# SeanChenxy/TDRN

Measured on AMD Instinct MI355X. Metric: frames/sec/GPU @320x320 dualrefinedet_vggbn; box Linf vs CPU ref, higher is better.
Workload: dtype bf16; 1 GPU; dualrefinedet_vggbn 320x320 multihead, bf16, batch 32 per GPU, forward + Detect(top_k 200, conf 0.01, nms 0.45), synthetic VOC-shaped frames + synthetic weights; global_batch=32, parallelism=frame-sharded x1, no per-frame collective, launch=eager, resident_batches=4, steps_in_flight=2

## Files before the change

include/tdrn_hip.h:

```cpp
#ifndef TDRN_HIP_H
#define TDRN_HIP_H

#include <stddef.h>
#include <stdint.h>

#ifdef __cplusplus
extern "C" {
#endif

#define TDRN_API __attribute__((visibility("default")))

#define TDRN_OK 0
#define TDRN_E_ARG (-1)
#define TDRN_E_SHAPE (-2)
#define TDRN_E_WORKSPACE (-3)
#define TDRN_E_UNSUPPORTED (-4)
#define TDRN_E_PARAM (-5)
#define TDRN_E_STATE (-6)
#define TDRN_E_VALUE (-7)
#define TDRN_E_DEVICE (-8)

TDRN_API const char *tdrn_version(void);
TDRN_API const char *tdrn_error_string(int code);

// ... 23 lines not shown
                                                  float *grad_weight, int N, int Cin, int H, int W, int Cout, int kW,
                                                  int kH, int dW, int dH, int padW, int padH, int dilationH,
                                                  int dilationW, int deformable_group, float scale,
                                                  void *workspace, size_t workspace_bytes, void *stream);


TDRN_API size_t tdrn_nms_workspace_bytes(int n);
TDRN_API int tdrn_nms(const float *dets, int n, double thresh, int strict_gt, int32_t *keep_out,
                      int32_t *num_out, void *workspace, size_t workspace_bytes, void *stream);

TDRN_API int tdrn_nms_topk(const float *dets, int n, float overlap, float min_score, int top_k,
                           int32_t *keep_out, int32_t *num_out, void *workspace,
                           size_t workspace_bytes, void *stream);

TDRN_API size_t tdrn_nms_topk_classes_workspace_bytes(int n, int num_classes);
TDRN_API int tdrn_nms_topk_classes(const float *boxes, const float *scores, int n, int num_classes, int first_class,
                                   float overlap, float min_score, int top_k, int32_t *keep_out, int32_t *num_out,
                                   void *workspace, size_t workspace_bytes, void *stream);

TDRN_API int tdrn_roi_resample(const float *feature, int C, int H, int W, const int32_t *cells, int n, int S, float *out,
                               void *stream);
TDRN_API int tdrn_ota_similarity(const float *boxes, const float *roi, int n, int F, const float *rows, const int32_t *row_off,
                                 int m, float *best, int32_t *arg, void *stream);

TDRN_API int tdrn_gpu_nms_host(int *keep_out, int *num_out, const float *boxes_host,
                               int boxes_num, int boxes_dim, float nms_overlap_thresh,
                               int device_id);

TDRN_API int tdrn_decode(const float *loc, const float *priors, int P, float var0, float var1,
                         float *boxes_out, void *stream);
TDRN_API int tdrn_center_size(const float *boxes, int P, float *out, void *stream);

TDRN_API int tdrn_encode(const float *matched, const float *priors, int P, float var0, float var1, float *out, void *stream);
TDRN_API size_t tdrn_match_workspace_bytes(int B, int P, int max_truths);
TDRN_API int tdrn_match(const float *truths, const int32_t *truth_off, int T_total, int max_truths, int B,
                        const float *priors, int P, const float *arm_loc, float threshold, float var0, float var1,
                        float *loc_t, int32_t *conf_t, void *workspace, size_t workspace_bytes, void *stream);
TDRN_API size_t tdrn_multibox_loss_workspace_bytes(int B, int P, int C);
TDRN_API int tdrn_multibox_loss_forward(const float *loc, const float *conf, const float *loc_t, const int32_t *conf_t,
                                        int B, int P, int C, int negpos_ratio, float *loss_out, uint8_t *sel,
                                        int32_t *num_pos, void *workspace, size_t workspace_bytes, void *stream);
TDRN_API int tdrn_multibox_loss_backward(const float *loc, const float *conf, const float *loc_t, const int32_t *conf_t,
                                         const uint8_t *sel, const int32_t *num_pos, const float *grad_loss, int B,
                                         int P, int C, float *grad_loc, float *grad_conf, void *stream);

#define TDRN_AUGMENT_MAX_TRUTHS 512
#define TDRN_AUGMENT_MAX_ROUNDS 32
#define TDRN_AUGMENT_MAX_SIZE 2048
#define TDRN_AUGMENT_CROP_FALLBACK 1
#define TDRN_AUGMENT_TAPE_EXHAUSTED 2
typedef struct {
    float brightness;
    float contrast_pre;
    float contrast_post;
    float saturation;
    float hue;
    int32_t perm[3];
    int32_t canvas_w, canvas_h, img_x, img_y;
    int32_t crop_x0, crop_y0, crop_x1, crop_y1;
    int32_t cropped;
    int32_t mirror;
    int32_t kept;
    int32_t status;
} tdrn_augment_params;
typedef struct {
    const uint8_t *data;
    int32_t h, w;
} tdrn_augment_image;
TDRN_API int tdrn_augment_sample(const int32_t *hw, const double *truths, const int32_t *truth_off, int T_total, int max_truths,
                                 int B, uint64_t seed, const int64_t *sample_ids, const double *tape, const int32_t *tape_off,
                                 tdrn_augment_params *params, float *out_truths, int32_t *out_off, void *stream);
TDRN_API int tdrn_augment_apply(const tdrn_augment_image *images, const tdrn_augment_params *params, int B, const float *mean,
                                int S, int to_rgb, float *out, void *stream);

#define TDRN_AUGMENT_TRANS_FALLBACK 4
typedef struct {
    tdrn_augment_params base;
    double shift_x, shift_y;
    int32_t trans_x, trans_y;
    int32_t attempts;
    int32_t reserved;
} tdrn_augment_pair_params;
TDRN_API int tdrn_augment_pair_sample(const int32_t *hw, const double *truths, const double *truths_t, const int32_t *truth_off,
                                      int T_total, int max_truths, int B, double max_trans_ratio, uint64_t seed,
                                      const int64_t *sample_ids, const double *tape, const int32_t *tape_off,
                                      tdrn_augment_pair_params *params, float *out_truths, float *out_truths_t,
                                      int32_t *out_off, void *stream);
TDRN_API int tdrn_augment_pair_apply(const tdrn_augment_image *images, const tdrn_augment_image *images_t,
                                     const tdrn_augment_pair_params *params, int B, const float *mean, int S, int to_rgb,
                                     float *out, float *out_t, void *stream);

TDRN_API int tdrn_prior_box(int n_maps, const int *feature_maps, double image_size,
                            const double *steps, const double *min_sizes,
                            const double *max_sizes, int n_max_sizes, const int *ar_count,
                            const double *ars, int clip, int flip, float *out_host);

TDRN_API size_t tdrn_detect_workspace_bytes(int B, int P, int C, int top_k);
TDRN_API int tdrn_detect(const float *loc, const float *conf, const float *priors,
                         const float *arm_loc, const float *scale_host, int B, int P, int C,
                         int top_k, float conf_thresh, double nms_thresh, float *out,
                         int32_t *counts_out, void *workspace, size_t workspace_bytes,
                         void *stream);
TDRN_API int tdrn_detect_dev_scale(const float *loc, const float *conf, const float *priors,
                                   const float *arm_loc, const float *scale_dev, int B, int P, int C,
                                   int top_k, float conf_thresh, double nms_thresh, float *out,
                                   int32_t *counts_out, void *workspace, size_t workspace_bytes,
                                   void *stream);

TDRN_API int tdrn_preprocess(const uint8_t *frames, int B, int H0, int W0, int S, const float mean_bgr[3],
                             int to_rgb, float *out, void *stream);
TDRN_API int tdrn_preprocess_u8(const uint8_t *frames, int B, int H0, int W0, int S, int to_rgb, uint8_t *out, void *stream);

typedef enum {
    TDRN_DRN_VGGBN = 0,
    TDRN_DRN_MOBILENET = 1,
    TDRN_SSD4SCALE_MOBILE = 2,
    TDRN_REFINEDET_VGG = 3,
    TDRN_SSD4SCALE_VGG = 4
} tdrn_model;

typedef struct {
    int model;
    int size;
    int num_classes;
    int c7_channel;
    int def_groups;
    int bn;
    int multihead;
    int deform;
    int test_phase;
    int dtype;
    int use_refine;
    int plan_flags;
    int reserved[4];
} tdrn_net_config;

#define TDRN_PLAN_NO_FUSE_FIRST 1
#define TDRN_PLAN_NO_LATE_SIDE  2
#define TDRN_PLAN_ONE_STREAM    4
#define TDRN_PLAN_NO_DEFORM_TS  8
#define TDRN_PLAN_CHAIN         16
#define TDRN_PLAN_NO_CONV_PP    32
#define TDRN_PLAN_NO_PP_SK      64
#define TDRN_PLAN_NO_CONV_PATCH 128
#define TDRN_PLAN_DWPW          512
#define TDRN_PLAN_NO_PW1X1      1024
#define TDRN_PLAN_NO_DW_SLIDE   2048
#define TDRN_PLAN_DW_SLIDE_ALL  4096
#define TDRN_PLAN_NO_CONV_WS    8192
#define TDRN_PLAN_NO_YGEMM_V2  16384
#define TDRN_PLAN_NO_HEAD3X3   32768
#define TDRN_PLAN_TS_ONE_RANGE  65536
#define TDRN_PLAN_NO_PATCH_TAIL 131072
#define TDRN_PLAN_FAULT_HANDOFF 256

typedef struct tdrn_net tdrn_net;

TDRN_API int tdrn_net_create(const tdrn_net_config *cfg, tdrn_net **out);
TDRN_API void tdrn_net_destroy(tdrn_net *net);

TDRN_API int tdrn_net_param_count(const tdrn_net *net);
TDRN_API int tdrn_net_param_info(const tdrn_net *net, int index, const char **name,
                                 int64_t shape[4], int *ndim);
TDRN_API int tdrn_net_set_param(tdrn_net *net, const char *name, const float *data_host,
                                int64_t numel);

TDRN_API size_t tdrn_net_weight_bytes(const tdrn_net *net);
TDRN_API size_t tdrn_net_workspace_bytes(const tdrn_net *net, int batch);
TDRN_API int tdrn_net_num_priors(const tdrn_net *net);

TDRN_API int tdrn_net_pack_weights(tdrn_net *net, void *weights_dev, size_t weights_bytes,
                                   void *stream);
TDRN_API int tdrn_net_adopt_weights(tdrn_net *net);

typedef struct {
    const float *x;
    int batch;
    float *arm_loc;
    float *odm_loc;
    float *conf;
    float *offsets[4];
    const float *ref_loc[4];
    float *loc_maps[4];
    void *reserved[4];
} tdrn_net_io;
typedef struct {
    const uint8_t *planes;
    float mean[3];
} tdrn_u8_frames;

TDRN_API int tdrn_net_forward(tdrn_net *net, const void *weights_dev, void *workspace,
                              size_t workspace_bytes, const tdrn_net_io *io, void *stream);

TDRN_API int tdrn_net_check(tdrn_net *net, unsigned *detail);

typedef struct {
    char name[48];
    int launches;
    double flops;
    double bytes;
    double ms;
} tdrn_kernel_stat;
TDRN_API int tdrn_net_profile(tdrn_net *net, int enable);
TDRN_API int tdrn_net_kernel_stats(tdrn_net *net, tdrn_kernel_stat *out, int max_entries);
TDRN_API int tdrn_net_op_stats(tdrn_net *net, tdrn_kernel_stat *out, int max_entries);
TDRN_API int tdrn_net_op_timeline(tdrn_net *net, float *start_ms, float *end_ms, int *lane, int max_entries);

typedef struct {
    int kind;
    int in, out, res;
    int pool;
    int off, y;
    int k, stride, pad, dil, relu, ceil_mode, splitk, groups;
    int out_kind;
    int level;
    int n_branches, k2, pad2, off_c0[2];
    int y_tap_major;
    int fused_first;
    int fused_dw;
    char w[48], b[48], bn[48], w2[48], b2[48];
    int y_groups;
} tdrn_op_info;
TDRN_API int tdrn_net_op_count(const tdrn_net *net);
TDRN_API int tdrn_net_op_info(const tdrn_net *net, int index, tdrn_op_info *out);

TDRN_API int tdrn_net_tensor_count(const tdrn_net *net);
TDRN_API int tdrn_net_tensor_info(const tdrn_net *net, int index, const char **label, int *C, int *H,
                                  int *W);
TDRN_API int tdrn_net_read_tensor(const tdrn_net *net, const void *workspace, int batch, int index,
                                  float *out_dev, void *stream);
TDRN_API int tdrn_net_write_tensor(const tdrn_net *net, void *workspace, int batch, int index,
                                   const float *in_dev, void *stream);
TDRN_API int tdrn_net_forward_from(tdrn_net *net, const void *weights_dev, void *workspace,
                                   size_t workspace_bytes, const tdrn_net_io *io, int first_op, void *stream);

#ifdef __cplusplus
}
#endif
#endif
```

tdrn_amd/_lib.py:

```python
import ctypes as C
import os

_HERE = os.path.dirname(os.path.abspath(__file__))
LIB_PATH = os.environ.get("TDRN_LIB_PATH") or os.path.join(_HERE, "lib", "libtdrn_hip.so")

F32, BF16, F16 = 0, 1, 2
DTYPES = {"fp32": F32, "f32": F32, "float32": F32, "bf16": BF16, "bfloat16": BF16, "fp16": F16,
          "f16": F16, "float16": F16, "half": F16}
DRN_VGGBN, DRN_MOBILENET, SSD4SCALE_MOBILE, REFINEDET_VGG, SSD4SCALE_VGG = range(5)

E_VALUE = -7


class TdrnError(RuntimeError):
    def __init__(self, code, what=""):
        self.code = code
        super().__init__("%s (tdrn error %d)%s" % (error_string(code), code,
                                                    (": " + what) if what else ""))


class NetConfig(C.Structure):
    _fields_ = [("model", C.c_int), ("size", C.c_int), ("num_classes", C.c_int),
                ("c7_channel", C.c_int), ("def_groups", C.c_int), ("bn", C.c_int),
                ("multihead", C.c_int), ("deform", C.c_int), ("test_phase", C.c_int),
                ("dtype", C.c_int), ("use_refine", C.c_int), ("plan_flags", C.c_int), ("reserved", C.c_int * 4)]


PLAN_NO_FUSE_FIRST, PLAN_NO_LATE_SIDE, PLAN_ONE_STREAM, PLAN_NO_DEFORM_TS, PLAN_CHAIN = 1, 2, 4, 8, 16
PLAN_NO_CONV_PP, PLAN_NO_PP_SK, PLAN_NO_CONV_PATCH, PLAN_FAULT_HANDOFF, PLAN_DWPW, PLAN_NO_PW1X1 = 32, 64, 128, 256, 512, 1024
PLAN_NO_DW_SLIDE, PLAN_DW_SLIDE_ALL, PLAN_NO_CONV_WS, PLAN_NO_YGEMM_V2, PLAN_NO_HEAD3X3, PLAN_TS_ONE_RANGE = 2048, 4096, 8192, 16384, 32768, 65536
PLAN_NO_PATCH_TAIL = 131072
E_DEVICE = -8


class NetIO(C.Structure):
    _fields_ = [("x", C.c_void_p), ("batch", C.c_int), ("arm_loc", C.c_void_p),
                ("odm_loc", C.c_void_p), ("conf", C.c_void_p), ("offsets", C.c_void_p * 4),
                ("ref_loc", C.c_void_p * 4), ("loc_maps", C.c_void_p * 4),
                ("reserved", C.c_void_p * 4)]


class KernelStat(C.Structure):
    _fields_ = [("name", C.c_char * 48), ("launches", C.c_int), ("flops", C.c_double),
                ("bytes", C.c_double), ("ms", C.c_double)]


class U8FramesABI(C.Structure):
    _fields_ = [("planes", C.c_void_p), ("mean", C.c_float * 3)]


class OpInfo(C.Structure):
    _fields_ = [("kind", C.c_int), ("in_", C.c_int), ("out", C.c_int), ("res", C.c_int), ("pool", C.c_int), ("off", C.c_int),
                ("y", C.c_int), ("k", C.c_int), ("stride", C.c_int), ("pad", C.c_int), ("dil", C.c_int), ("relu", C.c_int),
                ("ceil_mode", C.c_int), ("splitk", C.c_int), ("groups", C.c_int), ("out_kind", C.c_int), ("level", C.c_int),
                ("n_branches", C.c_int), ("k2", C.c_int), ("pad2", C.c_int), ("off_c0", C.c_int * 2), ("y_tap_major", C.c_int),
                ("fused_first", C.c_int), ("fused_dw", C.c_int), ("w", C.c_char * 48), ("b", C.c_char * 48), ("bn", C.c_char * 48), ("w2", C.c_char * 48),
                ("b2", C.c_char * 48), ("y_groups", C.c_int)]


class AugmentParams(C.Structure):
    _fields_ = [("brightness", C.c_float), ("contrast_pre", C.c_float), ("contrast_post", C.c_float), ("saturation", C.c_float),
                ("hue", C.c_float), ("perm", C.c_int32 * 3), ("canvas_w", C.c_int32), ("canvas_h", C.c_int32),
                ("img_x", C.c_int32), ("img_y", C.c_int32), ("crop_x0", C.c_int32), ("crop_y0", C.c_int32),
                ("crop_x1", C.c_int32), ("crop_y1", C.c_int32), ("cropped", C.c_int32), ("mirror", C.c_int32),
                ("kept", C.c_int32), ("status", C.c_int32)]


class AugmentImage(C.Structure):
    _fields_ = [("data", C.c_void_p), ("h", C.c_int32), ("w", C.c_int32)]


class AugmentPairParams(C.Structure):
    _fields_ = [("base", AugmentParams), ("shift_x", C.c_double), ("shift_y", C.c_double), ("trans_x", C.c_int32),
                ("trans_y", C.c_int32), ("attempts", C.c_int32), ("reserved", C.c_int32)]


AUGMENT_MAX_TRUTHS, AUGMENT_MAX_SIZE = 512, 2048
AUGMENT_CROP_FALLBACK, AUGMENT_TAPE_EXHAUSTED, AUGMENT_TRANS_FALLBACK = 1, 2, 4

OP_KINDS = ("first_conv", "conv", "conv_transpose", "depthwise", "maxpool", "l2norm", "offset_conv", "deform_heads", "other")

_lib = None

_SIGS = {
    "tdrn_version": (C.c_char_p, []),
    "tdrn_error_string": (C.c_char_p, [C.c_int]),
    "tdrn_deform_conv_workspace_bytes": (C.c_size_t, [C.c_int] * 15),
    "tdrn_deform_conv_forward": (C.c_int, [C.c_void_p] * 4 + [C.c_int] * 15 + [C.c_void_p, C.c_size_t, C.c_void_p]),
    "tdrn_deform_conv_backward_workspace_bytes": (C.c_size_t, [C.c_int] * 14),
    "tdrn_deform_conv_backward_input": (C.c_int, [C.c_void_p] * 6 + [C.c_int] * 14 + [C.c_void_p, C.c_size_t, C.c_void_p]),
    "tdrn_deform_conv_backward_parameters": (C.c_int, [C.c_void_p] * 4 + [C.c_int] * 14 + [C.c_float, C.c_void_p, C.c_size_t,
                                                                                            C.c_void_p]),
    "tdrn_nms_workspace_bytes": (C.c_size_t, [C.c_int]),
    "tdrn_nms": (C.c_int, [C.c_void_p, C.c_int, C.c_double, C.c_int, C.c_void_p, C.c_void_p,
                           C.c_void_p, C.c_size_t, C.c_void_p]),
    "tdrn_nms_topk": (C.c_int, [C.c_void_p, C.c_int, C.c_float, C.c_float, C.c_int, C.c_void_p, C.c_void_p,
                                C.c_void_p, C.c_size_t, C.c_void_p]),
    "tdrn_gpu_nms_host": (C.c_int, [C.c_void_p, C.c_void_p, C.c_void_p, C.c_int, C.c_int, C.c_float, C.c_int]),
    "tdrn_decode": (C.c_int, [C.c_void_p, C.c_void_p, C.c_int, C.c_float, C.c_float, C.c_void_p, C.c_void_p]),
    "tdrn_center_size": (C.c_int, [C.c_void_p, C.c_int, C.c_void_p, C.c_void_p]),
    "tdrn_encode": (C.c_int, [C.c_void_p, C.c_void_p, C.c_int, C.c_float, C.c_float, C.c_void_p, C.c_void_p]),
    "tdrn_match_workspace_bytes": (C.c_size_t, [C.c_int] * 3),
    "tdrn_match": (C.c_int, [C.c_void_p, C.c_void_p, C.c_int, C.c_int, C.c_int, C.c_void_p, C.c_int, C.c_void_p, C.c_float,
                             C.c_float, C.c_float, C.c_void_p, C.c_void_p, C.c_void_p, C.c_size_t, C.c_void_p]),
    "tdrn_multibox_loss_workspace_bytes": (C.c_size_t, [C.c_int] * 3),
    "tdrn_multibox_loss_forward": (C.c_int, [C.c_void_p] * 4 + [C.c_int] * 4 + [C.c_void_p] * 4 + [C.c_size_t, C.c_void_p]),
    "tdrn_multibox_loss_backward": (C.c_int, [C.c_void_p] * 7 + [C.c_int] * 3 + [C.c_void_p] * 3),
    "tdrn_augment_sample": (C.c_int, [C.c_void_p] * 3 + [C.c_int] * 3 + [C.c_uint64] + [C.c_void_p] * 7),
    "tdrn_augment_apply": (C.c_int, [C.c_void_p, C.c_void_p, C.c_int, C.c_void_p, C.c_int, C.c_int, C.c_void_p, C.c_void_p]),
    "tdrn_augment_pair_sample": (C.c_int, [C.c_void_p] * 4 + [C.c_int] * 3 + [C.c_double, C.c_uint64] + [C.c_void_p] * 8),
    "tdrn_augment_pair_apply": (C.c_int, [C.c_void_p] * 3 + [C.c_int, C.c_void_p, C.c_int, C.c_int] + [C.c_void_p] * 3),
    "tdrn_prior_box": (C.c_int, [C.c_int, C.c_void_p, C.c_double, C.c_void_p, C.c_void_p, C.c_void_p,
                                 C.c_int, C.c_void_p, C.c_void_p, C.c_int, C.c_int, C.c_void_p]),
    "tdrn_nms_topk_classes_workspace_bytes": (C.c_size_t, [C.c_int, C.c_int]),
    "tdrn_nms_topk_classes": (C.c_int, [C.c_void_p, C.c_void_p, C.c_int, C.c_int, C.c_int, C.c_float, C.c_float, C.c_int, C.c_void_p,
                                        C.c_void_p, C.c_void_p, C.c_size_t, C.c_void_p]),
    "tdrn_roi_resample": (C.c_int, [C.c_void_p, C.c_int, C.c_int, C.c_int, C.c_void_p, C.c_int, C.c_int, C.c_void_p, C.c_void_p]),
    "tdrn_ota_similarity": (C.c_int, [C.c_void_p, C.c_void_p, C.c_int, C.c_int, C.c_void_p, C.c_void_p, C.c_int, C.c_void_p, C.c_void_p,
                                      C.c_void_p]),
    "tdrn_preprocess": (C.c_int, [C.c_void_p, C.c_int, C.c_int, C.c_int, C.c_int, C.c_void_p, C.c_int, C.c_void_p, C.c_void_p]),
    "tdrn_preprocess_u8": (C.c_int, [C.c_void_p, C.c_int, C.c_int, C.c_int, C.c_int, C.c_int, C.c_void_p, C.c_void_p]),
    "tdrn_detect_workspace_bytes": (C.c_size_t, [C.c_int] * 4),
    "tdrn_detect": (C.c_int, [C.c_void_p] * 5 + [C.c_int] * 4 + [C.c_float, C.c_double, C.c_void_p,
                                                                  C.c_void_p, C.c_void_p, C.c_size_t, C.c_void_p]),
    "tdrn_detect_dev_scale": (C.c_int, [C.c_void_p] * 5 + [C.c_int] * 4 + [C.c_float, C.c_double, C.c_void_p,
                                                                            C.c_void_p, C.c_void_p, C.c_size_t, C.c_void_p]),
    "tdrn_net_create": (C.c_int, [C.POINTER(NetConfig), C.POINTER(C.c_void_p)]),
    "tdrn_net_destroy": (None, [C.c_void_p]),
    "tdrn_net_param_count": (C.c_int, [C.c_void_p]),
    "tdrn_net_param_info": (C.c_int, [C.c_void_p, C.c_int, C.POINTER(C.c_char_p), C.POINTER(C.c_int64 * 4),
                                      C.POINTER(C.c_int)]),
    "tdrn_net_set_param": (C.c_int, [C.c_void_p, C.c_char_p, C.c_void_p, C.c_int64]),
    "tdrn_net_weight_bytes": (C.c_size_t, [C.c_void_p]),
    "tdrn_net_workspace_bytes": (C.c_size_t, [C.c_void_p, C.c_int]),
    "tdrn_net_num_priors": (C.c_int, [C.c_void_p]),
    "tdrn_net_pack_weights": (C.c_int, [C.c_void_p, C.c_void_p, C.c_size_t, C.c_void_p]),
    "tdrn_net_adopt_weights": (C.c_int, [C.c_void_p]),
    "tdrn_net_forward": (C.c_int, [C.c_void_p, C.c_void_p, C.c_void_p, C.c_size_t, C.POINTER(NetIO), C.c_void_p]),
    "tdrn_net_check": (C.c_int, [C.c_void_p, C.POINTER(C.c_uint)]),
    "tdrn_net_op_count": (C.c_int, [C.c_void_p]),
    "tdrn_net_op_info": (C.c_int, [C.c_void_p, C.c_int, C.POINTER(OpInfo)]),
    "tdrn_net_tensor_count": (C.c_int, [C.c_void_p]),
    "tdrn_net_tensor_info": (C.c_int, [C.c_void_p, C.c_int, C.POINTER(C.c_char_p), C.POINTER(C.c_int),
                                       C.POINTER(C.c_int), C.POINTER(C.c_int)]),
    "tdrn_net_read_tensor": (C.c_int, [C.c_void_p, C.c_void_p, C.c_int, C.c_int, C.c_void_p, C.c_void_p]),
    "tdrn_net_write_tensor": (C.c_int, [C.c_void_p, C.c_void_p, C.c_int, C.c_int, C.c_void_p, C.c_void_p]),
    "tdrn_net_forward_from": (C.c_int, [C.c_void_p, C.c_void_p, C.c_void_p, C.c_size_t, C.POINTER(NetIO), C.c_int, C.c_void_p]),
    "tdrn_net_profile": (C.c_int, [C.c_void_p, C.c_int]),
    "tdrn_net_kernel_stats": (C.c_int, [C.c_void_p, C.POINTER(KernelStat), C.c_int]),
    "tdrn_net_op_stats": (C.c_int, [C.c_void_p, C.POINTER(KernelStat), C.c_int]),
    "tdrn_net_op_timeline": (C.c_int, [C.c_void_p, C.POINTER(C.c_float), C.POINTER(C.c_float), C.POINTER(C.c_int), C.c_int]),
}
EXPORTS = tuple(_SIGS)


def lib():
    global _lib
    if _lib is None:
        if not os.path.exists(LIB_PATH):
            raise ImportError(
                "libtdrn_hip.so is missing (%s): build it with `python -c 'import __graft_entry__ as g; "
                "g.build()'` or `make -C tdrn_amd/csrc`.  tdrn_amd has no CPU fallback." % LIB_PATH)
        try:
            import torch
            if torch.cuda.is_available():
                torch.cuda.init()
        except ImportError:
            pass
        l = C.CDLL(LIB_PATH)
        for name, (res, args) in _SIGS.items():
            fn = getattr(l, name)
            fn.restype = res
            fn.argtypes = args
        _lib = l
    return _lib


def error_string(code):
    try:
        return lib().tdrn_error_string(int(code)).decode()
    except Exception:
        return "tdrn error"


# ... 28 lines not shown
```

tdrn_amd/csrc/conv3x3_patch.hip:

```cpp
#include <cstdio>
#include <cstdlib>
#include <type_traits>

#include "kernels.h"
#include "mfma_prims.h"

#ifndef TDRN_PATCH_PRIO
#define TDRN_PATCH_PRIO 4
#endif
#ifndef TDRN_PATCH_ABLATE
#define TDRN_PATCH_ABLATE 0
#endif

namespace tdrn {

struct PatchParams {
    const char *in, *w, *zero;
    const float *bias;
    char *out, *out_pool;
    int B, H, W, Cin, Cout, Cs, Ktot;
    int relu;
    int tw, lgtw;
    int tiles_x, tiles_per_img;
    int m_tiles, n_tiles, items;
    int M;
    int tail_split;
    const float *fx, *fw, *fb;
    int fS, fCout;
    int ablate;
#ifdef TDRN_PATCH_STAMP
    unsigned *stamps;
#endif
#ifdef TDRN_PATCH_WGTIME
    unsigned long long *wgt;
#endif
};

#ifdef TDRN_PATCH_STAMP
#define STAMP_DECL unsigned long long st_t = __builtin_amdgcn_s_memtime(); unsigned st_acc[8] = {0, 0, 0, 0, 0, 0, 0, 0};
#define STAMP(k) do { const unsigned long long t_ = __builtin_amdgcn_s_memtime(); st_acc[k] += (unsigned)(t_ - st_t); st_t = t_; } while (0)
#define STAMP_FLUSH do { if (lane == 0) for (int k_ = 0; k_ < 8; ++k_) p.stamps[((size_t)blockIdx.x * 12 + wave) * 8 + k_] = st_acc[k_]; } while (0)
#else
#define STAMP_DECL
#define STAMP(k) do { } while (0)
#define STAMP_FLUSH do { } while (0)
#endif

namespace {

#ifndef TDRN_PATCH_RING
#define TDRN_PATCH_RING 3
#endif
constexpr int kRing = TDRN_PATCH_RING;
constexpr int kPatchSlots = kRing == 4 ? 43 : 44;
constexpr int kSlotsPerLoader = (kPatchSlots + 3) / 4;

}

template <typename DT, int BN, int TW, bool FUSE = false>
__global__ __launch_bounds__(768) void conv3x3_patch_kernel(const PatchParams p)
{
    static_assert(!FUSE || (BN == 64 && TW == 32 && sizeof(DT) == 2), "fused first conv: 16-bit, 64 couts, 8x32 tiles");
    constexpr bool FLAT = TW == 0;
    constexpr int LGTW = TW == 32 ? 5 : 4;
    constexpr int TPX = FUSE ? 512 : 256;
    constexpr int TH = TW ? TPX / TW : 0;
    constexpr int PXG = TPX / 64;
    constexpr int CG = 8 / PXG;
    constexpr int ES = elem_traits<DT>::bytes;
    constexpr int P16 = elem_traits<DT>::per16;
    constexpr int CK = 128 / ES;
    constexpr int BNH = BN / CG;
    constexpr int WC = BNH / 32;
    constexpr int WBYTES = BN * 128;
    constexpr int WL = BN / 32;
    constexpr int RING = BN == 128 ? kRing : 3;
    constexpr int SROWS = (ES == 2 ? 16 : 8) / ((RING == 4 && BN == 128) ? 2 : 1);
    constexpr int SSTRIDE = BNH * ES + 16;
    constexpr int NPB = FUSE ? 1 : 2;
    constexpr int PSLOTS = FUSE ? ((TH + 2) * (TW + 2) + 7) / 8 : kPatchSlots;
    constexpr int PBYTES = PSLOTS * 1024;
    constexpr int OFF_W = NPB * PBYTES;
    constexpr int OFF_S = OFF_W + RING * WBYTES;
    constexpr int OFF_B = OFF_S + 8 * SROWS * SSTRIDE;
    constexpr int RAWR = TH + 4, RAWC = 36;
    constexpr int RAWN = 3 * RAWR * RAWC;
    constexpr int RAWP = (RAWN + 63) / 64, RAWJ = (RAWP + 3) / 4;
    constexpr int FTILES = ((TH + 2) * (TW + 2) + 31) / 32, FTJ = (FTILES + 3) / 4;
    constexpr int RAWB = ((RAWN + 63) / 64) * 256;
    constexpr int OFF_R = OFF_B + 1024;
    constexpr int LDS = FUSE ? OFF_R + 2 * RAWB + 256 : OFF_B + 1024;
    static_assert(LDS <= 160 * 1024, "LDS budget");
    __shared__ __attribute__((aligned(16))) char smem[LDS];

    const int lane = threadIdx.x & 63;
    const int wave = __builtin_amdgcn_readfirstlane(threadIdx.x >> 6);
    const int nchunks = p.Cin / CK;
#ifdef TDRN_PATCH_WGTIME
    if (threadIdx.x == 0) p.wgt[2 * blockIdx.x] = __builtin_amdgcn_s_memrealtime();
#endif

    const XcdItems xi = xcd_items(p.items);
    const int slot = xi.slot, istride = xi.istride;
    int avail = p.items - xi.xcd * xi.per_xcd;
    avail = avail < xi.per_xcd ? avail : xi.per_xcd;
    int n_full = avail > slot ? (avail - slot + istride - 1) / istride : 0;
    const int item0 = xi.item0();
    [[maybe_unused]] int n_tail = 0, tail_enc = 0;
    constexpr bool TAILOK = BN == 128 && sizeof(DT) == 2 && !FUSE;
    if constexpr (TAILOK) {
        if (p.tail_split && avail > 0) {
            const int full = avail / istride, rem = avail - full * istride;
            if (full > 0 && rem > 0 && 2 * rem <= istride) {
                n_full = full;
                if (slot < 2 * rem) {
                    n_tail = 1;
                    tail_enc = 2 * (xi.xcd * xi.per_xcd + full * istride) + slot;
                }
            }
        }
    }
    const int n_it = n_full + n_tail;
    const int n_steps = n_it * nchunks * 9;
    auto item_mt = [&](int it) { return (it < n_full ? item0 + it * istride : tail_enc >> 1) / p.n_tiles; };
    auto item_c0 = [&](int it) {
        const int item = it < n_full ? item0 + it * istride : tail_enc >> 1;
        return (item % p.n_tiles) * BN + (it < n_full ? 0 : (tail_enc & 1) * 64);
    };
    const int RS = TW ? TW + 2 : p.W;

    if (wave >= 8) {
        if (TDRN_PATCH_PRIO == 4) __builtin_amdgcn_s_setprio(2);
        if (TDRN_PATCH_PRIO == 5) __builtin_amdgcn_s_setprio(3);
        const int lw = wave - 8;
        const int lrow = lane >> 3, pc = lane & 7;
        unsigned poff[kSlotsPerLoader];
        int pyx[kSlotsPerLoader];
        int plc[kSlotsPerLoader];
        {
#pragma unroll
            for (int j = 0; j < kSlotsPerLoader; ++j) {
                const int pr = (lw + 4 * j) * 8 + lrow;
                plc[j] = (pc ^ ((pr >> 1) & 7)) << 4;
                if (TW) {
                    const int py = pr / RS, px = pr - py * RS;
                    pyx[j] = py < TH + 2 ? ((py << 16) | px) : -1;
                } else {
                    pyx[j] = pr < 256 + 2 * p.W + 2 ? pr : -1;
                }
            }
        }
        const int f_r32 = lane & 31, f_hh = lane >> 5;
        [[maybe_unused]] int r_rq[FUSE ? RAWJ : 1], r_off[FUSE ? RAWJ : 1];
        [[maybe_unused]] int koff1[16];
        [[maybe_unused]] u32x4 wq1[2][2];
        if constexpr (FUSE) {
#pragma unroll
            for (int j = 0; j < RAWJ; ++j) {
                const int i = (lw + 4 * j) * 64 + lane;
                const int c = i / (RAWR * RAWC), rem = i - c * (RAWR * RAWC);
                const int r = rem / RAWC, q = rem - r * RAWC;
                r_rq[j] = i < RAWN ? ((r << 16) | q) : -1;
                r_off[j] = (c * p.fS + r) * p.fS + q;
            }
#pragma unroll
            for (int s2 = 0; s2 < 16; ++s2) {
                const int k = 16 * (s2 >> 3) + 8 * f_hh + (s2 & 7);
                const int c = k / 9, r = (k - 9 * c) / 3, q = k - 9 * c - 3 * r;
                koff1[s2] = k < 27 ? (c * RAWR + r) * RAWC + q : 0;
            }
#pragma unroll
            for (int ci = 0; ci < 2; ++ci)
#pragma unroll
                for (int ks = 0; ks < 2; ++ks)
#pragma unroll
                    for (int jj = 0; jj < 4; ++jj) {
                        const int co = ci * 32 + f_r32, k0 = 16 * ks + 8 * f_hh + 2 * jj;
                        const float a = (k0 < 27 && co < p.fCout) ? p.fw[co * 27 + k0] : 0.f;
                        const float b2 = (k0 + 1 < 27 && co < p.fCout) ? p.fw[co * 27 + k0 + 1] : 0.f;
                        wq1[ci][ks][jj] = pack2<DT>(a, b2);
                    }
            if (lw == 0) ((float *)(smem + OFF_R + 2 * RAWB))[lane] = lane < p.fCout ? p.fb[lane] : 0.f;
        }
        auto tile_origin = [&](int item, int &b, int &y0, int &x0) {
            const int mt = item / p.n_tiles;
            b = mt / p.tiles_per_img;
            const int tt = mt - b * p.tiles_per_img, ty = tt / p.tiles_x, tx = tt - ty * p.tiles_x;
            y0 = ty * TH; x0 = tx * TW;
        };
        auto load_raw = [&](int item, int buf) -> int {
            int n = 0;
            if constexpr (FUSE) {
                int b, y0, x0;
                tile_origin(item, b, y0, x0);
                const int iy0 = y0 - 2, ix0 = x0 - 2;
                const float *xb = p.fx + (size_t)b * 3 * p.fS * p.fS + ((long long)iy0 * p.fS + ix0);
                char *dst = smem + OFF_R + buf * RAWB;
#pragma unroll
                for (int j = 0; j < RAWJ; ++j) {
                    if ((lw + 4 * j) * 64 >= RAWN) continue;
                    const int yy = iy0 + (r_rq[j] >> 16), xx = ix0 + (r_rq[j] & 0xffff);
                    const bool ok = r_rq[j] >= 0 && (unsigned)yy < (unsigned)p.fS && (unsigned)xx < (unsigned)p.fS;
                    const char *src = ok ? (const char *)(xb + r_off[j]) : p.zero + (lane & 15) * 4;
                    if constexpr (!(TDRN_PATCH_ABLATE & 1))
                        __builtin_amdgcn_global_load_lds((const __attribute__((address_space(1))) void *)src,
                                                         (__attribute__((address_space(3))) void *)(dst + (lw + 4 * j) * 256), 4, 0, 0);
                    ++n;
                }
            }
            return n;
        };
        [[maybe_unused]] int f_y0 = 0, f_x0 = 0;
        auto first_conv_tile = [&](int tt, int rawb, char *dstbuf) {
            if constexpr (FUSE) {
                const int y0 = f_y0, x0 = f_x0;
                const int pq = tt * 32 + f_r32;
                const bool valid = pq < (TH + 2) * RS;
                const int py = pq / RS, px = pq - py * RS;
                const bool inimg = valid && (unsigned)(y0 - 1 + py) < (unsigned)p.fS && (unsigned)(x0 - 1 + px) < (unsigned)p.fS;
                const float *raw = (const float *)(smem + OFF_R + rawb * RAWB);
                const float *b1 = (const float *)(smem + OFF_R + 2 * RAWB);
                const int porg = valid ? py * RAWC + px : 0;
                float xv[16];
#pragma unroll
                for (int s2 = 0; s2 < 16; ++s2) xv[s2] = raw[porg + koff1[s2]];
                f32x16 a1[2];
#pragma unroll
                for (int ci = 0; ci < 2; ++ci)
#pragma unroll
                    for (int g = 0; g < 4; ++g) {
                        const f32x4 bv = *(const f32x4 *)(b1 + ci * 32 + 8 * g + 4 * f_hh);
#pragma unroll
                        for (int j = 0; j < 4; ++j) a1[ci][4 * g + j] = bv[j];
                    }
#pragma unroll
                for (int ks = 0; ks < 2; ++ks) {
                    u32x4 xq;
#pragma unroll
                    for (int jj = 0; jj < 4; ++jj) xq[jj] = pack2<DT>(xv[8 * ks + 2 * jj], xv[8 * ks + 2 * jj + 1]);
#pragma unroll
                    for (int ci = 0; ci < 2; ++ci) Mma32<DT>::run(wq1[ci][ks], xq, a1[ci]);
                }
                if (valid) {
                    char *row = dstbuf + pq * 128 + 8 * f_hh;
                    const int sw = (pq >> 1) & 7;
#pragma unroll
                    for (int ci = 0; ci < 2; ++ci)
#pragma unroll
                        for (int g = 0; g < 4; ++g) {
                            float q4[4];
#pragma unroll
                            for (int j = 0; j < 4; ++j) q4[j] = inimg ? fmaxf(a1[ci][4 * g + j], 0.f) : 0.f;
                            *(uint2 *)(row + (((4 * ci + g) ^ sw) << 4)) = make_uint2(pack2<DT>(q4[0], q4[1]), pack2<DT>(q4[2], q4[3]));
                        }
                }
            }
        };
        int table_mt = -1;
        auto patch_table = [&](int mt) {
            if (mt == table_mt) return;
            table_mt = mt;
            const long long rowbytes = (long long)p.Cin * ES;
            if (TW) {
                const int b = mt / p.tiles_per_img, tt = mt - b * p.tiles_per_img;
                const int ty = tt / p.tiles_x, tx = tt - ty * p.tiles_x;
                const int y0 = ty * TH - 1, x0 = tx * TW - 1;
#pragma unroll
                for (int j = 0; j < kSlotsPerLoader; ++j) {
                    const int y = y0 + (pyx[j] >> 16), x = x0 + (pyx[j] & 0xffff);
                    const bool ok = pyx[j] >= 0 && (unsigned)y < (unsigned)p.H && (unsigned)x < (unsigned)p.W;
                    poff[j] = ok ? (unsigned)((((long long)b * p.H + y) * p.W + x) * rowbytes + plc[j]) : 0xFFFFFFFFu;
                }
            } else {
                const long long j0 = (long long)mt * 256 - p.W - 1;
#pragma unroll
                for (int j = 0; j < kSlotsPerLoader; ++j) {
                    const long long pix = j0 + pyx[j];
                    const bool ok = pyx[j] >= 0 && pix >= 0 && pix < p.M;
                    poff[j] = ok ? (unsigned)(pix * rowbytes + plc[j]) : 0xFFFFFFFFu;
                }
            }
        };
        unsigned woff[WL];
#pragma unroll
        for (int k = 0; k < WL; ++k) {
            const int n = (lw + 4 * k) * 8 + lrow;
            woff[k] = (unsigned)((size_t)n * p.Ktot * ES + ((pc ^ ((n >> 1) & 7)) << 4));
        }
        constexpr bool live = !(TDRN_PATCH_ABLATE & 1);
        int ws = 0, w_it = 0, w_cc = 0, w_tap = 0, wslot = 0;
        const char *wbase = p.w;
        unsigned wk = 0;
        int w_pieces = WL;
        auto weight_item = [&]() {
            wbase = p.w + (size_t)item_c0(w_it) * p.Ktot * ES;
            if constexpr (TAILOK) w_pieces = w_it < n_full ? WL : WL / 2;
        };
        constexpr bool wfixed = (TDRN_PATCH_ABLATE & 16) != 0, pfixed = (TDRN_PATCH_ABLATE & 32) != 0;
        auto load_weights = [&]() -> int {
            const int np = w_pieces;
            if (live) {
                char *dst = smem + OFF_W + wslot * WBYTES;
#pragma unroll
                for (int k = 0; k < WL; ++k)
                    if (!TAILOK || k < np) lds_dma16_ptr(wfixed ? p.w + (woff[k] & 0xffffu) : wbase + wk + woff[k], dst + (lw + 4 * k) * 1024);
            }
            ++ws;
            wslot = wslot == RING - 1 ? 0 : wslot + 1;
            wk += (unsigned)(p.Cin * ES);
            if (++w_tap == 9) {
                w_tap = 0;
                if (++w_cc == nchunks) {
                    w_cc = 0;
                    ++w_it;
                    if (w_it < n_it) weight_item();
                }
                wk = (unsigned)(w_cc * 128);
            }
            return np;
        };
        auto load_patch = [&](int j, unsigned ccoff, char *dstbuf) {
            if (!live || lw + 4 * j >= kPatchSlots || FUSE) return;
            const unsigned o = poff[j];
            lds_dma16_ptr(o == 0xFFFFFFFFu ? p.zero : (pfixed ? p.in + (o & 0xfffffu) : p.in + (size_t)o + ccoff), dstbuf + (lw + 4 * j) * 1024);
        };
        int p_it = 0, p_cc = 0, pbuf = 0;
        auto next_patch_chunk = [&]() {
            if (NPB == 2) pbuf ^= 1;
            if (++p_cc == nchunks) {
                p_cc = 0;
                ++p_it;
            }
        };

        if constexpr (FUSE) {
            if (n_it > 0) load_raw(item0, 0);
            asm volatile("s_waitcnt vmcnt(0) lgkmcnt(0)" ::: "memory");
            __builtin_amdgcn_s_barrier();
            if (n_it > 0) {
                int b_;
                tile_origin(item0, b_, f_y0, f_x0);
#pragma unroll
                for (int q = 0; q < FTJ; ++q)
                    if (lw + 4 * q < FTILES) first_conv_tile(lw + 4 * q, 0, smem);
            }
        }
        if (n_it > 0) {
            weight_item();
            if constexpr (!FUSE) {
                patch_table(item_mt(0));
#pragma unroll
                for (int j = 0; j < kSlotsPerLoader; ++j) load_patch(j, 0u, smem);
            }
#pragma unroll
            for (int k = 0; k < RING - 1; ++k)
                if (k < n_steps) load_weights();
            next_patch_chunk();
            if (lw == 0 && live)
                lds_dma16_ptr(lane < (n_full > 0 ? BN : 64) / 4 ? (const char *)(p.bias + item_c0(0)) + lane * 16 : p.zero, smem + OFF_B);
        }
        asm volatile("s_waitcnt vmcnt(0) lgkmcnt(0)" ::: "memory");
        __builtin_amdgcn_s_barrier();

        int tap = 0, c_it = 0, c_cc = 0, carried = 0;
        STAMP_DECL
        const int last_piece = lw + 4 * (kSlotsPerLoader - 1) < kPatchSlots ? 1 : 0;
        for (int g = 0; g < n_steps; ++g) {
            int issued = 0;
            if (ws < n_steps) issued = load_weights();
            if constexpr (FUSE) {
                if (tap == 0 && c_it + 1 < n_it) issued += load_raw(item0 + (c_it + 1) * istride, (c_it + 1) & 1);
            } else if (p_it < n_it && tap < 6) {
                char *dstbuf = smem + pbuf * PBYTES;
                const unsigned ccoff = (unsigned)(p_cc * 128);
                switch (tap) {
                    case 0:
                        patch_table(item_mt(p_it));
                        load_patch(0, ccoff, dstbuf); load_patch(1, ccoff, dstbuf); issued += 2; break;
                    case 1: load_patch(2, ccoff, dstbuf); load_patch(3, ccoff, dstbuf); issued += 2; break;
                    case 2: load_patch(4, ccoff, dstbuf); load_patch(5, ccoff, dstbuf); issued += 2; break;
                    case 3: load_patch(6, ccoff, dstbuf); load_patch(7, ccoff, dstbuf); issued += 2; break;
                    case 4: load_patch(8, ccoff, dstbuf); load_patch(9, ccoff, dstbuf); issued += 2; break;
                    default: load_patch(10, ccoff, dstbuf); issued += last_piece; break;
                }
            }
            if (lw == 0 && c_cc == nchunks - 1 && tap == 6 && c_it + 1 < n_it) {
                if (live) lds_dma16_ptr(lane < (c_it + 1 < n_full ? BN : 64) / 4 ? (const char *)(p.bias + item_c0(c_it + 1)) + lane * 16 : p.zero, smem + OFF_B);
                issued += 1;
            }
            STAMP(0);
            wait_vmcnt(live ? issued + (RING == 4 ? carried : 0) : 0);
            if constexpr (FUSE) asm volatile("s_waitcnt lgkmcnt(0)" ::: "memory");
            STAMP(1);
            carried = issued;
            __builtin_amdgcn_s_barrier();
            STAMP(2);
            if (++tap == 9) {
                tap = 0;
                next_patch_chunk();
                if (++c_cc == nchunks) {
                    if constexpr (FUSE) {
                        if (c_it + 1 < n_it) {
                            int b_;
                            tile_origin(item0 + (c_it + 1) * istride, b_, f_y0, f_x0);
#pragma unroll
                            for (int q = 0; q < FTJ; ++q)
                                if (lw + 4 * q < FTILES) first_conv_tile(lw + 4 * q, (c_it + 1) & 1, smem);
                            asm volatile("s_waitcnt lgkmcnt(0)" ::: "memory");
                            __builtin_amdgcn_s_barrier();
                        }
                    }
                    c_cc = 0;
                    ++c_it;
                }
            }
        }
        STAMP_FLUSH;
        return;
    }

    const int r32 = lane & 31, hh = lane >> 5;
    const int cw = wave % PXG;
    const int chalf = wave / PXG;
    char *stg = smem + OFF_S + wave * SROWS * SSTRIDE;
    f32x16 acc[WC][2];

    int base_i[2];
    unsigned tapmask[2] = {0x1FFu, 0x1FFu};
    unsigned need_mask = 0;
#pragma unroll
    for (int pt = 0; pt < 2; ++pt) {
        const int i = cw * 64 + pt * 32 + r32;
        base_i[pt] = TW ? (i >> LGTW) * RS + (i & (TW - 1)) : i;
    }
    const int wsw = (r32 >> 1) & 7;
    constexpr int CPR = BNH * ES / 16;
    constexpr int RPI = 64 / CPR;
    const int my_ch = lane % CPR, my_row = lane / CPR;
    constexpr bool compute = !(TDRN_PATCH_ABLATE & 2);

    int cur_mt = -1, n0 = 0;
    long long tile_pix0 = 0;
    int tile_row0 = 0, tile_x0 = 0;
    auto setup_item = [&](int it) {
        const int mt = item_mt(it);
        n0 = item_c0(it);
        if (mt == cur_mt) return;
        cur_mt = mt;
        if (TW) {
            const int b = mt / p.tiles_per_img, tt = mt - b * p.tiles_per_img;
            const int ty = tt / p.tiles_x, tx = tt - ty * p.tiles_x;
            tile_row0 = b * p.H + ty * TH;
            tile_x0 = tx * TW;
            tile_pix0 = (long long)tile_row0 * p.W + tile_x0;
            return;
        }
        tile_pix0 = (long long)mt * 256;
        need_mask = 0;
#pragma unroll
        for (int pt = 0; pt < 2; ++pt) {
            const long long m = tile_pix0 + cw * 64 + pt * 32 + r32;
            unsigned mk = 0;
            if (m < p.M) {
                const int rem = (int)(m % ((long long)p.H * p.W));
                const int y = rem / p.W, x = rem - y * p.W;
#pragma unroll
                for (int t = 0; t < 9; ++t) {
                    const int yy = y + t / 3 - 1, xx = x + t % 3 - 1;
                    if ((unsigned)yy < (unsigned)p.H && (unsigned)xx < (unsigned)p.W) mk |= 1u << t;
                }
            }
            tapmask[pt] = mk;
            unsigned bad = ~mk & 0x1FFu;
#pragma unroll
            for (int o = 32; o >= 1; o >>= 1) bad |= __shfl_xor(bad, o, 64);
            need_mask |= bad;
        }
        need_mask = __builtin_amdgcn_readfirstlane(need_mask);
    };

    typedef short pk_s2 __attribute__((ext_vector_type(2)));
    [[maybe_unused]] const pk_s2 relu_lo = p.relu ? pk_s2{0, 0} : pk_s2{(short)-32768, (short)-32768};
    auto pack_relu16 = [&](float a, float b) -> unsigned {
        if constexpr (sizeof(DT) == 2) return __builtin_bit_cast(unsigned, __builtin_elementwise_max(__builtin_bit_cast(pk_s2, pack2<DT>(a, b)), relu_lo));
        else return 0u;
    };
    auto epilogue16 = [&](auto wcn_tag) {
        if constexpr (sizeof(DT) == 2) {
            constexpr int WCN = decltype(wcn_tag)::value;
            const int cbase = n0 + chalf * (32 * WCN);
            constexpr int NPAIR = 2 * WCN;
            if (p.out && !(TDRN_PATCH_ABLATE & 4)) {
#pragma unroll
                for (int pt = 0; pt < 2; ++pt) {
                    const int i = cw * 64 + pt * 32 + r32;
                    long long gp;
                    if (TW) gp = tile_pix0 + (long long)(i >> LGTW) * p.W + (i & (TW - 1));
                    else { gp = tile_pix0 + i; if (gp >= p.M) gp = -1; }
                    char *row = p.out + ((size_t)(gp < 0 ? 0 : gp) * p.Cs + cbase) * 2;
#pragma unroll
                    for (int pr = 0; pr < NPAIR; ++pr) {
                        const int ci = pr >> 1, g0 = 2 * (pr & 1);
                        const f32x16 &t = acc[ci][pt];
                        const unsigned ax = pack_relu16(t[4 * g0], t[4 * g0 + 1]), ay = pack_relu16(t[4 * g0 + 2], t[4 * g0 + 3]);
                        const unsigned bx = pack_relu16(t[4 * g0 + 4], t[4 * g0 + 5]), by = pack_relu16(t[4 * g0 + 6], t[4 * g0 + 7]);
                        auto rx = __builtin_amdgcn_permlane32_swap(ax, bx, false, false);
                        auto ry = __builtin_amdgcn_permlane32_swap(ay, by, false, false);
                        if (gp >= 0 && cbase + (2 * pr + hh) * 8 < p.Cout)
                            *(u32x4 *)(row + (2 * pr + hh) * 16) = u32x4{rx[0], ry[0], rx[1], ry[1]};
                    }
                }
            }
            if constexpr (TW != 0) if (p.out_pool) {
                const int PW = p.W >> 1;
#pragma unroll
                for (int pt = 0; pt < 2; ++pt) {
                    if (TW == 32 && pt == 1) break;
                    uint2 pk[WCN][4];
#pragma unroll
                    for (int ci = 0; ci < WCN; ++ci)
#pragma unroll
                        for (int g = 0; g < 4; ++g) {
                            float m[4];
#pragma unroll
                            for (int j = 0; j < 4; ++j) {
                                float v = acc[ci][pt][4 * g + j];
                                if (TW == 32) {
                                    v = fmaxf(v, acc[ci][1][4 * g + j]);
                                } else {
                                    float va = v, vb = v;
                                    asm volatile("s_nop 1\n\tv_permlane16_swap_b32 %0, %1" : "+v"(va), "+v"(vb));
                                    v = fmaxf(va, vb);
                                }
                                v = fmaxf(v, __builtin_bit_cast(float, __builtin_amdgcn_update_dpp(0, __builtin_bit_cast(int, v), 0xB1, 0xF, 0xF, true)));
                                m[j] = v;
                            }
                            pk[ci][g] = make_uint2(pack_relu16(m[0], m[1]), pack_relu16(m[2], m[3]));
                        }
                    const int i = cw * 64 + pt * 32 + r32;
                    const long long gpool = (long long)((tile_row0 + (i >> LGTW)) >> 1) * PW + ((tile_x0 + (i & (TW - 1))) >> 1);
                    char *row = p.out_pool + ((size_t)gpool * p.Cs + cbase) * 2;
                    constexpr int NDUP = TW == 32 ? 2 : 4;
                    const int sel = TW == 32 ? (r32 & 1) : ((r32 & 1) | ((r32 >> 3) & 2));
#pragma unroll
                    for (int rd = 0; rd < (NPAIR + NDUP - 1) / NDUP; ++rd) {
                        uint2 a = pk[0][0], b = pk[0][1];
#pragma unroll
                        for (int d = 0; d < NDUP; ++d) {
                            const int pr = rd * NDUP + d;
                            if (pr < NPAIR) {
                                const bool mine = sel == d;
                                a.x = mine ? pk[pr >> 1][2 * (pr & 1)].x : a.x; a.y = mine ? pk[pr >> 1][2 * (pr & 1)].y : a.y;
                                b.x = mine ? pk[pr >> 1][2 * (pr & 1) + 1].x : b.x; b.y = mine ? pk[pr >> 1][2 * (pr & 1) + 1].y : b.y;
                            }
                        }
                        const int mypr = rd * NDUP + sel;
                        auto rx = __builtin_amdgcn_permlane32_swap(a.x, b.x, false, false);
                        auto ry = __builtin_amdgcn_permlane32_swap(a.y, b.y, false, false);
                        if (mypr < NPAIR && cbase + (2 * mypr + hh) * 8 < p.Cout)
                            *(u32x4 *)(row + (2 * mypr + hh) * 16) = u32x4{rx[0], ry[0], rx[1], ry[1]};
                    }
                }
            }
        }
    };

    auto epilogue = [&](auto wcn_tag) {
        if constexpr (sizeof(DT) == 2) { epilogue16(wcn_tag); return; }
        const int my_c = n0 + chalf * BNH + my_ch * P16;
        auto pixel_of = [&](int i) -> long long {
            if (TW) return tile_pix0 + (long long)(i >> LGTW) * p.W + (i & (TW - 1));
            const long long m = tile_pix0 + i;
            return m < p.M ? m : -1;
        };
        auto stage_quad = [&](const f32x16 &t, int ci, int g, int srow) {
            float q4[4];
#pragma unroll
            for (int j = 0; j < 4; ++j) q4[j] = p.relu ? fmaxf(t[4 * g + j], 0.f) : t[4 * g + j];
            char *d = stg + srow * SSTRIDE + (ci * 32 + 8 * g + 4 * hh) * ES;
            if constexpr (ES == 4) {
                *(f32x4 *)d = f32x4{q4[0], q4[1], q4[2], q4[3]};
            } else if constexpr (sizeof(DT) == 2 && __is_same(DT, bf16_t)) {
                typedef __bf16 bf2 __attribute__((ext_vector_type(2)));
                typedef float fl2 __attribute__((ext_vector_type(2)));
                const bf2 lo = __builtin_convertvector(fl2{q4[0], q4[1]}, bf2), hi = __builtin_convertvector(fl2{q4[2], q4[3]}, bf2);
                *(uint2 *)d = make_uint2(__builtin_bit_cast(unsigned, lo), __builtin_bit_cast(unsigned, hi));
            } else {
                typedef _Float16 h2 __attribute__((ext_vector_type(2)));
                typedef float fl2 __attribute__((ext_vector_type(2)));
                const h2 lo = __builtin_convertvector(fl2{q4[0], q4[1]}, h2), hi = __builtin_convertvector(fl2{q4[2], q4[3]}, h2);
                *(uint2 *)d = make_uint2(__builtin_bit_cast(unsigned, lo), __builtin_bit_cast(unsigned, hi));
            }
        };
        if (p.out && !(TDRN_PATCH_ABLATE & 4)) {
#pragma unroll
            for (int pt = 0; pt < 2; ++pt) {
#pragma unroll 1
                for (int rd = 0; rd < 32 / SROWS; ++rd) {
                    if (r32 / SROWS == rd) {
#pragma unroll
                        for (int ci = 0; ci < WC; ++ci)
#pragma unroll
                            for (int g = 0; g < 4; ++g) stage_quad(acc[ci][pt], ci, g, r32 % SROWS);
                    }
                    __builtin_amdgcn_s_waitcnt(0xC07F);
                    __builtin_amdgcn_wave_barrier();
#pragma unroll
                    for (int k = 0; k < SROWS / RPI; ++k) {
                        const int row = my_row + k * RPI;
                        const long long gp = pixel_of(cw * 64 + pt * 32 + rd * SROWS + row);
                        if (gp >= 0 && my_c < p.Cout)
                            *(u32x4 *)(p.out + ((size_t)gp * p.Cs + my_c) * ES) = *(const u32x4 *)(stg + row * SSTRIDE + my_ch * 16);
                    }
                    __builtin_amdgcn_wave_barrier();
                }
            }
        }
        if (p.out_pool) {
            const int PW = p.W >> 1;
            constexpr int npool = TW == 32 ? 16 : 8;
            const bool holder = (r32 & 1) == 0 && (TW == 32 || r32 < 16);
            const int prow_l = r32 >> 1;
#pragma unroll
            for (int pt = 0; pt < 2; ++pt) {
                if (TW == 32 && pt == 1) break;
#pragma unroll
                for (int ci = 0; ci < WC; ++ci)
#pragma unroll
                    for (int e = 0; e < 16; ++e) {
                        float v = acc[ci][pt][e];
                        if (TW == 32) v = fmaxf(v, acc[ci][1][e]);
                        else v = fmaxf(v, __shfl_xor(v, 16, 64));
                        v = fmaxf(v, __builtin_bit_cast(float, __builtin_amdgcn_update_dpp(0, __builtin_bit_cast(int, v), 0xB1, 0xF, 0xF, true)));
                        acc[ci][pt][e] = v;
                    }
#pragma unroll 1
                for (int rd = 0; rd < (npool + SROWS - 1) / SROWS; ++rd) {
                    if (holder && prow_l / SROWS == rd) {
#pragma unroll
                        for (int ci = 0; ci < WC; ++ci)
#pragma unroll
                            for (int g = 0; g < 4; ++g) stage_quad(acc[ci][pt], ci, g, prow_l % SROWS);
                    }
                    __builtin_amdgcn_s_waitcnt(0xC07F);
                    __builtin_amdgcn_wave_barrier();
                    const int rows_here = (npool - rd * SROWS) < SROWS ? (npool - rd * SROWS) : SROWS;
#pragma unroll
                    for (int k = 0; k < SROWS / RPI; ++k) {
                        const int row = my_row + k * RPI;
                        if (row < rows_here && my_c < p.Cout) {
                            const int pl = rd * SROWS + row;
                            const int i0 = cw * 64 + pt * 32 + 2 * pl;
                            const long long gpool = (long long)((tile_row0 + (i0 >> LGTW)) >> 1) * PW + ((tile_x0 + (i0 & (TW - 1))) >> 1);
                            *(u32x4 *)(p.out_pool + ((size_t)gpool * p.Cs + my_c) * ES) = *(const u32x4 *)(stg + row * SSTRIDE + my_ch * 16);
                        }
                    }
                    __builtin_amdgcn_wave_barrier();
                }
            }
        }
    };

    u32x4 wfA[WC], pfA[2], wfB[WC], pfB[2];
    const char *wsb = smem + OFF_W;
    const char *psb = smem;
    int prow[2] = {base_i[0], base_i[1]};
    int psw[2] = {(base_i[0] >> 1) & 7, (base_i[1] >> 1) & 7};
    auto load_frags = [&](auto wcn_tag, u32x4 *wf, u32x4 *pf, int kk) {
        constexpr int WCN = decltype(wcn_tag)::value;
        if (!compute) return;
        const int lc = 2 * kk + hh;
#pragma unroll
        for (int ci = 0; ci < WCN; ++ci) wf[ci] = *(const u32x4 *)(wsb + (chalf * (32 * WCN) + ci * 32 + r32) * 128 + ((lc ^ wsw) << 4));
#pragma unroll
        for (int pt = 0; pt < 2; ++pt) pf[pt] = *(const u32x4 *)(psb + prow[pt] * 128 + ((lc ^ psw[pt]) << 4));
    };
    auto mma_frags = [&](auto wcn_tag, const u32x4 *wf, u32x4 *pf, unsigned m0, unsigned m1) {
        constexpr int WCN = decltype(wcn_tag)::value;
        if (!compute) return;
        if constexpr (FLAT) {
#pragma unroll
            for (int j = 0; j < 4; ++j) {
                pf[0][j] &= m0;
                pf[1][j] &= m1;
            }
        }
#pragma unroll
        for (int ci = 0; ci < WCN; ++ci)
#pragma unroll
            for (int pt = 0; pt < 2; ++pt) Mma32<DT>::run(wf[ci], pf[pt], acc[ci][pt]);
    };
    auto init_acc = [&](auto wcn_tag) {
        constexpr int WCN = decltype(wcn_tag)::value;
        const char *bsrc = smem + OFF_B;
#pragma unroll
        for (int ci = 0; ci < WCN; ++ci)
#pragma unroll
            for (int g = 0; g < 4; ++g) {
                const f32x4 bv = *(const f32x4 *)(bsrc + (chalf * (32 * WCN) + ci * 32 + 8 * g + 4 * hh) * 4);
#pragma unroll
                for (int pt = 0; pt < 2; ++pt)
#pragma unroll
                    for (int j = 0; j < 4; ++j) acc[ci][pt][4 * g + j] = bv[j];
            }
    };

    if constexpr (FUSE) __builtin_amdgcn_s_barrier();
    __builtin_amdgcn_s_barrier();
    if (TDRN_PATCH_PRIO == 2 && wave >= 4) __builtin_amdgcn_s_setprio(1);
    if (TDRN_PATCH_PRIO == 3) __builtin_amdgcn_s_setprio(1);
    typedef std::integral_constant<int, WC> full_t;
    typedef std::integral_constant<int, 1> half_t;
    if (n_it > 0) {
        setup_item(0);
        init_acc(full_t{});
        load_frags(full_t{}, wfA, pfA, 0);
    }
    int it = 0, cc = 0, tap = 0, tq = 0, delta = 0, wslot = 0, pbuf = 0;
    STAMP_DECL
    auto step = [&](auto wcn) {
        unsigned m0 = 0xFFFFFFFFu, m1 = 0xFFFFFFFFu;
        if constexpr (FLAT) {
            m0 = ((tapmask[0] >> tap) & 1u) ? 0xFFFFFFFFu : 0u;
            m1 = ((tapmask[1] >> tap) & 1u) ? 0xFFFFFFFFu : 0u;
        }
        if (TDRN_PATCH_PRIO == 0) __builtin_amdgcn_s_setprio(1);
        load_frags(wcn, wfB, pfB, 1);
        __builtin_amdgcn_sched_barrier(0);
        mma_frags(wcn, wfA, pfA, m0, m1);
        __builtin_amdgcn_sched_barrier(0);
        load_frags(wcn, wfA, pfA, 2);
        __builtin_amdgcn_sched_barrier(0);
        mma_frags(wcn, wfB, pfB, m0, m1);
        __builtin_amdgcn_sched_barrier(0);
        load_frags(wcn, wfB, pfB, 3);
        __builtin_amdgcn_sched_barrier(0);
        mma_frags(wcn, wfA, pfA, m0, m1);
        if (TDRN_PATCH_PRIO == 0) __builtin_amdgcn_s_setprio(0);
        __builtin_amdgcn_s_waitcnt(0xC07F);
        STAMP(0);
        __builtin_amdgcn_s_barrier();
        STAMP(1);
        const bool item_done = tap == 8 && cc == nchunks - 1;
        wslot = wslot == RING - 1 ? 0 : wslot + 1;
        ++tap;
        if (++tq == 3) {
            tq = 0;
            delta += RS;
        }
        if (tap == 9) {
            tap = 0; tq = 0; delta = 0;
            pbuf ^= 1;
            if (++cc == nchunks) cc = 0;
        }
        wsb = smem + OFF_W + wslot * WBYTES;
        psb = smem + (NPB == 2 ? pbuf : 0) * PBYTES;
#pragma unroll
        for (int pt = 0; pt < 2; ++pt) {
            prow[pt] = base_i[pt] + delta + tq;
            psw[pt] = (prow[pt] >> 1) & 7;
        }
        if (!(FUSE && item_done)) load_frags(wcn, wfA, pfA, 0);
        __builtin_amdgcn_sched_barrier(0);
        if (TDRN_PATCH_PRIO == 0) __builtin_amdgcn_s_setprio(1);
        mma_frags(wcn, wfB, pfB, m0, m1);
        if (TDRN_PATCH_PRIO == 0) __builtin_amdgcn_s_setprio(0);
        STAMP(2);
        if (item_done) {
            epilogue(wcn);
            ++it;
            if (it < n_it) {
                setup_item(it);
                if (TAILOK && it >= n_full) {
                    init_acc(half_t{});
                    load_frags(half_t{}, wfA, pfA, 0);
                } else {
                    init_acc(full_t{});
                }
                if constexpr (FUSE) {
                    __builtin_amdgcn_s_barrier();
                    load_frags(wcn, wfA, pfA, 0);
                }
            }
            STAMP(3);
        }
    };
    const int n_steps_full = n_full * nchunks * 9;
#pragma unroll 1
    for (int g = 0; g < n_steps_full; ++g) step(full_t{});
    if constexpr (TAILOK) {
#pragma unroll 1
        for (int g = n_steps_full; g < n_steps; ++g) step(half_t{});
    }
    STAMP_FLUSH;
#ifdef TDRN_PATCH_WGTIME
    if (threadIdx.x == 0) p.wgt[2 * blockIdx.x + 1] = __builtin_amdgcn_s_memrealtime();
#endif
}

int patch_conv_supported(const ConvArgs &a)
{
    if (a.kdisable & KOFF_CONV_PATCH) return 0;
    if (a.kh != 3 || a.kw != 3 || a.stride != 1 || a.pad != 1 || a.dil != 1) return 0;
    if (a.phases != 1 || a.out_f32 || a.res) return 0;
    if (a.Ho != a.H || a.Wo != a.W) return 0;
    if (a.Npad % 64) return 0;
    if (a.o_rs != (long long)a.Wo * a.o_cs || a.o_bs != (long long)a.Ho * a.Wo * a.o_cs || a.o_base) return 0;
    if (!a.fuse_x && (long long)a.B * a.H * a.W * a.Cin * dtype_bytes(a.dtype) >= (1ll << 32)) return 0;
    if (a.W % 32 == 0 && a.H % 8 == 0) return 32;
    if (a.W % 16 == 0 && a.H % 16 == 0) return 16;
    if (2 * a.W + 2 + 256 <= kPatchSlots * 8) return -1;
    return 0;
}

template <typename DT, int BN> static int launch_patch_cfg(const PatchParams &p_in, hipStream_t s)
{
    PatchParams p = p_in;
    const int grid = persistent_grid(p.items);
#ifdef TDRN_PATCH_WGTIME
    static unsigned long long *wgt = nullptr;
    static long calls = 0, want = -1;
    if (!wgt) TDRN_HIP_TRY(hipMalloc((void **)&wgt, 256 * 2 * sizeof(unsigned long long)));
    if (want < 0) { const char *e = getenv("TDRN_WGTIME_CALL"); want = e ? atol(e) : 2000; }
    p.wgt = wgt;
    const bool report = calls >= want && calls < want + 18;
    ++calls;
    if (report) TDRN_HIP_TRY(hipMemsetAsync(wgt, 0, 256 * 2 * sizeof(unsigned long long), s));
    struct Report {
        bool on; hipStream_t s; int grid; const PatchParams &p; unsigned long long *d;
        ~Report() {
            if (!on) return;
            (void)hipStreamSynchronize(s);
            unsigned long long h[512];
            (void)hipMemcpy(h, d, sizeof(h), hipMemcpyDeviceToHost);
            unsigned long long t0 = ~0ull, t1 = 0;
            int n = 0;
            for (int i = 0; i < grid; ++i) if (h[2 * i]) { t0 = h[2 * i] < t0 ? h[2 * i] : t0; t1 = h[2 * i + 1] > t1 ? h[2 * i + 1] : t1; ++n; }
            double late = 0, busy = 0, worst = 0, e_min = 1e18; int n5 = 0, n20 = 0;
            for (int i = 0; i < grid; ++i) if (h[2 * i]) {
                const double d0 = (h[2 * i] - t0) * 0.01, b = (h[2 * i + 1] - h[2 * i]) * 0.01, e = (h[2 * i + 1] - t0) * 0.01;
                late += d0; busy += b; worst = d0 > worst ? d0 : worst; e_min = e < e_min ? e : e_min; n5 += d0 > 5; n20 += d0 > 20;
            }
            fprintf(stderr, "wgtime %dx%d Cin %d Cout %d items %d grid %d: span %.1f us, workgroup busy mean %.1f us, first end at %.1f us; start later than the first: mean %.1f us, max %.1f us, > 5 us: %d, > 20 us: %d of %d\n",
                    p.H, p.W, p.Cin, p.Cout, p.items, grid, (t1 - t0) * 0.01, busy / n, e_min, late / n, worst, n5, n20, n);
        }
    } rep{report, s, grid, p, wgt};
#endif
    if constexpr (BN == 64 && sizeof(DT) == 2) {
        if (p.fx) {
            if (p.tw != 32 || p.n_tiles != 1 || p.H % 16) return TDRN_E_UNSUPPORTED;
            hipLaunchKernelGGL((conv3x3_patch_kernel<DT, 64, 32, true>), dim3(grid), dim3(768), 0, s, p);
            return hip_status(hipGetLastError());
        }
    }
    if (p.fx) return TDRN_E_UNSUPPORTED;
    if (p.tw == 0) hipLaunchKernelGGL((conv3x3_patch_kernel<DT, BN, 0>), dim3(grid), dim3(768), 0, s, p);
    else if (p.tw == 32) hipLaunchKernelGGL((conv3x3_patch_kernel<DT, BN, 32>), dim3(grid), dim3(768), 0, s, p);
    else hipLaunchKernelGGL((conv3x3_patch_kernel<DT, BN, 16>), dim3(grid), dim3(768), 0, s, p);
    return hip_status(hipGetLastError());
}

int launch_conv3x3_patch(const ConvArgs &a, void *out_pool, hipStream_t s)
{
    const int mode = patch_conv_supported(a);
    if (!mode) return TDRN_E_UNSUPPORTED;
    if (out_pool && (mode < 0 || (a.H & 1) || (a.W & 1))) return TDRN_E_UNSUPPORTED;
    if (out_pool && ws_conv_supported(a)) {
        const int rc = launch_conv3x3_ws(a, out_pool, s);
        if (rc != TDRN_E_UNSUPPORTED) return rc;
    }
    if (!out_pool && pp_conv_supported(a)) {
        const int rc = launch_conv3x3_pp(a, s);
        if (rc != TDRN_E_UNSUPPORTED) return rc;
    }
    PatchParams p;
    p.in = (const char *)a.in; p.w = (const char *)a.w; p.zero = (const char *)a.zero_page; p.bias = a.bias;
    p.out = (char *)a.out; p.out_pool = (char *)out_pool;
    p.B = a.B; p.H = a.H; p.W = a.W; p.Cin = a.Cin; p.Cout = a.Cout; p.Cs = (int)a.o_cs; p.Ktot = 9 * a.Cin;
    p.relu = a.relu;
    p.tw = mode > 0 ? mode : 0;
    p.lgtw = mode == 32 ? 5 : (mode == 16 ? 4 : 0);
    p.M = a.B * a.H * a.W;
    conv_tiles(a.B, a.H, a.W, p.tw, a.fuse_x ? 512 : 256, p.tiles_x, p.tiles_per_img, p.m_tiles);
    int BN = a.Npad % 128 == 0 ? 128 : 64;
    if (BN == 128 && p.m_tiles * (a.Npad / 128) < 160) BN = 64;
    p.n_tiles = a.Npad / BN;
    p.items = p.m_tiles * p.n_tiles;
    static int ablate = -1;
    if (ablate < 0) ablate = dev_ablate_env("TDRN_CONV_ABLATE");
    p.ablate = ablate;
    p.fx = a.fuse_x; p.fw = a.fuse_w; p.fb = a.fuse_b; p.fS = a.H; p.fCout = a.fuse_cout;
    p.tail_split = !(a.kdisable & KOFF_PATCH_TAIL);
    if (p.items <= 0) return TDRN_OK;
#ifdef TDRN_PATCH_STAMP
    static unsigned *stamps = nullptr;
    if (!stamps) TDRN_HIP_TRY(hipMalloc((void **)&stamps, 256 * 12 * 8 * sizeof(unsigned)));
    TDRN_HIP_TRY(hipMemsetAsync(stamps, 0, 256 * 12 * 8 * sizeof(unsigned), s));
    p.stamps = stamps;
    struct Report {
        const PatchParams &p; hipStream_t s; int BN, nchunks;
        ~Report()
        {
            static unsigned host[256 * 12 * 8];
            (void)hipStreamSynchronize(s);
            (void)hipMemcpy(host, p.stamps, sizeof(host), hipMemcpyDeviceToHost);
            double c[4] = {0, 0, 0, 0}, l[3] = {0, 0, 0};
            int nc = 0, nl = 0;
            for (int b = 0; b < 256; ++b)
                for (int w = 0; w < 12; ++w) {
                    const unsigned *v = host + (b * 12 + w) * 8;
                    if (v[0] + v[1] + v[2] == 0) continue;
                    if (w < 8) { for (int k = 0; k < 4; ++k) c[k] += v[k]; ++nc; }
                    else { for (int k = 0; k < 3; ++k) l[k] += v[k]; ++nl; }
                }
            if (!nc || !nl) return;
            const double steps = (double)((p.items + 255) / 256) * nchunks * 9;
            fprintf(stderr, "patch_stamp H%d W%d Cin%d Cout%d BN%d tw%d items%d steps/CU~%.0f | consumer cyc/wave: slices0-2 %.0f barrier %.0f slice3 %.0f epilogue %.0f"
                            " | loader cyc/wave: issue %.0f vmcnt %.0f barrier %.0f\n",
                    p.H, p.W, p.Cin, p.Cout, BN, p.tw, p.items, steps, c[0] / nc, c[1] / nc, c[2] / nc, c[3] / nc, l[0] / nl, l[1] / nl, l[2] / nl);
        }
    } report{p, s, BN, (int)(p.Cin * dtype_bytes(a.dtype) / 128)};
#endif
#define LP(DT)                                                    \
    return BN == 128 ? launch_patch_cfg<DT, 128>(p, s) : launch_patch_cfg<DT, 64>(p, s)
    switch (a.dtype) {
        case TDRN_F32: LP(float);
        case TDRN_BF16: LP(bf16_t);
        case TDRN_F16: LP(f16_t);
    }
#undef LP
    return TDRN_E_ARG;
}

}
```

tdrn_amd/csrc/conv3x3_pp.hip:

```cpp
#include <cstdio>
#include <type_traits>

#include "kernels.h"
#include "mfma_prims.h"

#ifndef TDRN_PP_ABLATE
#define TDRN_PP_ABLATE 0
#endif

namespace tdrn {

struct PPParams {
    const char *in, *w, *zero;
    const float *bias;
    char *out;
    int B, H, W, Cin, Cout, Cs, Ktot;
    int relu;
    int tiles_x, tiles_per_img;
    int m_tiles, n_tiles, items;
    int n_major;
    int M;
    float *sk_slab;
    unsigned *sk_flag;
    unsigned *status;
// ... 319 lines not shown
            for (int pt = 0; pt < 2; ++pt) Mma32<DT>::run(wf[ci][k2], pf[pt][k2], acc[ci][pt]);
    };
#define PP_SB() __builtin_amdgcn_sched_barrier(0)

    int kseg = 0, cur_item, cc, c1cur;
    seg(0, cur_item, cc, c1cur);
    int n_kseg = 0, n_item = 0, n_cc = 0, n_c1 = 0;
    auto next_chunk = [&]() {
        if (cc + 1 < c1cur) {
            n_kseg = kseg; n_item = cur_item; n_cc = cc + 1; n_c1 = c1cur;
        } else {
            n_kseg = kseg + 1;
            if (n_kseg < n_seg) seg(n_kseg, n_item, n_cc, n_c1);
        }
    };
    next_chunk();
    unsigned w_cur = weight_off(cur_item, cc), w_nxt = n_kseg < n_seg ? weight_off(n_item, n_cc) : 0u;
    int pbuf = 0, cpar = 0;
    patch_tile(cur_item);
#pragma unroll
    for (int j = 0; j < kPPPieces; ++j) {
        prep_patch(j, (unsigned)(cc * 128), 0);
        issue_patch();
    }
    pp_any = false;
#pragma unroll
    for (int k = 0; k < 4; ++k) weight_piece(k, w_cur, 0);
    if (wave == 0 && cc == 0) load_bias(cur_item);
    if (wave == 1 && lane < 8) *(u32x4 *)(smem + OFF_Z + lane * 16) = u32x4{0u, 0u, 0u, 0u};
    asm volatile("s_waitcnt vmcnt(0) lgkmcnt(0)" ::: "memory");
    PP_VM0();
    wg_barrier();
    setup_item(cur_item);
    begin_acc(cc);
    step_addresses(0, 0, 0, 0u);
    PP_LGKM0();
    PP_VM0();
    if (grp == 1) wg_barrier();

    const unsigned tapbytes = (unsigned)(p.Cin * ES);
    auto step = [&](auto tapc) {
        constexpr int T = decltype(tapc)::value;
        const bool nvalid = n_kseg < n_seg;
        const bool more = T < 8 || nvalid;
        const unsigned w_next = T < 8 ? w_cur + (unsigned)(T + 1) * tapbytes : w_nxt;
        const int slot_next = (cpar + T + 1) & 1;
        read_frags(0);
        PP_SB();
        if (more) {
            weight_piece(0, w_next, slot_next);
            weight_piece(1, w_next, slot_next);
        }
        PP_LGKM0();
        wg_barrier();
        __builtin_amdgcn_s_setprio(1);
        mma_quad(0, 0);
        PP_SB();
        if (more) weight_piece(2, w_next, slot_next);
        PP_SB();
        mma_quad(0, 1);
        mma_quad(1, 0);
        PP_SB();
        if (more) weight_piece(3, w_next, slot_next);
        PP_SB();
        mma_quad(1, 1);
        __builtin_amdgcn_s_setprio(0);
        wg_barrier();
        read_frags(1);
        PP_SB();
        pp_any = false;
        if constexpr (T < kPPPieces) {
            if (nvalid) {
                if constexpr (T == 0) patch_tile(n_item);
                prep_patch(T, (unsigned)(n_cc * 128), (pbuf ^ 1) * PBYTES);
            }
        }
        const int fly_patch = pp_any ? 1 : 0;
        if constexpr (T < kPPPieces) issue_patch();
        bool bias_now = false;
        if constexpr (T == 6) {
            bias_now = wave == 0 && nvalid && n_kseg != kseg && n_cc == 0;
            if (bias_now) load_bias(n_item);
        }
        PP_LGKM0();
        wg_barrier();
        __builtin_amdgcn_s_setprio(1);
        mma_quad(0, 0);
        mma_quad(0, 1);
        PP_SB();
        if constexpr (T < 8) step_addresses(slot_next, pbuf, ((T + 1) / 3) * RS + (T + 1) % 3, (unsigned)(T + 1));
        else if (n_kseg == kseg) step_addresses(slot_next, pbuf ^ 1, 0, 0u);
        PP_SB();
        mma_quad(1, 0);
        mma_quad(1, 1);
        __builtin_amdgcn_s_setprio(0);
        {
            const int fly = (TDRN_PP_ABLATE & (1 | 8 | 16)) ? 0 : fly_patch + (bias_now ? 1 : 0);
            if (fly == 0) asm volatile("s_waitcnt vmcnt(0)" ::: "memory");
            else if (fly == 1) asm volatile("s_waitcnt vmcnt(1)" ::: "memory");
            else asm volatile("s_waitcnt vmcnt(2)" ::: "memory");
        }
        wg_barrier();
    };
#pragma unroll 1
    for (;;) {
        step(std::integral_constant<int, 0>{});
        step(std::integral_constant<int, 1>{});
        step(std::integral_constant<int, 2>{});
        step(std::integral_constant<int, 3>{});
        step(std::integral_constant<int, 4>{});
        step(std::integral_constant<int, 5>{});
        step(std::integral_constant<int, 6>{});
        step(std::integral_constant<int, 7>{});
        step(std::integral_constant<int, 8>{});
        const bool seg_done = n_kseg != kseg;
        const int dead_buf = pbuf;
        const int c1_done = c1cur;
        pbuf ^= 1;
        cpar ^= 1;
        kseg = n_kseg; cur_item = n_item; cc = n_cc; c1cur = n_c1;
        if (kseg < n_seg) {
            w_cur = w_nxt;
            next_chunk();
            w_nxt = n_kseg < n_seg ? weight_off(n_item, n_cc) : 0u;
        }
        if (seg_done) {
            if (grp == 0) wg_barrier();
            if (c1_done == nchunks) epilogue(smem + dead_buf * PBYTES + wave * STRIP);
            else write_partial();
            if (kseg < n_seg) {
                setup_item(cur_item);
                begin_acc(cc);
                step_addresses(cpar, pbuf, 0, 0u);
            }
            PP_LGKM0();
            if (grp == 1) wg_barrier();
            if (kseg >= n_seg) break;
        }
    }
    if (grp == 0) wg_barrier();

}

size_t conv_pp_sk_bytes() { return 1024 + (size_t)256 * 8 * 32 * 64 * 16; }

int pp_conv_supported(const ConvArgs &a)
{
    if (a.kdisable & KOFF_CONV_PP) return 0;
    if (a.dtype == TDRN_F32 || a.fuse_x) return 0;
    if (a.Cin < 256 || a.Cin % 64 || a.Npad % 256) return 0;
    return patch_conv_supported(a);
}

int launch_conv3x3_pp(const ConvArgs &a, hipStream_t s)
{
    const int mode = pp_conv_supported(a);
    if (!mode) return TDRN_E_UNSUPPORTED;
    PPParams p;
    p.in = (const char *)a.in; p.w = (const char *)a.w; p.zero = (const char *)a.zero_page; p.bias = a.bias;
    p.out = (char *)a.out;
    p.B = a.B; p.H = a.H; p.W = a.W; p.Cin = a.Cin; p.Cout = a.Cout; p.Cs = (int)a.o_cs; p.Ktot = 9 * a.Cin;
    p.relu = a.relu;
    p.M = a.B * a.H * a.W;
    const int tw = mode > 0 ? mode : 0;
    conv_tiles(a.B, a.H, a.W, tw, 256, p.tiles_x, p.tiles_per_img, p.m_tiles);
    p.n_tiles = a.Npad / 256;
    p.items = p.m_tiles * p.n_tiles;
    p.n_major = p.n_tiles > 1 ? 1 : 0;
    if (p.items <= 0) return TDRN_OK;
    if (p.items < 192) return TDRN_E_UNSUPPORTED;
    const int grid = persistent_grid(p.items);
    p.sk_slab = nullptr; p.sk_flag = nullptr;
    p.status = a.status; p.fault = a.fault_handoff; p.poll_max = a.fault_handoff ? (1u << 10) : (1u << 20);
    if (a.sk_ws && !(a.kdisable & KOFF_PP_SK) && grid == 256 && p.items > grid && p.items % grid != 0) {
        p.sk_flag = (unsigned *)a.sk_ws;
        p.sk_slab = (float *)((char *)a.sk_ws + 1024);
        if (!a.sk_flags_zero) TDRN_HIP_TRY(hipMemsetAsync(p.sk_flag, 0, 1024, s));
    }
#define PP_LAUNCH(DT)                                                                                                  \
    do {                                                                                                               \
        if (tw == 0) hipLaunchKernelGGL((conv3x3_pp_kernel<DT, 0>), dim3(grid), dim3(512), 0, s, p);                  \
        else if (tw == 32) hipLaunchKernelGGL((conv3x3_pp_kernel<DT, 32>), dim3(grid), dim3(512), 0, s, p);           \
        else hipLaunchKernelGGL((conv3x3_pp_kernel<DT, 16>), dim3(grid), dim3(512), 0, s, p);                          \
    } while (0)
    if (a.dtype == TDRN_BF16) PP_LAUNCH(bf16_t);
    else PP_LAUNCH(f16_t);
#undef PP_LAUNCH
    return hip_status(hipGetLastError());
}

}
```

tdrn_amd/csrc/kernels.h:

```cpp
#pragma once
#include <cmath>

#include "common.h"

namespace tdrn {

constexpr size_t kZeroPageBytes = 256;

int allow_big_lds(const void *kernel);

enum KernelOff {
    KOFF_CONV_PP = 1,
    KOFF_PP_SK = 2,
    KOFF_CONV_PATCH = 4,
    KOFF_PW1X1 = 8,
    KOFF_DW_SLIDE = 16,
    KOFF_DW_STRIP_SMALL = 32,
    KOFF_CONV_WS = 64,
    KOFF_YGEMM_V2 = 128,
    KOFF_HEAD3X3 = 256,
    KOFF_TS_RANGES = 512,
    KOFF_PATCH_TAIL = 1024,
};

struct ConvArgs {
    const void *in = nullptr, *w = nullptr, *res = nullptr, *zero_page = nullptr;
    const float *bias = nullptr;
    void *out = nullptr;
    int B = 0, H = 0, W = 0, Cin = 0;
    int Ho = 0, Wo = 0, Cout = 0, Npad = 0;
    int kh = 1, kw = 1, stride = 1, pad = 0, dil = 1;
    int relu = 0, out_f32 = 0, phases = 1;
    int splitk = 1;
    void *partial = nullptr;
    long long o_bs = 0, o_rs = 0, o_cs = 0, o_base = 0, o_pr = 0, o_pc = 0;
    int dtype = TDRN_BF16;
    const float *fuse_x = nullptr, *fuse_w = nullptr, *fuse_b = nullptr;
    int fuse_cout = 0;
    const unsigned char *fuse_x8 = nullptr;
    float fuse_mean[3] = {0.f, 0.f, 0.f};
    void *sk_ws = nullptr;
    bool sk_flags_zero = false;
    int kdisable = 0;
    unsigned *status = nullptr;
    int fault_handoff = 0;
};
int launch_conv(const ConvArgs &a, hipStream_t s);
struct ChainLayer { ConvArgs a; int dep[2] = {-1, -1}; };
int conv_chain_supported(const ConvArgs &a);
int conv_chain_max_layers();
size_t conv_chain_ctr_bytes();
int launch_conv_chain(const ChainLayer *layers, int n, unsigned *ctr, hipStream_t s, unsigned *status = nullptr);
int conv_splitk_choice(const ConvArgs &a);
size_t conv_splitk_bytes(const ConvArgs &a, int splits);
int head3x3_supported(const ConvArgs &a);
int launch_head3x3(const ConvArgs &a, hipStream_t s);
int patch_conv_supported(const ConvArgs &a);
int patch_conv_takes(const ConvArgs &a);
int launch_conv3x3_patch(const ConvArgs &a, void *out_pool, hipStream_t s);
int pp_conv_supported(const ConvArgs &a);
int launch_conv3x3_pp(const ConvArgs &a, hipStream_t s);
size_t conv_pp_sk_bytes();
int ws_conv_supported(const ConvArgs &a);
int launch_conv3x3_ws(const ConvArgs &a, void *out_pool, hipStream_t s);
inline int persistent_grid(int items) { return items >= 256 ? 256 : ((items + 7) / 8) * 8; }
inline void conv_tiles(int B, int H, int W, int tw, int px, int &tiles_x, int &tiles_per_img, int &m_tiles)
{
    tiles_x = tw ? W / tw : 0;
    tiles_per_img = tw ? tiles_x * (H / (px / tw)) : 0;
    m_tiles = tw ? B * tiles_per_img : cdiv(B * H * W, 256);
}
int conv_n_pad(int cout);
constexpr int kChanPad = 64;

int launch_first_conv(const float *x, const float *w, const float *bias, void *out, int B, int S,
                      int stride, int Cout, int Cpad, int relu, int dtype, hipStream_t s);
int launch_maxpool2(const void *in, void *out, int B, int H, int W, int C, int ceil_mode, int dtype,
                    hipStream_t s);
int launch_l2norm(const void *in, const float *w, void *out, long long pixels, int C, int dtype,
                  hipStream_t s);
int launch_dwconv3(const void *in, const float *w, const float *bias, void *out, int B, int H, int W,
                   int C, int stride, int relu, int dtype, hipStream_t s, int kdisable = 0);
struct DwPwArgs {
    const void *in = nullptr, *w = nullptr;
    const float *wdw = nullptr, *bdw = nullptr, *bias = nullptr;
    void *out = nullptr;
    int B = 0, H = 0, W = 0, Cin = 0, Cout = 0, Npad = 0, Cs = 0;
    int stride = 1, relu_dw = 1, relu = 1, dtype = TDRN_BF16;
};
int dwpw_supported(const DwPwArgs &a);
int launch_dwpw(const DwPwArgs &a, hipStream_t s);
int pw1x1_supported(const ConvArgs &a);
int launch_pw1x1(const ConvArgs &a, hipStream_t s);
int launch_softmax_rows(const float *in, float *out, long long R, int C, hipStream_t s);
int launch_offset_conv(const float *loc, long long loc_bs, long long loc_ps, const float *w,
                       const float *bias, float *off, int B, int HW, int n_in, int n_out,
                       hipStream_t s);
struct OffsetProblem { const float *loc; long long loc_bs, loc_ps; const float *w, *bias; float *off; int B, HW, n_out, blk0; };
struct OffsetMulti { OffsetProblem pr[4]; int n; };
int launch_offset_conv_multi(const OffsetProblem *pr, int n, hipStream_t s);
int launch_nchw_to_nhwc(const float *in, void *out, int B, int C, int HW, int Cpad, int dtype,
                        hipStream_t s);
int launch_nchw_to_nhwc_grouped(const float *in, void *out, int B, int C, int HW, int G, int cpg_pad, int dtype,
                                hipStream_t s);
int launch_repack_oihw(const float *w, void *out, int Cout, int Npad, int Cin, int taps, int G, int cpg_pad, int dtype,
                       hipStream_t s);
int launch_nhwc_to_nchw_f32(const float *in, long long in_bs, long long in_ps, float *out, int B,
                            int C, int HW, hipStream_t s);
int launch_nhwc_any_to_nchw_f32(const void *in, int dtype, int Cpad, float *out, int B, int C, int HW, hipStream_t s);
int launch_preprocess(const unsigned char *in, int B, int H0, int W0, int S, const float *mean_bgr, int to_rgb, float *out,
                      hipStream_t s);
int launch_preprocess_u8(const unsigned char *in, int B, int H0, int W0, int S, int to_rgb, unsigned char *out, hipStream_t s);
int launch_u8_planes_to_f32(const unsigned char *in, int B, int S, const float *mean, float *out, hipStream_t s);
int launch_fill_zero(void *p, size_t bytes, hipStream_t s);

struct DeformBranch {
    const float *off = nullptr;
    int off_stride = 0;
    const void *w = nullptr;
    int kh = 3, kw = 3, pad = 1, stride = 1, dil = 1, G = 1;
    int pad_w = -1, stride_w = -1, dil_w = -1;
    int off_rows = 0, off_row0 = 0;
};
struct DeformArgs {
    const void *in = nullptr, *zero_page = nullptr;
    DeformBranch br[2];
    int n_branches = 1;
    int B = 0, H = 0, W = 0, Cin = 0, Ho = 0, Wo = 0, Cout = 0, Npad = 0;
    float *out0 = nullptr, *out1 = nullptr;
    int split = 0;
    long long o0_bs = 0, o0_ps = 0, o1_bs = 0, o1_ps = 0;
    int dtype = TDRN_BF16;
};
int launch_deform(const DeformArgs &a, hipStream_t s);
int launch_deform_multi(const DeformArgs *args, int n, hipStream_t s, int split_branches);
int deform_n_pad(int cout);
struct DeformBwdGeom { int N, Cin, H, W, Cout, kh, kw, sh, sw, ph, pw, dh, dw, G, Ho, Wo; };
int deform_bwd_cpg64(const DeformBwdGeom &g);
int deform_bwd_data_px(const DeformBwdGeom &g);
int launch_deform_bwd_data(const DeformBwdGeom &g, const float *in_nhwc, const float *off, const float *gout, const float *wr,
                           float *gin_nhwc, float *goff, hipStream_t s);
int launch_deform_bwd_input_add(const DeformBwdGeom &g, const float *gin_nhwc, float *grad_input, hipStream_t s);
void deform_bwd_weight_splits(const DeformBwdGeom &g, int &splits, int &per_split);
int launch_deform_bwd_weight(const DeformBwdGeom &g, const float *in_nhwc, const float *off, const float *gout, float *slab, float *grad_weight,
                             float scale, hipStream_t s);
int deform_sample_supported(const DeformArgs &a);
int deform_sample_cols(int taps);
constexpr int deform_y_col(int tap) { return (tap / 3) * 256 + (tap % 3) * 80; }
int deform_ts_max_batch(int H, int W, int ycs, int taps);
int launch_deform_sample_multi(const DeformArgs *args, const void *const *y, const int *ycs, int n, hipStream_t s, int tap_major = 0);
int ygemm_supported(int Cin, int ycols, int dtype);
int launch_ygemm(const void *x, const void *w, void *y, long long M, int N, int ycs, int dtype, hipStream_t s, int taps = 0);
struct YGemmProblem { const void *x, *w; void *y; long long M; int N, ycs, taps; };
int launch_ygemm_multi(const YGemmProblem *pr, int n, int dtype, hipStream_t s, int kdisable = 0);

int launch_decode(const float *loc, const float *priors, int P, float v0, float v1, float *out,
                  hipStream_t s);
int launch_center_size(const float *boxes, int P, float *out, hipStream_t s);
size_t detect_workspace_bytes(int B, int P, int C, int top_k);
int launch_detect(const float *loc, const float *conf, const float *priors, const float *arm_loc,
                  const float *scale4, int scale_on_device, int B, int P, int C, int top_k, float conf_thresh,
                  double nms_thresh, float *out, int32_t *counts, void *ws, size_t ws_bytes,
                  hipStream_t s);
size_t nms_workspace_bytes(int n);
size_t nms_classes_workspace_bytes(int n, int C);
int launch_roi_resample(const float *feat, int C, int H, int W, const int32_t *cells, int n, int S, float *out, hipStream_t s);
int launch_ota_similarity(const float *boxes, const float *roi, int n, int F, const float *rows, const int32_t *row_off, int m, float *best,
                          int32_t *arg, hipStream_t s);
int launch_nms_classes(const float *boxes, const float *scores, int n, int C, int first_class, float overlap, float min_score, int top_k,
                       int32_t *keep_out, int32_t *num_out, void *ws, size_t ws_bytes, hipStream_t s);
int launch_nms(const float *dets, int n, double thresh, int strict_gt, int presorted,
               int32_t *keep_out, int32_t *num_out, void *ws, size_t ws_bytes, hipStream_t s,
               int plain_rule = 0, float min_score = -INFINITY, int pre_top_k = 0);

constexpr int kMaxMatchTruths = 512;
constexpr int kMaxLossClasses = 1024;
size_t match_workspace_bytes(int B, int P, int max_truths);
int launch_match(const float *truths, const int32_t *truth_off, int T_total, int max_truths, int B, const float *priors, int P,
                 const float *arm_loc, float threshold, float var0, float var1, float *loc_t, int32_t *conf_t, void *ws,
                 size_t ws_bytes, hipStream_t s);
int launch_encode(const float *matched, const float *priors, int P, float v0, float v1, float *out, hipStream_t s);
size_t multibox_loss_workspace_bytes(int B, int P, int C);
int launch_multibox_loss_forward(const float *loc, const float *conf, const float *loc_t, const int32_t *conf_t, int B, int P,
                                 int C, int negpos_ratio, float *loss_out, uint8_t *sel, int32_t *num_pos, void *ws,
                                 size_t ws_bytes, hipStream_t s);
int launch_multibox_loss_backward(const float *loc, const float *conf, const float *loc_t, const int32_t *conf_t,
                                  const uint8_t *sel, const int32_t *num_pos, const float *grad_loss, int B, int P, int C,
                                  float *grad_loc, float *grad_conf, hipStream_t s);

int launch_augment_sample(const int32_t *hw, const double *truths, const int32_t *truth_off, int T_total, int max_truths, int B,
                          uint64_t seed, const int64_t *sample_ids, const double *tape, const int32_t *tape_off,
                          tdrn_augment_params *params, float *out_truths, int32_t *out_off, hipStream_t s);
int launch_augment_apply(const tdrn_augment_image *images, const tdrn_augment_params *params, int B, const float *mean, int S,
                         int to_rgb, float *out, hipStream_t s);

int launch_augment_pair_sample(const int32_t *hw, const double *truths, const double *truths_t, const int32_t *truth_off,
                               int T_total, int max_truths, int B, double max_trans_ratio, uint64_t seed,
                               const int64_t *sample_ids, const double *tape, const int32_t *tape_off,
                               tdrn_augment_pair_params *params, float *out_truths, float *out_truths_t, int32_t *out_off,
                               hipStream_t s);
int launch_augment_pair_apply(const tdrn_augment_image *images, const tdrn_augment_image *images_t,
                              const tdrn_augment_pair_params *params, int B, const float *mean, int S, int to_rgb, float *out,
                              float *out_t, hipStream_t s);

}
```

tdrn_amd/csrc/net.h:

```cpp
#pragma once
#include "net_plan.h"

struct tdrn_net : tdrn::Plan {
    tdrn::StagedParams staged;
    bool weights_ready = false;
    int profile = 0;
    std::vector<hipEvent_t> ev;
    std::vector<int> ev_stat;
    std::vector<int> ev_op;
    tdrn_kernel_stat stats[tdrn::ST_COUNT];
    int last_batch = 0;
    const void *offs_ws = nullptr;
    int offs_batch = 0, offs_key_batch = 0;
    int dev = -1;
    unsigned *status = nullptr;
    bool lanes_ready = false;
    hipStream_t side[tdrn::kLanes - 1] = {nullptr, nullptr, nullptr};
    hipEvent_t ev_fork = nullptr, ev_zero = nullptr, ev_skz = nullptr, ev_join[tdrn::kLanes - 1] = {nullptr, nullptr, nullptr};
    std::vector<hipEvent_t> tensor_ev;
    int first_op = 0;

    int init_lanes();
    int check_status(unsigned *detail);
    int collect_stats(tdrn_kernel_stat *out, int max_entries);
};

namespace tdrn {
namespace pool {
int cur_dev();
int get_timing_event(int dev, hipEvent_t *e);
int get_status(unsigned **w);
}
int run_forward(tdrn_net &n, const void *blob, void *ws, size_t ws_bytes, const tdrn_net_io *io, hipStream_t s0);
}
```

tdrn_amd/csrc/net.hip:

```cpp
#include <cstring>
#include <mutex>

#include "net.h"

namespace tdrn {

namespace pool {
std::mutex mu;
std::map<int, std::vector<hipStream_t>> streams;
std::map<int, std::vector<hipEvent_t>> events;
std::map<int, std::vector<hipEvent_t>> timing_events;
std::vector<unsigned *> status_words;
int cur_dev()
{
    int d = 0;
    (void)hipGetDevice(&d);
    return d;
}
template <class H, class Create>
int get(std::map<int, std::vector<H>> &m, int dev, H *h, Create create)
{
    {
        std::lock_guard<std::mutex> g(mu);
        auto &v = m[dev];
        if (!v.empty()) { *h = v.back(); v.pop_back(); return TDRN_OK; }
    }
    return hip_status(create(h));
}
template <class H>
void put(std::map<int, std::vector<H>> &m, int dev, H h) { if (h) { std::lock_guard<std::mutex> g(mu); m[dev].push_back(h); } }
int get_stream(int dev, hipStream_t *s) { return get(streams, dev, s, [](hipStream_t *p) { return hipStreamCreateWithFlags(p, hipStreamNonBlocking); }); }
int get_event(int dev, hipEvent_t *e) { return get(events, dev, e, [](hipEvent_t *p) { return hipEventCreateWithFlags(p, hipEventDisableTiming); }); }
int get_timing_event(int dev, hipEvent_t *e) { return get(timing_events, dev, e, [](hipEvent_t *p) { return hipEventCreate(p); }); }
int get_status(unsigned **w)
{
    {
        std::lock_guard<std::mutex> g(mu);
        if (!status_words.empty()) { *w = status_words.back(); status_words.pop_back(); memset(*w, 0, 64); return TDRN_OK; }
    }
    void *p = nullptr;
    TDRN_HIP_TRY(hipHostMalloc(&p, 64, hipHostMallocMapped | hipHostMallocPortable));
    memset(p, 0, 64);
    *w = (unsigned *)p;
    return TDRN_OK;
}
void put_status(unsigned *w) { if (w) { std::lock_guard<std::mutex> g(mu); status_words.push_back(w); } }
}

namespace {
const char *kStatNames[] = {"conv_igemm_mfma", "first_conv", "maxpool2x2", "l2norm", "dwconv3x3", "offset_conv1x1",
                            "deform_gemm_mfma", "softmax21", "layout", "conv3x3_patch_mfma", "dwpw_mfma"};
}
}

using namespace tdrn;

int tdrn_net::init_lanes()
{
    if (lanes_ready) return TDRN_OK;
    for (int i = 0; i < kLanes - 1; ++i) {
        TDRN_TRY(pool::get_stream(dev, &side[i]));
        TDRN_TRY(pool::get_event(dev, &ev_join[i]));
    }
    TDRN_TRY(pool::get_event(dev, &ev_fork));
    TDRN_TRY(pool::get_event(dev, &ev_zero));
    TDRN_TRY(pool::get_event(dev, &ev_skz));
    tensor_ev.assign(tensors.size(), nullptr);
    for (size_t t = 0; t < tensors.size(); ++t)
        if (tensor_shared[t]) TDRN_TRY(pool::get_event(dev, &tensor_ev[t]));
    lanes_ready = true;
    return TDRN_OK;
}

int tdrn_net::check_status(unsigned *detail)
{
    unsigned d = 0;
    if (status) {
        volatile unsigned *w = status;
        d = (w[0] ? 1u : 0u) | (w[1] ? 2u : 0u);
        if (d) { w[0] = 0; w[1] = 0; }
    }
    if (detail) *detail = d;
    return d ? TDRN_E_DEVICE : TDRN_OK;
}

int tdrn_net::collect_stats(tdrn_kernel_stat *out, int max_entries)
{
    for (int i = 0; i < ST_COUNT; ++i) {
        memset(&stats[i], 0, sizeof(stats[i]));
        strncpy(stats[i].name, kStatNames[i], sizeof(stats[i].name) - 1);
    }
    for (size_t i = 0; i < ops.size(); ++i) {
        const Op &o = ops[i];
        if (launch_head(i)) stats[o.stat].launches += 1;
        stats[o.stat].flops += o.flops * last_batch;
        stats[o.stat].bytes += o.bytes * last_batch;
    }
    for (size_t i = 0; i < ev_stat.size(); ++i) {
        float ms = 0.f;
        TDRN_HIP_TRY(hipEventSynchronize(ev[2 * i + 1]));
        TDRN_HIP_TRY(hipEventElapsedTime(&ms, ev[2 * i], ev[2 * i + 1]));
        stats[ev_stat[i]].ms += ms;
    }
    int n = 0;
    for (int i = 0; i < ST_COUNT && n < max_entries; ++i)
        if (stats[i].launches) out[n++] = stats[i];
    return n;
}

extern "C" {

int tdrn_net_create(const tdrn_net_config *cfg, tdrn_net **out)
{
    if (!cfg || !out) return TDRN_E_ARG;
    tdrn_net *n = new tdrn_net();
    n->cfg = *cfg;
    const int rc = n->build();
    if (rc != TDRN_OK) {
        delete n;
        return rc;
    }
    *out = n;
    return TDRN_OK;
}

void tdrn_net_destroy(tdrn_net *net)
{
    if (!net) return;
    const int d = net->dev;
    for (hipEvent_t e : net->ev) pool::put(pool::timing_events, d, e);
    for (hipEvent_t e : net->tensor_ev) pool::put(pool::events, d, e);
    for (int i = 0; i < kLanes - 1; ++i) {
        pool::put(pool::events, d, net->ev_join[i]);
        pool::put(pool::streams, d, net->side[i]);
    }
    pool::put(pool::events, d, net->ev_fork);
    pool::put(pool::events, d, net->ev_zero);
    pool::put(pool::events, d, net->ev_skz);
    pool::put_status(net->status);
    delete net;
}

int tdrn_net_param_count(const tdrn_net *net) { return net ? (int)net->params.size() : TDRN_E_ARG; }

int tdrn_net_param_info(const tdrn_net *net, int index, const char **name, int64_t shape[4], int *ndim)
{
    if (!net || index < 0 || index >= (int)net->params.size()) return TDRN_E_ARG;
    const ParamSpec &p = net->params[index];
    if (name) *name = p.name.c_str();
    if (ndim) *ndim = (int)p.shape.size();
    if (shape)
        for (size_t i = 0; i < 4; ++i) shape[i] = i < p.shape.size() ? p.shape[i] : 1;
    return TDRN_OK;
}

int tdrn_net_set_param(tdrn_net *net, const char *name, const float *data_host, int64_t numel)
{
    if (!net || !name || !data_host) return TDRN_E_ARG;
    auto it = net->param_index.find(name);
    if (it == net->param_index.end()) return TDRN_E_PARAM;
    int64_t want = 1;
    for (int64_t d : net->params[it->second].shape) want *= d;
    if (want != numel) return TDRN_E_PARAM;
    net->staged[name].assign(data_host, data_host + numel);
    net->weights_ready = false;
    return TDRN_OK;
}

size_t tdrn_net_weight_bytes(const tdrn_net *net) { return net ? net->blob_bytes : 0; }
size_t tdrn_net_workspace_bytes(const tdrn_net *net, int batch) { return net && batch > 0 ? net->ws_per_sample * (size_t)batch + net->ws_fixed : 0; }
int tdrn_net_num_priors(const tdrn_net *net) { return net ? net->P : TDRN_E_ARG; }

int tdrn_net_pack_weights(tdrn_net *net, void *weights_dev, size_t weights_bytes, void *stream)
{
    if (!net || !weights_dev) return TDRN_E_ARG;
    if (weights_bytes < net->blob_bytes) return TDRN_E_WORKSPACE;
    for (const ParamSpec &p : net->params)
        if (!net->staged.count(p.name)) return TDRN_E_PARAM;
    std::vector<char> host;
    TDRN_TRY(pack_weights(*net, net->staged, host));
    hipStream_t s = (hipStream_t)stream;
    TDRN_HIP_TRY(hipMemcpyAsync(weights_dev, host.data(), host.size(), hipMemcpyHostToDevice, s));
    TDRN_HIP_TRY(hipStreamSynchronize(s));
    net->weights_ready = true;
    net->staged.clear();
    return TDRN_OK;
}

int tdrn_net_adopt_weights(tdrn_net *net)
{
    if (!net) return TDRN_E_ARG;
    net->weights_ready = true;
    return TDRN_OK;
}

int tdrn_net_forward(tdrn_net *net, const void *weights_dev, void *workspace, size_t workspace_bytes, const tdrn_net_io *io,
                     void *stream)
{
    if (!net) return TDRN_E_ARG;
    return run_forward(*net, weights_dev, workspace, workspace_bytes, io, (hipStream_t)stream);
}

int tdrn_net_check(tdrn_net *net, unsigned *detail)
{
    if (!net) return TDRN_E_ARG;
    return net->check_status(detail);
}

int tdrn_net_op_count(const tdrn_net *net) { return net ? (int)net->ops.size() : TDRN_E_ARG; }

int tdrn_net_op_info(const tdrn_net *net, int index, tdrn_op_info *out)
{
    if (!net || !out || index < 0 || index >= (int)net->ops.size()) return TDRN_E_ARG;
    const Op &o = net->ops[index];
    memset(out, 0, sizeof(*out));
    switch (o.kind) {
        case OP_FIRST: out->kind = 0; break;
        case OP_CONV: out->kind = o.phases == 4 ? 2 : 1; break;
        case OP_DW: out->kind = 3; break;
        case OP_POOL: out->kind = 4; break;
        case OP_L2NORM: out->kind = 5; break;
        case OP_OFFSET: out->kind = 6; break;
        case OP_DEFORM: out->kind = 7; break;
        default: out->kind = 8; break;
    }
    out->in = o.in; out->out = o.out; out->res = o.res; out->pool = o.pool_t; out->off = o.off_t; out->y = o.y_t;
    out->k = o.k; out->stride = o.stride; out->pad = o.pad; out->dil = o.dil; out->relu = o.relu; out->ceil_mode = o.ceil;
    out->splitk = o.splitk; out->groups = o.G; out->out_kind = o.out_kind; out->level = o.scale;
    out->n_branches = o.n_branches; out->k2 = o.k2; out->pad2 = o.pad2; out->off_c0[0] = o.off_c0[0]; out->off_c0[1] = o.off_c0[1];
    if (o.kind == OP_DEFORM && o.y_t >= 0) {
        out->y_tap_major = net->y_tap_major ? 1 : 0;
        out->y_groups = o.y_groups;
    }
    out->fused_first = (index == net->fuse_first) ? 1 : 0;
    out->fused_dw = o.fused_dw;
    auto cp = [](char *d, const std::string &v) { strncpy(d, v.c_str(), 47); };
    cp(out->w, o.w); cp(out->b, o.b); cp(out->bn, o.bn); cp(out->w2, o.w2); cp(out->b2, o.b2);
    return TDRN_OK;
}

int tdrn_net_tensor_count(const tdrn_net *net) { return net ? (int)net->tensors.size() : TDRN_E_ARG; }

int tdrn_net_tensor_info(const tdrn_net *net, int index, const char **label, int *C, int *H, int *W)
{
    if (!net || index < 0 || index >= (int)net->tensors.size()) return TDRN_E_ARG;
    const Tensor &t = net->tensors[index];
    if (label) *label = t.label.c_str();
    if (C) *C = t.C;
    if (H) *H = t.H;
    if (W) *W = t.W;
    return TDRN_OK;
}

int tdrn_net_read_tensor(const tdrn_net *net, const void *workspace, int batch, int index, float *out_dev, void *stream)
{
    if (!net || !workspace || !out_dev || batch <= 0 || index < 0 || index >= (int)net->tensors.size()) return TDRN_E_ARG;
    const Tensor &t = net->tensors[index];
    return launch_nhwc_any_to_nchw_f32((const char *)workspace + t.off * (size_t)batch, t.f32 ? TDRN_F32 : net->cfg.dtype,
                                       t.Cpad, out_dev, batch, t.C, t.H * t.W, (hipStream_t)stream);
}

int tdrn_net_write_tensor(const tdrn_net *net, void *workspace, int batch, int index, const float *in_dev, void *stream)
{
    if (!net || !workspace || !in_dev || batch <= 0 || index < 0 || index >= (int)net->tensors.size()) return TDRN_E_ARG;
    const Tensor &t = net->tensors[index];
    return launch_nchw_to_nhwc(in_dev, (char *)workspace + t.off * (size_t)batch, batch, t.C, t.H * t.W, t.Cpad,
                               t.f32 ? TDRN_F32 : net->cfg.dtype, (hipStream_t)stream);
}

int tdrn_net_forward_from(tdrn_net *net, const void *weights_dev, void *workspace, size_t workspace_bytes, const tdrn_net_io *io,
                          int first_op, void *stream)
{
    if (!net || first_op < 0 || first_op > (int)net->ops.size()) return TDRN_E_ARG;
    if (net->use_lanes) return TDRN_E_STATE;
    net->first_op = first_op;
    const int rc = run_forward(*net, weights_dev, workspace, workspace_bytes, io, (hipStream_t)stream);
    net->first_op = 0;
    return rc;
}

int tdrn_net_profile(tdrn_net *net, int enable)
{
    if (!net) return TDRN_E_ARG;
    net->profile = enable < 0 ? 0 : (enable > 2 ? 2 : enable);
    return TDRN_OK;
}

int tdrn_net_op_stats(tdrn_net *net, tdrn_kernel_stat *out, int max_entries)
{
    if (!net || !out || max_entries <= 0) return TDRN_E_ARG;
    int n = 0;
    for (size_t i = 0; i < net->ev_op.size() && n < max_entries; ++i) {
        const Op &o = net->ops[net->ev_op[i]];
        float ms = 0.f;
        TDRN_HIP_TRY(hipEventSynchronize(net->ev[2 * i + 1]));
        TDRN_HIP_TRY(hipEventElapsedTime(&ms, net->ev[2 * i], net->ev[2 * i + 1]));
        tdrn_kernel_stat &k = out[n++];
        memset(&k, 0, sizeof(k));
        std::string name = std::string(kStatNames[o.stat]) + ":" + (o.w.empty() ? (o.in >= 0 ? net->tensors[o.in].label : "") : o.w);
        if (o.kind == OP_CONV && o.chain == 0) name = "conv_chain:" + o.w + "+" + std::to_string(net->chain_ops.size() - 1);
        strncpy(k.name, name.c_str(), sizeof(k.name) - 1);
        k.launches = 1;
        k.flops = o.flops * net->last_batch;
        k.bytes = o.bytes * net->last_batch;
        if (o.kind == OP_CONV && o.chain == 0)
            for (size_t j = 1; j < net->chain_ops.size(); ++j) {
                k.flops += net->ops[net->chain_ops[j]].flops * net->last_batch;
                k.bytes += net->ops[net->chain_ops[j]].bytes * net->last_batch;
            }
        if (o.kind == OP_DEFORM)
            for (int j = net->ev_op[i] - 1; j >= 0 && net->ops[j].kind == OP_DEFORM; --j) {
                k.flops += net->ops[j].flops * net->last_batch;
                k.bytes += net->ops[j].bytes * net->last_batch;
            }
        k.ms = ms;
    }
    return n;
}

int tdrn_net_op_timeline(tdrn_net *net, float *start_ms, float *end_ms, int *lane, int max_entries)
{
    if (!net || !start_ms || !end_ms || max_entries <= 0) return TDRN_E_ARG;
    int n = 0;
    for (size_t i = 0; i < net->ev_op.size() && n < max_entries; ++i, ++n) {
        TDRN_HIP_TRY(hipEventSynchronize(net->ev[2 * i + 1]));
        TDRN_HIP_TRY(hipEventElapsedTime(&start_ms[n], net->ev[0], net->ev[2 * i]));
        TDRN_HIP_TRY(hipEventElapsedTime(&end_ms[n], net->ev[0], net->ev[2 * i + 1]));
        if (lane) lane[n] = net->profile == 2 && net->use_lanes ? net->ops[net->ev_op[i]].lane : 0;
    }
    return n;
}

int tdrn_net_kernel_stats(tdrn_net *net, tdrn_kernel_stat *out, int max_entries)
{
    if (!net || !out || max_entries <= 0) return TDRN_E_ARG;
    return net->collect_stats(out, max_entries);
}

}
```

tdrn_amd/csrc/net_plan.h:

```cpp
#pragma once
#include <map>
#include <string>
#include <vector>

#include "kernels.h"

namespace tdrn {

enum OpKind { OP_FIRST, OP_CONV, OP_POOL, OP_L2NORM, OP_DW, OP_OFFSET, OP_DEFORM, OP_SOFTMAX, OP_OFF_OUT, OP_LOC_OUT,
              OP_REFLOC_IN };
enum OutKind { OUT_TENSOR = 0, OUT_ARM_LOC = 1, OUT_ODM_LOC = 2, OUT_CONF = 3 };
enum { ST_CONV, ST_FIRST, ST_POOL, ST_L2, ST_DW, ST_OFFSET, ST_DEFORM, ST_SOFTMAX, ST_LAYOUT, ST_CONV3, ST_DWPW, ST_COUNT };

struct Tensor { int C, Cpad, H, W; bool f32; size_t off;  std::string label; };
struct ParamSpec { std::string name; std::vector<int64_t> shape; };
using StagedParams = std::map<std::string, std::vector<float>>;

struct Op {
    OpKind kind;
    int in = -1, out = -1, res = -1;
    int Cin = 0, Cout = 0, Npad = 0, k = 1, stride = 1, pad = 0, dil = 1, relu = 0, phases = 1, ceil = 0;
    int out_kind = OUT_TENSOR, scale = 0, hw = 0;
    int G = 1, n_branches = 1, k2 = 0, pad2 = 0;
    int taps = 0;
    int split = 0;
    int off_t = -1, off_c0[2] = {0, 0}, off_n = 0;
    int loc_src = OUT_ARM_LOC;
    std::string w, b, bn, w2, b2;
    size_t w_off = 0, b_off = 0, w2_off = 0;
    int y_t = -1, y_cols = 0;
    int y_groups = 1;
    size_t wt_off = 0, bt_off = 0;
    double flops = 0, bytes = 0;
    int stat = 0;
    int lane = 0;
    int pool_t = -1;
    int splitk = 1;
    bool chain_tag = false;
    int chain = -1;
    int fused_dw = 0;
    size_t chain_partial = 0;
};

constexpr int kLanes = 4;
constexpr size_t kTailCtl = 256;

struct Plan {
    tdrn_net_config cfg{};
    int es = 2;
    std::vector<Tensor> tensors;
    std::vector<ParamSpec> params;
    std::map<std::string, size_t> param_index;
    std::vector<Op> ops;
    size_t ws_per_sample = 0, blob_bytes = kZeroPageBytes;
    size_t ws_fixed = 0;
    int P = 0, fm[4] = {0, 0, 0, 0}, scale_off[5] = {0, 0, 0, 0, 0};
    size_t splitk_off[kLanes] = {0, 0, 0, 0};
    int t_late = -1;
    std::vector<int> chain_ops;
    size_t chain_partial_off = 0;
    bool pp_sk_planned = false;
    int fuse_first = -1;
    int x_t = -1;
    bool late_side = true;
    bool use_lanes = true;
    bool y_tap_major = true;
    int kdisable = 0, fault_handoff = 0;
    std::vector<int> tensor_lane;
    std::vector<char> tensor_shared;

    int build();
    int producer_of(int t) const;
    int readers_of(int t) const;
    void conv_geometry(const Op &o, int B, ConvArgs &a) const;
    bool launch_continues(size_t i) const
    {
        return i + 1 < ops.size() && ops[i + 1].kind == ops[i].kind && (ops[i].kind == OP_DEFORM || ops[i].kind == OP_OFFSET);
    }
    bool launch_head(size_t i) const
    {
        const Op &o = ops[i];
        return !(i > 0 && launch_continues(i - 1)) && !(o.kind == OP_CONV && (o.chain > 0 || o.fused_dw));
    }

private:
    int cur_lane = 0, plan_error = TDRN_OK;
    int T(int C, int H, int W, bool f32 = false);
    void P_(const std::string &name, std::vector<int64_t> shape);
    void bn_params(const std::string &bn, int C);
    int push(Op &o, const std::string &l = "") { o.lane = cur_lane; if (!l.empty()) label(o.out, l); ops.push_back(o); return o.out; }
    void label(int t, const std::string &l) { if (t >= 0) tensors[t].label = l; }
    size_t blob(size_t bytes);
    int first_conv(const std::string &w, bool bias, const std::string &bn, int Cout, int stride, int S);
    int conv(int in, const std::string &w, bool bias, const std::string &bn, int Cout, int k, int stride, int pad, int dil,
             int relu, int res = -1, int out_kind = OUT_TENSOR, int scale = 0, const std::string &w2 = "", int k2 = 0);
    int conv_transpose2(int in, const std::string &w, bool bias, int Cout, int res, int relu);
    bool can_fuse_pool(int in) const;
    int pool(int in, int ceil_mode, bool in_needed_elsewhere = false);
    int l2norm(int in, const std::string &name);
    int dwconv(int in, const std::string &w, const std::string &bn, int stride);
    int conv_dw(int in, const std::string &name, int Cout, int stride);
    int offset_conv(int scale, int H, int W, const std::string &w1, const std::string &w2, bool bias, int n1, int n2,
                    int loc_src, int ref_tensor = -1);
    void deform_heads(int in, int off_t, int scale, int G, const std::string &loc1, const std::string &conf1,
                      const std::string &loc2, const std::string &conf2, int off_c1, int out_loc_kind);
    void softmax_op();
    void offsets_out(int scale, int off_t, int n);
    void loc_maps_out(int scale);
    int ref_loc_in(int scale, int H, int W);
    void set_pyramid(int s0);
    void vgg_trunk(int S, bool bn, int c7, int &c43, int &c53, int &fc7);
    void vgg_sources(int src[4]);
    void tcb(const int src[4], bool bias, int odm[4]);
    void drn_heads(const int src[4], const int odm[4], bool bias);
    void mobilenet_sources(int S, int c7, bool extras_bias, int src[4]);
    int build_drn(bool mobile);
    int build_refinedet_vgg();
    int build_ssd4scale(bool mobile);
    void alias_u8_input();
    void hoist_l2norm_to_side_lanes();
    void plan_fuse_first();
    void plan_splitk();
    void plan_chain();
    void place_splitk_slabs();
    void plan_dwpw();
    void plan_workspace_tail();
    void mark_shared_tensors();
};

int pack_weights(const Plan &p, const StagedParams &staged, std::vector<char> &host);

}
```

tdrn_amd/csrc/net_plan.hip:

```cpp
#include <algorithm>
#include <cstdlib>

#include "net_plan.h"

namespace tdrn {

int Plan::T(int C, int H, int W, bool f32)
{
    Tensor t;
    t.C = C; t.H = H; t.W = W; t.f32 = f32;
    t.Cpad = f32 ? C : (int)align_up((size_t)C, kChanPad);
    t.off = ws_per_sample;
    ws_per_sample += align_up((size_t)t.Cpad * H * W * (f32 ? 4 : es), 256);
    tensors.push_back(t);
    return (int)tensors.size() - 1;
}
void Plan::P_(const std::string &name, std::vector<int64_t> shape)
{
    param_index[name] = params.size();
    params.push_back(ParamSpec{name, std::move(shape)});
}
void Plan::bn_params(const std::string &bn, int C)
{
    P_(bn + ".weight", {C}); P_(bn + ".bias", {C}); P_(bn + ".running_mean", {C}); P_(bn + ".running_var", {C});
// ... 371 lines not shown
        for (int s = 0; s < 4; ++s) rl[s] = ref_loc_in(s, fm[s], fm[s]);
        for (int s = 0; s < 4; ++s) ot[s] = offset_conv(s, fm[s], fm[s], "offset." + std::to_string(s), "", true, 8 * 18, 0, -1, rl[s]);
        for (int s = 0; s < 4; ++s) offsets_out(s, ot[s], 8 * 18);
        for (int s = 0; s < 4; ++s) {
            const std::string ss = std::to_string(s);
            deform_heads(src[s], ot[s], s, 8, "arm_loc." + ss, "arm_conf." + ss, "", "", 0, OUT_ARM_LOC);
        }
    }
    for (int s = 0; s < 4 && !cfg.deform; ++s) {
        const std::string ss = std::to_string(s);
        conv(src[s], "arm_loc." + ss, true, "", 12, 3, 1, 1, 1, 0, -1, OUT_ARM_LOC, s);
        conv(src[s], "arm_conf." + ss, true, "", nc3, 3, 1, 1, 1, 0, -1, OUT_CONF, s);
        loc_maps_out(s);
    }
    if (cfg.test_phase) softmax_op();
    return TDRN_OK;
}

int Plan::producer_of(int t) const
{
    int prod = -1;
    for (size_t j = 0; j < ops.size(); ++j)
        if (ops[j].out == t || ops[j].pool_t == t) prod = (int)j;
    return prod;
}

int Plan::readers_of(int t) const
{
    int readers = 0;
    for (const Op &o : ops) readers += (o.in == t) + (o.res == t);
    return readers;
}

void Plan::conv_geometry(const Op &o, int B, ConvArgs &a) const
{
    const Tensor &ti = tensors[o.in];
    a.B = B; a.H = ti.H; a.W = ti.W; a.Cin = o.Cin; a.Ho = o.hw >> 16; a.Wo = o.hw & 0xffff;
    a.Cout = o.Cout; a.Npad = o.Npad; a.kh = a.kw = o.k; a.stride = o.stride; a.pad = o.pad; a.dil = o.dil;
    a.phases = o.phases; a.dtype = cfg.dtype;
    a.kdisable = kdisable;
}

void Plan::alias_u8_input()
{
    if (ops.empty() || ops[0].kind != OP_FIRST) return;
    const size_t need = align_up((size_t)3 * cfg.size * cfg.size * 4, 256);
    auto touched_early = [&](int t) {
        for (size_t i = 0; i < 2 && i < ops.size(); ++i)
            if (ops[i].in == t || ops[i].out == t || ops[i].res == t || ops[i].pool_t == t || ops[i].off_t == t) return true;
        return false;
    };
    int victim = -1;
    for (size_t i = 2; i < ops.size() && victim < 0; ++i) {
        if (ops[i].lane != 0 || !(ops[i].kind == OP_CONV || ops[i].kind == OP_DW || ops[i].kind == OP_POOL) || ops[i].in < 0) continue;
        for (int t : {ops[i].out, ops[i].pool_t}) {
            if (t < 0 || victim >= 0 || touched_early(t)) continue;
            const Tensor &v = tensors[t];
            if (align_up((size_t)v.Cpad * v.H * v.W * (v.f32 ? 4 : es), 256) >= need) victim = t;
        }
    }
    if (victim >= 0) {
        Tensor t;
        t.C = 3; t.H = cfg.size; t.W = cfg.size; t.f32 = true; t.Cpad = 3; t.off = tensors[victim].off;
        tensors.push_back(t);
        x_t = (int)tensors.size() - 1;
    } else {
        x_t = T(3, cfg.size, cfg.size, true);
    }
}

void Plan::hoist_l2norm_to_side_lanes()
{
    int side = 1;
    for (size_t i = 0; i < ops.size(); ++i) {
        if (ops[i].kind != OP_L2NORM) continue;
        const int prod = producer_of(ops[i].in);
        if (prod < 0) continue;
        Op o = ops[i];
        o.lane = side;
        side = side == 1 ? 2 : 1;
        ops.erase(ops.begin() + (long)i);
        ops.insert(ops.begin() + prod + 1, o);
    }
}

void Plan::plan_fuse_first()
{
    fuse_first = -1;
    if ((cfg.plan_flags & TDRN_PLAN_NO_FUSE_FIRST) || cfg.dtype == TDRN_F32 || (kdisable & KOFF_CONV_PATCH) || ops.size() <= 1 || ops[0].kind != OP_FIRST ||
        ops[1].kind != OP_CONV || ops[0].stride != 1 || tensors[ops[0].out].Cpad != 64) return;
    const Op &c = ops[1];
    const Tensor &ti = tensors[ops[0].out];
    if (c.in == ops[0].out && readers_of(ops[0].out) == 1 && c.k == 3 && c.stride == 1 && c.pad == 1 && c.dil == 1 && c.phases == 1 && c.res < 0 &&
        c.out_kind == OUT_TENSOR && c.Npad == 64 && c.Cin == 64 && ti.W % 32 == 0 && ti.H % 16 == 0 && ti.H == ti.W && c.lane == 0)
        fuse_first = 1;
    if (fuse_first >= 0) {
        ops[1].flops += ops[0].flops;
        ops[1].bytes += 3.0 * ops[0].hw * ops[0].hw * 4 - (double)ti.H * ti.W * ti.Cpad * es;
        ops[0].flops = 0; ops[0].bytes = 0;
    }
}

void Plan::plan_splitk()
{
    constexpr int kSplitkRefBatch = 32;
    for (Op &o : ops) {
        if (o.kind == OP_CONV && o.pool_t >= 0) o.stat = ST_CONV3;
        if (o.kind != OP_CONV || o.pool_t >= 0) continue;
        ConvArgs a;
        conv_geometry(o, kSplitkRefBatch, a);
        a.out_f32 = o.out_kind != OUT_TENSOR;
        o.splitk = conv_splitk_choice(a);
        a.o_cs = o.out_kind == OUT_TENSOR ? tensors[o.out].Cpad : 0;
        a.o_rs = (long long)a.Wo * a.o_cs; a.o_bs = (long long)a.Ho * a.Wo * a.o_cs;
        a.res = o.res >= 0 ? (const void *)1 : nullptr;
        if (o.splitk == 1 && patch_conv_takes(a)) o.stat = ST_CONV3;
        if (o.chain_tag && !(o.out_kind == OUT_TENSOR && conv_chain_supported(a))) o.chain_tag = false;
    }
}

void Plan::plan_chain()
{
    chain_ops.clear();
    const bool chain_on = (cfg.plan_flags & TDRN_PLAN_CHAIN) != 0;
    int first = -1;
    for (size_t i = 0; i < ops.size() && chain_on; ++i) {
        Op &o = ops[i];
        if (o.kind != OP_CONV || !o.chain_tag || (int)chain_ops.size() == conv_chain_max_layers()) continue;
        bool ok = true;
        for (int t : {o.in, o.res}) {
            if (t < 0) continue;
            const int prod = producer_of(t);
            const bool member = prod >= 0 && ops[prod].chain >= 0;
            if (!member && first >= 0 && prod > first) ok = false;
        }
        if (!ok) continue;
        if (first < 0) first = (int)i;
        o.chain = (int)chain_ops.size();
        chain_ops.push_back((int)i);
    }
    if (chain_ops.size() < 3) {
        for (int i : chain_ops) ops[i].chain = -1;
        chain_ops.clear();
    }
    std::vector<int> level(ops.size(), 0);
    for (size_t k = 0; k < chain_ops.size(); ++k)
        for (int t : {ops[chain_ops[k]].in, ops[chain_ops[k]].res})
            for (size_t j = 0; j < k; ++j)
                if (t >= 0 && ops[chain_ops[j]].out == t && level[chain_ops[j]] + 1 > level[chain_ops[k]]) level[chain_ops[k]] = level[chain_ops[j]] + 1;
    std::stable_sort(chain_ops.begin(), chain_ops.end(), [&](int a, int b) { return level[a] < level[b]; });
    for (size_t k = 0; k < chain_ops.size(); ++k) ops[chain_ops[k]].chain = (int)k;
}

void Plan::place_splitk_slabs()
{
    size_t lane_bytes[kLanes] = {0, 0, 0, 0};
    size_t chain_bytes = 0;
    for (Op &o : ops) {
        if (o.kind != OP_CONV || o.pool_t >= 0 || o.splitk <= 1) continue;
        const size_t per_sample = align_up((size_t)o.splitk * o.phases * (o.hw >> 16) * (o.hw & 0xffff) * o.Npad * sizeof(float), 256);
        if (o.chain >= 0) {
            o.chain_partial = chain_bytes;
            chain_bytes += per_sample;
        } else if (per_sample > lane_bytes[o.lane]) {
            lane_bytes[o.lane] = per_sample;
        }
    }
    for (int i : chain_ops) ops[i].lane = 0;
    chain_partial_off = ws_per_sample;
    ws_per_sample += chain_bytes;
    if (const char *pd = getenv("TDRN_PLAN_DUMP")) {
        if (atoi(pd))
            for (const Op &o : ops)
                if (o.kind == OP_CONV)
                    fprintf(stderr, "plan: %-28s lane %d  %dx%d k%d s%d d%d  Cin %4d Cout %4d  splitk %d  %s  chain %d\n", o.w.c_str(), o.lane,
                            o.hw >> 16, o.hw & 0xffff, o.k, o.stride, o.dil, o.Cin, o.Cout, o.splitk, o.stat == ST_CONV3 ? "patch" : "igemm", o.chain);
    }
    for (int l = 0; l < kLanes; ++l) {
        splitk_off[l] = ws_per_sample;
        ws_per_sample += lane_bytes[l];
    }
}

void Plan::plan_dwpw()
{
    if (cfg.dtype == TDRN_F32 || !(cfg.plan_flags & TDRN_PLAN_DWPW)) return;
    for (size_t i = 0; i + 1 < ops.size(); ++i) {
        Op &d = ops[i];
        Op &c = ops[i + 1];
        if (d.kind != OP_DW || c.kind != OP_CONV || c.in != d.out || c.k != 1 || c.stride != 1 || c.pad != 0 || c.phases != 1 || c.res >= 0 ||
            c.out_kind != OUT_TENSOR || c.splitk != 1 || c.lane != d.lane || c.pool_t >= 0 || c.chain >= 0) continue;
        if (readers_of(d.out) != 1) continue;
        const Tensor &ti = tensors[d.in];
        DwPwArgs a;
        a.B = 1; a.H = ti.H; a.W = ti.W; a.Cin = c.Cin; a.Cout = c.Cout; a.Npad = c.Npad; a.Cs = tensors[c.out].Cpad;
        a.stride = d.stride; a.dtype = cfg.dtype;
        if (ti.Cpad != c.Cin || !dwpw_supported(a)) continue;
        d.fused_dw = 1; c.fused_dw = 1;
        d.stat = ST_DWPW;
        d.flops += c.flops;
        d.bytes = (double)ti.H * ti.W * ti.Cpad * es + (double)ti.H * ti.W * tensors[c.out].Cpad * es;
        c.flops = 0; c.bytes = 0;
    }
}

void Plan::plan_workspace_tail()
{
    ws_fixed = 0;
    pp_sk_planned = false;
    if (cfg.dtype != TDRN_F32)
        for (const Op &o : ops)
            if (o.kind == OP_CONV && o.stat == ST_CONV3 && o.lane == 0 && o.Cin >= 256 && o.Npad % 256 == 0) pp_sk_planned = true;
    if (pp_sk_planned || !chain_ops.empty()) ws_fixed = kTailCtl + (pp_sk_planned ? align_up(conv_pp_sk_bytes(), 256) : 1024);
}

void Plan::mark_shared_tensors()
{
    tensor_lane.assign(tensors.size(), 0);
    tensor_shared.assign(tensors.size(), 0);
    for (const Op &o : ops) {
        if (o.out >= 0) tensor_lane[o.out] = o.lane;
        if (o.pool_t >= 0) tensor_lane[o.pool_t] = o.lane;
    }
    for (const Op &o : ops)
        for (int t : {o.in, o.res, o.off_t})
            if (t >= 0 && tensor_lane[t] != o.lane) tensor_shared[t] = 1;
}

int Plan::build()
{
    es = dtype_bytes(cfg.dtype);
    static const struct { int plan_flag, koff; } kSwitches[] = {
        {TDRN_PLAN_NO_CONV_PP, KOFF_CONV_PP},       {TDRN_PLAN_NO_PP_SK, KOFF_PP_SK},
        {TDRN_PLAN_NO_CONV_PATCH, KOFF_CONV_PATCH}, {TDRN_PLAN_NO_PW1X1, KOFF_PW1X1},
        {TDRN_PLAN_NO_DW_SLIDE, KOFF_DW_SLIDE},     {TDRN_PLAN_DW_SLIDE_ALL, KOFF_DW_STRIP_SMALL},
        {TDRN_PLAN_NO_CONV_WS, KOFF_CONV_WS},       {TDRN_PLAN_NO_YGEMM_V2, KOFF_YGEMM_V2},
        {TDRN_PLAN_NO_HEAD3X3, KOFF_HEAD3X3},       {TDRN_PLAN_TS_ONE_RANGE, KOFF_TS_RANGES},
        {TDRN_PLAN_NO_PATCH_TAIL, KOFF_PATCH_TAIL},
    };
    kdisable = 0;
    for (const auto &sw : kSwitches)
        if (cfg.plan_flags & sw.plan_flag) kdisable |= sw.koff;
    fault_handoff = (cfg.plan_flags & TDRN_PLAN_FAULT_HANDOFF) ? 1 : 0;
    late_side = !(cfg.plan_flags & TDRN_PLAN_NO_LATE_SIDE);
    use_lanes = !(cfg.plan_flags & TDRN_PLAN_ONE_STREAM);
    if (cfg.size < 128 || cfg.size > 1280 || cfg.size % 64 != 0) return TDRN_E_ARG;
    if (cfg.num_classes < 2 || cfg.num_classes > 21 * 4) return TDRN_E_ARG;
    if (cfg.dtype < 0 || cfg.dtype > 2) return TDRN_E_ARG;
    if (cfg.def_groups < 1) return TDRN_E_ARG;
    int rc;
    switch (cfg.model) {
        case TDRN_DRN_VGGBN: rc = build_drn(false); break;
        case TDRN_DRN_MOBILENET: rc = build_drn(true); break;
        case TDRN_SSD4SCALE_MOBILE: rc = build_ssd4scale(true); break;
        case TDRN_SSD4SCALE_VGG: rc = build_ssd4scale(false); break;
        case TDRN_REFINEDET_VGG: rc = build_refinedet_vgg(); break;
        default: return TDRN_E_UNSUPPORTED;
    }
    if (rc != TDRN_OK) return rc;
    if (plan_error != TDRN_OK) return plan_error;
    alias_u8_input();
    hoist_l2norm_to_side_lanes();
    plan_fuse_first();
    plan_splitk();
    plan_chain();
    place_splitk_slabs();
    plan_dwpw();
    plan_workspace_tail();
    y_tap_major = true;
    for (const Op &d : ops)
        if (d.kind == OP_DEFORM && d.y_t >= 0 && !ygemm_supported(d.Cin, d.y_cols, cfg.dtype)) y_tap_major = false;
    mark_shared_tensors();
    return TDRN_OK;
}

}
```

tdrn_amd/csrc/net_run.hip:

```cpp
#include "net.h"

namespace tdrn {
namespace {

struct Run {
    tdrn_net &n;
    const Plan &p;
    const void *blob; void *ws; size_t ws_bytes; const tdrn_net_io *io; hipStream_t s0;
    const char *wb = nullptr;
    const tdrn_u8_frames *u8 = nullptr;
    const float *xin = nullptr;
    int B = 0, C = 0;
    int Bk = 0;
    bool lanes = false, join_on = false, reuse_offsets = false;
    bool lane_used[kLanes] = {true, false, false, false};
    bool zeroed_early = false, skz_pending = false, dwpw_done = false;
    char *tail = nullptr;
    DeformArgs dargs[4];
    int ts_op[4] = {-1, -1, -1, -1}, n_dargs = 0;
    OffsetProblem oq[4];
    int oq_op[4], n_oq = 0;
    size_t evi = 0;
    int offset_ops_enqueued = 0;

    Run(tdrn_net &net, const void *blob_, void *ws_, size_t ws_bytes_, const tdrn_net_io *io_, hipStream_t s)
        : n(net), p(net), blob(blob_), ws(ws_), ws_bytes(ws_bytes_), io(io_), s0(s) {}
    ~Run() { (void)join(); }
    int join()
    {
        if (!join_on) return TDRN_OK;
        join_on = false;
        int rc = TDRN_OK;
        for (int l = 1; l < kLanes; ++l)
            if (lane_used[l]) {
                hipError_t e = hipEventRecord(n.ev_join[l - 1], n.side[l - 1]);
                if (e == hipSuccess) e = hipStreamWaitEvent(s0, n.ev_join[l - 1], 0);
                if (e != hipSuccess && rc == TDRN_OK) rc = (int)e;
            }
        return rc;
    }

    char *tptr(int id) const { return (char *)ws + p.tensors[id].off * (size_t)B; }
    float *loc_out(const Op &o) const { return o.out_kind == OUT_ARM_LOC ? io->arm_loc : io->odm_loc; }
    bool launch_open(const Op &o) const { return (o.kind == OP_DEFORM && n_dargs > 0) || (o.kind == OP_OFFSET && n_oq > 0); }
    int record(int t, hipStream_t s) const
    {
        if (lanes && t >= 0 && p.tensor_shared[t]) TDRN_HIP_TRY(hipEventRecord(n.tensor_ev[t], s));
        return TDRN_OK;
    }

    int check_args()
    {
        if (!n.weights_ready) return TDRN_E_STATE;
        if (!blob || !ws || !io || io->batch <= 0) return TDRN_E_ARG;
        u8 = (const tdrn_u8_frames *)io->reserved[3];
        if (u8 ? !u8->planes : !io->x) return TDRN_E_ARG;
        xin = u8 ? nullptr : io->x;
        B = io->batch;
        if (ws_bytes < p.ws_per_sample * (size_t)B + p.ws_fixed) return TDRN_E_WORKSPACE;
        if (!io->conf) return TDRN_E_ARG;
        const int d = pool::cur_dev();
        if (n.dev < 0) n.dev = d;
        else if (n.dev != d) return TDRN_E_STATE;
        if (p.ws_fixed) {
            if (!n.status) TDRN_TRY(pool::get_status(&n.status));
            TDRN_TRY(n.check_status(nullptr));
        }
        const bool is_drn = p.cfg.model == TDRN_DRN_VGGBN || p.cfg.model == TDRN_DRN_MOBILENET || p.cfg.model == TDRN_REFINEDET_VGG;
        const bool has_arm = p.cfg.model != TDRN_REFINEDET_VGG || p.cfg.use_refine;
        if (is_drn && !io->odm_loc) return TDRN_E_ARG;
        if (has_arm && !io->arm_loc) return TDRN_E_ARG;
        wb = (const char *)blob;
        C = p.cfg.num_classes;
        n.last_batch = B;
        return TDRN_OK;
    }

    int fork()
    {
        if (n.profile && n.ev.size() < 2 * p.ops.size()) {
            const size_t old = n.ev.size();
            n.ev.resize(2 * p.ops.size());
            for (size_t i = old; i < n.ev.size(); ++i) TDRN_TRY(pool::get_timing_event(n.dev, &n.ev[i]));
        }
        n.ev_stat.clear();
        n.ev_op.clear();
        lanes = p.use_lanes && n.profile != 1;
        if (lanes) {
            TDRN_TRY(n.init_lanes());
            TDRN_HIP_TRY(hipEventRecord(n.ev_fork, s0));
        }
        join_on = lanes;
        return TDRN_OK;
    }

    int open_lane(int lane, hipStream_t s)
    {
        if (!lane_used[lane]) TDRN_HIP_TRY(hipStreamWaitEvent(s, n.ev_fork, 0));
        lane_used[lane] = true;
        return TDRN_OK;
    }

    int zero_split_outputs(const Op &o, hipStream_t s) const
    {
        TDRN_HIP_TRY(hipMemsetAsync(loc_out(o), 0, (size_t)B * p.P * 4 * sizeof(float), s));
        TDRN_HIP_TRY(hipMemsetAsync(io->conf, 0, (size_t)B * p.P * C * sizeof(float), s));
        return TDRN_OK;
    }

    int zero_early()
    {
        if (lanes) {
            const Op *dsplit = nullptr;
            int n_deform_groups = 0;
            for (size_t k = 0; k < p.ops.size(); ++k)
                if (p.ops[k].kind == OP_DEFORM) {
                    if (p.ops[k].split && p.ops[k].y_t < 0 && !dsplit) dsplit = &p.ops[k];
                    if (k == 0 || p.ops[k - 1].kind != OP_DEFORM) ++n_deform_groups;
                }
            if (dsplit && n_deform_groups == 1) {
                TDRN_TRY(open_lane(1, n.side[0]));
                TDRN_TRY(zero_split_outputs(*dsplit, n.side[0]));
                TDRN_HIP_TRY(hipEventRecord(n.ev_zero, n.side[0]));
                zeroed_early = true;
            }
        }
        tail = (char *)ws + p.ws_per_sample * (size_t)B;
        if (!p.ws_fixed) return TDRN_OK;
        if (lanes) {
            TDRN_TRY(open_lane(1, n.side[0]));
            TDRN_HIP_TRY(hipMemsetAsync(tail, 0, kTailCtl + 1024, n.side[0]));
            TDRN_HIP_TRY(hipEventRecord(n.ev_skz, n.side[0]));
            skz_pending = true;
        } else {
            TDRN_HIP_TRY(hipMemsetAsync(tail, 0, kTailCtl + 1024, s0));
        }
        return TDRN_OK;
    }

    int check_reuse()
    {
        reuse_offsets = p.cfg.deform && io->reserved[0] != nullptr;
        if (reuse_offsets && (n.offs_ws != ws || n.offs_batch != B)) return TDRN_E_STATE;
        Bk = B;
        if (io->reserved[1]) {
            const long long kb = (long long)(intptr_t)io->reserved[1];
            if (!p.cfg.deform || kb < 1 || kb > B || B % kb) return TDRN_E_ARG;
            Bk = (int)kb;
        }
        if (reuse_offsets && n.offs_key_batch != Bk) return TDRN_E_STATE;
        if (p.cfg.deform && !reuse_offsets) { n.offs_ws = nullptr; n.offs_batch = 0; n.offs_key_batch = 0; }
        return TDRN_OK;
    }

    int prologue()
    {
        TDRN_TRY(check_args());
        TDRN_TRY(fork());
        TDRN_TRY(zero_early());
        return check_reuse();
    }

    int epilogue()
    {
        const int jrc = join();
        int offset_ops_planned = 0;
        for (const Op &d : p.ops) offset_ops_planned += d.kind == OP_OFFSET;
        if (jrc == TDRN_OK && p.cfg.deform && !reuse_offsets && offset_ops_planned > 0 && offset_ops_enqueued == offset_ops_planned) {
            n.offs_ws = ws; n.offs_batch = B; n.offs_key_batch = Bk;
        }
        return jrc;
    }

    bool skipped(size_t oi)
    {
        const Op &o = p.ops[oi];
        if (o.kind == OP_CONV && o.fused_dw && dwpw_done) { dwpw_done = false; return true; }
        if (o.kind == OP_OFF_OUT && !io->offsets[o.scale]) return true;
        if (o.kind == OP_LOC_OUT && !io->loc_maps[o.scale]) return true;
        if (reuse_offsets && (o.kind == OP_REFLOC_IN || o.kind == OP_OFFSET)) return true;
        if (o.kind == OP_FIRST && p.fuse_first >= 0) return true;
        if (o.kind == OP_CONV && o.chain > 0) return true;
        return (int)oi < n.first_op;
    }

    int stream_for(const Op &o, int &lane, hipStream_t &s)
    {
        lane = lanes ? o.lane : 0;
        s = lane == 0 ? s0 : n.side[lane - 1];
        if (!lanes) return TDRN_OK;
        TDRN_TRY(open_lane(lane, s));
        for (int t : {o.in, o.res, o.off_t})
            if (t >= 0 && p.tensor_lane[t] != lane) TDRN_HIP_TRY(hipStreamWaitEvent(s, n.tensor_ev[t], 0));
        if (p.late_side && lane != 0 && (o.kind == OP_CONV || o.kind == OP_OFFSET) && p.t_late >= 0 && p.tensor_shared[p.t_late])
            TDRN_HIP_TRY(hipStreamWaitEvent(s, n.tensor_ev[p.t_late], 0));
        return TDRN_OK;
    }

    int wait_tail_zeroed()
    {
        if (!skz_pending) return TDRN_OK;
        TDRN_HIP_TRY(hipStreamWaitEvent(s0, n.ev_skz, 0));
        skz_pending = false;
        return TDRN_OK;
    }

    void conv_args(const Op &o, ConvArgs &a) const
    {
        p.conv_geometry(o, B, a);
        a.in = tptr(o.in); a.w = wb + o.w_off; a.bias = (const float *)(wb + o.b_off); a.zero_page = wb;
        a.relu = o.relu;
        a.status = n.status; a.fault_handoff = p.fault_handoff;
        if (o.out_kind == OUT_TENSOR) {
            const Tensor &to = p.tensors[o.out];
            a.out = tptr(o.out);
            if (o.res >= 0) a.res = tptr(o.res);
            a.o_cs = to.Cpad;
            if (o.phases == 4) {
                a.o_bs = (long long)to.H * to.W * to.Cpad; a.o_rs = 2ll * to.W * to.Cpad; a.o_cs = 2ll * to.Cpad;
                a.o_pr = (long long)to.W * to.Cpad; a.o_pc = to.Cpad;
            } else {
                a.o_bs = (long long)to.H * to.W * to.Cpad; a.o_rs = (long long)to.W * to.Cpad;
            }
        } else {
            const int per = o.out_kind == OUT_CONF ? 3 * C : 12;
            const int per_prior = o.out_kind == OUT_CONF ? C : 4;
            a.out = o.out_kind == OUT_CONF ? io->conf : loc_out(o); a.out_f32 = 1;
            a.o_base = (long long)p.scale_off[o.scale] * per_prior;
            a.o_bs = (long long)p.P * per_prior; a.o_rs = (long long)a.Wo * per; a.o_cs = per;
        }
        if (o.splitk > 1) {
            a.splitk = o.splitk;
            a.partial = (char *)ws + (o.chain >= 0 ? p.chain_partial_off + o.chain_partial : p.splitk_off[o.lane]) * (size_t)B;
        }
    }

    int ensure_f32_input(hipStream_t s)
    {
        if (xin) return TDRN_OK;
        TDRN_TRY(launch_u8_planes_to_f32(u8->planes, B, p.cfg.size, u8->mean, (float *)tptr(p.x_t), s));
        xin = (const float *)tptr(p.x_t);
        return TDRN_OK;
    }

    int launch_first(const Op &f, hipStream_t s) const
    {
        return launch_first_conv(xin, (const float *)(wb + f.w_off), (const float *)(wb + f.b_off), tptr(f.out), B, f.hw, f.stride, f.Cout,
                                 p.tensors[f.out].Cpad, f.relu, p.cfg.dtype, s);
    }

    int run_conv_chain(hipStream_t s)
    {
        ChainLayer cl[16];
        const int nl = (int)p.chain_ops.size();
        for (int k = 0; k < nl; ++k) {
            const Op &m = p.ops[p.chain_ops[k]];
            conv_args(m, cl[k].a);
            int nd = 0;
            for (int t : {m.in, m.res}) {
                if (t < 0) continue;
                int dep = -1;
                for (int j = 0; j < k; ++j)
                    if (p.ops[p.chain_ops[j]].out == t) dep = j;
                if (dep >= 0) cl[k].dep[nd++] = dep;
                else if (lanes && p.tensor_lane[t] != 0) TDRN_HIP_TRY(hipStreamWaitEvent(s, n.tensor_ev[t], 0));
            }
        }
        TDRN_TRY(wait_tail_zeroed());
        TDRN_TRY(launch_conv_chain(cl, nl, (unsigned *)tail, s, n.status));
        for (int k = 1; k < nl; ++k) TDRN_TRY(record(p.ops[p.chain_ops[k]].out, s));
        return TDRN_OK;
    }

    int run_conv(size_t oi, hipStream_t s)
    {
        const Op &o = p.ops[oi];
        ConvArgs a;
        conv_args(o, a);
        if (o.lane == 0 && p.pp_sk_planned) {
            a.sk_ws = tail + kTailCtl;
            a.sk_flags_zero = true;
            if (skz_pending && pp_conv_supported(a)) TDRN_TRY(wait_tail_zeroed());
        }
        const Op &f = p.ops[0];
        if ((int)oi == p.fuse_first) {
            a.fuse_w = (const float *)(wb + f.w_off); a.fuse_b = (const float *)(wb + f.b_off);
            a.fuse_cout = f.Cout;
            if (!xin && o.pool_t >= 0) {
                a.fuse_x8 = u8->planes; a.fuse_mean[0] = u8->mean[0]; a.fuse_mean[1] = u8->mean[1]; a.fuse_mean[2] = u8->mean[2];
                a.out = nullptr;
                const int rc = ws_conv_supported(a) ? launch_conv3x3_ws(a, tptr(o.pool_t), s) : TDRN_E_UNSUPPORTED;
                if (rc != TDRN_E_UNSUPPORTED) return rc;
                a.fuse_x8 = nullptr;
                a.out = tptr(o.out);
            }
            TDRN_TRY(ensure_f32_input(s));
            a.fuse_x = xin;
        }
        if (a.fuse_x && patch_conv_supported(a) <= 0) {
            TDRN_TRY(launch_first(f, s));
            a.fuse_x = nullptr; a.fuse_w = nullptr; a.fuse_b = nullptr; a.fuse_cout = 0;
        }
        if (o.pool_t < 0) return launch_conv(a, s);
        if (patch_conv_supported(a) > 0) {
            a.out = nullptr;
            return launch_conv3x3_patch(a, tptr(o.pool_t), s);
        }
        TDRN_TRY(launch_conv(a, s));
        return launch_maxpool2(a.out, tptr(o.pool_t), B, a.Ho, a.Wo, p.tensors[o.pool_t].Cpad, 0, p.cfg.dtype, s);
    }

    int run_dw(size_t oi, hipStream_t s)
    {
        const Op &o = p.ops[oi];
        const Tensor &ti = p.tensors[o.in];
        if (o.fused_dw) {
            const Op &c = p.ops[oi + 1];
            DwPwArgs a;
            a.in = tptr(o.in); a.w = wb + c.w_off; a.wdw = (const float *)(wb + o.w_off); a.bdw = (const float *)(wb + o.b_off);
            a.bias = (const float *)(wb + c.b_off); a.out = tptr(c.out);
            a.B = B; a.H = ti.H; a.W = ti.W; a.Cin = c.Cin; a.Cout = c.Cout; a.Npad = c.Npad; a.Cs = p.tensors[c.out].Cpad;
            a.stride = o.stride; a.relu_dw = o.relu; a.relu = c.relu; a.dtype = p.cfg.dtype;
            if (dwpw_supported(a)) {
                dwpw_done = true;
                TDRN_TRY(launch_dwpw(a, s));
                return record(c.out, s);
            }
        }
        return launch_dwconv3(tptr(o.in), (const float *)(wb + o.w_off), (const float *)(wb + o.b_off), tptr(o.out), B, ti.H, ti.W, ti.Cpad,
                              o.stride, o.relu, p.cfg.dtype, s, p.kdisable);
    }

    int run_offset(size_t oi, int lane, hipStream_t s)
    {
        const Op &o = p.ops[oi];
        const float *loc;
        long long bs, ps;
        if (o.in >= 0) { loc = (const float *)tptr(o.in); bs = (long long)o.hw * 12; ps = 12; }
        else { loc = io->arm_loc + (size_t)p.scale_off[o.scale] * 4; bs = (long long)p.P * 4; ps = 12; }
        oq[n_oq] = OffsetProblem{loc, bs, ps, (const float *)(wb + o.w_off), (const float *)(wb + o.b_off),
                                 (float *)tptr(o.out), o.in >= 0 ? Bk : B, o.hw, o.off_n, 0};
        oq_op[n_oq++] = (int)oi;
        if (p.launch_continues(oi) && n_oq < 4 && (lanes ? p.ops[oi + 1].lane : 0) == lane) return TDRN_OK;
        TDRN_TRY(launch_offset_conv_multi(oq, n_oq, s));
        for (int i = 0; i + 1 < n_oq; ++i) TDRN_TRY(record(p.ops[oq_op[i]].out, s));
        n_oq = 0;
        return TDRN_OK;
    }

    int run_deform(size_t oi, hipStream_t s)
    {
        const Op &o = p.ops[oi];
        const Tensor &ti = p.tensors[o.in];
        const Tensor &tf = p.tensors[o.off_t];
        DeformArgs a;
        a.in = tptr(o.in); a.zero_page = wb; a.n_branches = o.n_branches;
        const float *off = (const float *)tptr(o.off_t);
        a.br[0] = DeformBranch{off + o.off_c0[0], tf.C, wb + o.w_off, 3, 3, 1, 1, 1, o.G};
        if (o.n_branches == 2) a.br[1] = DeformBranch{off + o.off_c0[1], tf.C, wb + o.w2_off, 5, 5, 2, 1, 1, o.G};
        if (Bk < B)
            for (int k = 0; k < o.n_branches; ++k) a.br[k].off_rows = Bk * ti.H * ti.W;
        a.B = B; a.H = ti.H; a.W = ti.W; a.Cin = o.Cin; a.Ho = ti.H; a.Wo = ti.W; a.Cout = o.Cout; a.Npad = o.Npad;
        a.out0 = loc_out(o) + (size_t)p.scale_off[o.scale] * 4; a.o0_bs = (long long)p.P * 4; a.o0_ps = 12;
        a.out1 = io->conf + (size_t)p.scale_off[o.scale] * C; a.o1_bs = (long long)p.P * C; a.o1_ps = 3 * C;
        a.split = 12; a.dtype = p.cfg.dtype;
        dargs[n_dargs++] = a;
        if (o.y_t >= 0) ts_op[n_dargs - 1] = (int)oi;
        if (p.launch_continues(oi) && n_dargs < 4) return TDRN_OK;
        const int rc = o.y_t >= 0 ? run_deform_ts(s) : run_deform_gather(o, s);
        n_dargs = 0;
        return rc;
    }

    int run_deform_ts(hipStream_t s)
    {
        int Bc = B;
        size_t per_frame = 0;
        for (int i = 0; i < n_dargs; ++i) {
            const Op &d = p.ops[ts_op[i]];
            const int fit = deform_ts_max_batch(dargs[i].H, dargs[i].W, d.y_cols, d.taps);
            Bc = fit < Bc ? fit : Bc;
            per_frame += (size_t)dargs[i].H * dargs[i].W * d.y_cols * p.es;
        }
        if (Bc < 1) return TDRN_E_UNSUPPORTED;
        constexpr size_t kRangeBytes = (size_t)192 << 20;
        if (per_frame > 0 && !(p.kdisable & KOFF_TS_RANGES)) {
            long long fit = (long long)kRangeBytes / (long long)per_frame;
            fit = fit < 1 ? 1 : fit;
            if (fit < Bc) Bc = (int)fit;
        }
        const int n_groups = p.ops[ts_op[0]].y_groups;
        for (int b0 = 0; b0 < B; b0 += Bc)
            for (int yg = 0; yg < n_groups; ++yg) TDRN_TRY(run_deform_ts_range(b0, B - b0 < Bc ? B - b0 : Bc, yg, n_groups, s));
        return TDRN_OK;
    }

    int run_deform_ts_range(int b0, int nb, int yg, int n_groups, hipStream_t s)
    {
        DeformArgs ca[4];
        YGemmProblem yq[4];
        const void *ts_y[4] = {nullptr, nullptr, nullptr, nullptr};
        int ts_cs[4] = {0, 0, 0, 0}, n_yq = 0;
        const int es = p.es, dtype = p.cfg.dtype;
        bool all_ygemm = true;
        for (int i = 0; i < n_dargs; ++i) all_ygemm = all_ygemm && ygemm_supported(p.ops[ts_op[i]].Cin, p.ops[ts_op[i]].y_cols, dtype);
        for (int i = 0; i < n_dargs; ++i) {
            const Op &d = p.ops[ts_op[i]];
            DeformArgs &c = ca[i];
            c = dargs[i];
            const size_t px0 = (size_t)b0 * c.H * c.W;
            c.B = nb;
            c.in = (const char *)c.in + px0 * c.Cin * es;
            for (int k = 0; k < c.n_branches; ++k) {
                if (c.br[k].off_rows) c.br[k].off_row0 = (int)(px0 % (size_t)c.br[k].off_rows);
                else c.br[k].off += px0 * c.br[k].off_stride;
            }
            c.out0 += (size_t)b0 * c.o0_bs;
            c.out1 += (size_t)b0 * c.o1_bs;
            if (d.y_groups != n_groups) return TDRN_E_STATE;
            void *ybuf = tptr(d.y_t) + (size_t)yg * d.y_cols * c.H * c.W * es * B;
            const char *wty = wb + d.wt_off + (size_t)yg * d.y_cols * d.Cin * es;
            const int y_taps = p.y_tap_major ? d.taps : 0;
            c.Cout = d.Cout - 80 * yg < 80 ? d.Cout - 80 * yg : 80;
            if (yg > 0) { c.split = 0; c.out1 += 80 * yg - 12; }
            if (all_ygemm) {
                yq[n_yq++] = YGemmProblem{c.in, wty, ybuf, (long long)nb * c.H * c.W, d.y_cols, d.y_cols, y_taps};
            } else if (ygemm_supported(d.Cin, d.y_cols, dtype)) {
                TDRN_TRY(launch_ygemm(c.in, wty, ybuf, (long long)nb * c.H * c.W, d.y_cols, d.y_cols, dtype, s, y_taps));
            } else {
                ConvArgs g;
                p.conv_geometry(d, nb, g);
                g.Cout = g.Npad = d.y_cols; g.kh = g.kw = 1; g.pad = 0;
                g.in = c.in; g.w = wty; g.bias = (const float *)(wb + d.bt_off); g.zero_page = wb; g.out = ybuf;
                g.o_cs = d.y_cols; g.o_rs = (long long)c.W * d.y_cols; g.o_bs = (long long)c.H * c.W * d.y_cols;
                TDRN_TRY(launch_conv(g, s));
            }
            ts_y[i] = ybuf; ts_cs[i] = d.y_cols;
        }
        if (n_yq > 0) TDRN_TRY(launch_ygemm_multi(yq, n_yq, dtype, s, p.kdisable));
        return launch_deform_sample_multi(ca, ts_y, ts_cs, n_dargs, s, p.y_tap_major ? 1 : 0);
    }

    int run_deform_gather(const Op &o, hipStream_t s)
    {
        if (o.split) {
            if (zeroed_early) TDRN_HIP_TRY(hipStreamWaitEvent(s, n.ev_zero, 0));
            else TDRN_TRY(zero_split_outputs(o, s));
        }
        if (dargs[0].Npad <= 128) return launch_deform_multi(dargs, n_dargs, s, o.split);
        for (int c0 = 0; c0 < dargs[0].Cout; c0 += 128) {
            DeformArgs ga[4];
            for (int i = 0; i < n_dargs; ++i) {
                ga[i] = dargs[i];
                const int cols = dargs[i].Cout - c0 < 128 ? dargs[i].Cout - c0 : 128;
                ga[i].Cout = cols; ga[i].Npad = deform_n_pad(cols);
                for (int k = 0; k < ga[i].n_branches; ++k)
                    ga[i].br[k].w = (const char *)dargs[i].br[k].w + (size_t)c0 * dargs[i].br[k].kh * dargs[i].br[k].kw * dargs[i].Cin * p.es;
                if (c0 > 0) { ga[i].out1 += c0 - dargs[i].split; ga[i].split = 0; }
            }
            TDRN_TRY(launch_deform_multi(ga, n_dargs, s, o.split));
        }
        return TDRN_OK;
    }

    int run_op(size_t oi)
    {
        const Op &o = p.ops[oi];
        if (skipped(oi)) return TDRN_OK;
        int lane;
        hipStream_t s;
        TDRN_TRY(stream_for(o, lane, s));
        if (n.profile && !launch_open(o)) TDRN_HIP_TRY(hipEventRecord(n.ev[evi], s));
        const Tensor *ti = o.in >= 0 ? &p.tensors[o.in] : nullptr;
        switch (o.kind) {
            case OP_FIRST:
                TDRN_TRY(ensure_f32_input(s));
                TDRN_TRY(launch_first(o, s));
                break;
            case OP_CONV: TDRN_TRY(o.chain >= 0 ? run_conv_chain(s) : run_conv(oi, s)); break;
            case OP_POOL:
                TDRN_TRY(launch_maxpool2(tptr(o.in), tptr(o.out), B, ti->H, ti->W, ti->Cpad, o.ceil, p.cfg.dtype, s));
                break;
            case OP_L2NORM:
                TDRN_TRY(launch_l2norm(tptr(o.in), (const float *)(wb + o.w_off), tptr(o.out), (long long)B * ti->H * ti->W, ti->Cpad, p.cfg.dtype, s));
                break;
            case OP_DW: TDRN_TRY(run_dw(oi, s)); break;
            case OP_REFLOC_IN:
                if (!io->ref_loc[o.scale]) return TDRN_E_ARG;
                if (io->reserved[2]) TDRN_HIP_TRY(hipStreamWaitEvent(s, (hipEvent_t)io->reserved[2], 0));
                TDRN_TRY(launch_nchw_to_nhwc(io->ref_loc[o.scale], tptr(o.out), Bk, 12, o.hw, 12, TDRN_F32, s));
                break;
            case OP_OFFSET: TDRN_TRY(run_offset(oi, lane, s)); break;
            case OP_DEFORM: TDRN_TRY(run_deform(oi, s)); break;
            case OP_SOFTMAX: TDRN_TRY(launch_softmax_rows(io->conf, io->conf, (long long)B * p.P, C, s)); break;
            case OP_OFF_OUT:
                TDRN_TRY(launch_nhwc_to_nchw_f32((const float *)tptr(o.in), (long long)ti->H * ti->W * ti->C, ti->C, io->offsets[o.scale], Bk, o.Cout,
                                                 ti->H * ti->W, s));
                break;
            case OP_LOC_OUT:
                TDRN_TRY(launch_nhwc_to_nchw_f32(io->arm_loc + (size_t)p.scale_off[o.scale] * 4, (long long)p.P * 4, 12, io->loc_maps[o.scale], B, 12,
                                                 p.fm[o.scale] * p.fm[o.scale], s));
                break;
        }
        offset_ops_enqueued += o.kind == OP_OFFSET;
        if (!launch_open(o)) TDRN_TRY(record(o.out, s));
        TDRN_TRY(record(o.pool_t, s));
        if (n.profile && !launch_open(o)) {
            TDRN_HIP_TRY(hipEventRecord(n.ev[evi + 1], s));
            n.ev_stat.push_back(o.stat);
            n.ev_op.push_back((int)oi);
            evi += 2;
        }
        return TDRN_OK;
    }
};

}

int run_forward(tdrn_net &n, const void *blob, void *ws, size_t ws_bytes, const tdrn_net_io *io, hipStream_t s0)
{
    Run r(n, blob, ws, ws_bytes, io, s0);
    TDRN_TRY(r.prologue());
    for (size_t oi = 0; oi < n.ops.size(); ++oi) TDRN_TRY(r.run_op(oi));
    return r.epilogue();
}

}
```

Before: 12690 frames/s.

## Group paired trans_layers 3x3 convs into one multi-problem patch kernel launch

Adds a multi-problem variant of the 3x3 patch conv kernel that takes up to four independent conv problems and maps a flat item index to each problem's geometry. The planner pairs the trans_layers.0 and trans_layers.1 convs at each half into one launch on lane 1, and the runner issues that single grouped launch while skipping the member op. This aims to cut launch count and let small, under-filled convs share one grid so more CUs stay busy. In exchange the kernel does per-item problem lookups and recomputes weight offsets, which adds register pressure and branching. It also forces these ops onto a single lane, which may remove overlap they had before.

```diff
diff --git a/include/tdrn_hip.h b/include/tdrn_hip.h
--- a/include/tdrn_hip.h
+++ b/include/tdrn_hip.h
@@ -199,6 +199,7 @@
 #define TDRN_PLAN_NO_HEAD3X3   32768
 #define TDRN_PLAN_TS_ONE_RANGE  65536
 #define TDRN_PLAN_NO_PATCH_TAIL 131072
+#define TDRN_PLAN_NO_PATCH_GROUP 262144
 #define TDRN_PLAN_FAULT_HANDOFF 256
 
 typedef struct tdrn_net tdrn_net;
diff --git a/tdrn_amd/_lib.py b/tdrn_amd/_lib.py
--- a/tdrn_amd/_lib.py
+++ b/tdrn_amd/_lib.py
@@ -29,7 +29,7 @@
 PLAN_NO_FUSE_FIRST, PLAN_NO_LATE_SIDE, PLAN_ONE_STREAM, PLAN_NO_DEFORM_TS, PLAN_CHAIN = 1, 2, 4, 8, 16
 PLAN_NO_CONV_PP, PLAN_NO_PP_SK, PLAN_NO_CONV_PATCH, PLAN_FAULT_HANDOFF, PLAN_DWPW, PLAN_NO_PW1X1 = 32, 64, 128, 256, 512, 1024
 PLAN_NO_DW_SLIDE, PLAN_DW_SLIDE_ALL, PLAN_NO_CONV_WS, PLAN_NO_YGEMM_V2, PLAN_NO_HEAD3X3, PLAN_TS_ONE_RANGE = 2048, 4096, 8192, 16384, 32768, 65536
-PLAN_NO_PATCH_TAIL = 131072
+PLAN_NO_PATCH_TAIL, PLAN_NO_PATCH_GROUP = 131072, 262144
 E_DEVICE = -8
 
 
diff --git a/tdrn_amd/csrc/conv3x3_patch.hip b/tdrn_amd/csrc/conv3x3_patch.hip
--- a/tdrn_amd/csrc/conv3x3_patch.hip
+++ b/tdrn_amd/csrc/conv3x3_patch.hip
@@ -36,6 +36,32 @@
 #endif
 };
 
+constexpr int kMaxPatchProblems = 4;
+struct PatchProb {
+    const char *in, *w;
+    const float *bias;
+    char *out;
+    int H, W, Cin, Cout, Cs, Ktot, M;
+    int relu;
+    int tiles_x, tiles_per_img, n_tiles;
+    int q;
+    static constexpr char *out_pool = nullptr;
+};
+struct PatchMulti {
+    PatchProb pr[kMaxPatchProblems];
+    int start[kMaxPatchProblems + 1];
+    int n;
+    const char *zero;
+    int items;
+    int tail_split;
+#ifdef TDRN_PATCH_STAMP
+    unsigned *stamps;
+#endif
+#ifdef TDRN_PATCH_WGTIME
+    unsigned long long *wgt;
+#endif
+};
+
 #ifdef TDRN_PATCH_STAMP
 #define STAMP_DECL unsigned long long st_t = __builtin_amdgcn_s_memtime(); unsigned st_acc[8] = {0, 0, 0, 0, 0, 0, 0, 0};
 #define STAMP(k) do { const unsigned long long t_ = __builtin_amdgcn_s_memtime(); st_acc[k] += (unsigned)(t_ - st_t); st_t = t_; } while (0)
@@ -57,10 +83,19 @@
 
 }
 
-template <typename DT, int BN, int TW, bool FUSE = false>
-__global__ __launch_bounds__(768) void conv3x3_patch_kernel(const PatchParams p)
+template <bool MULTI, typename P> __device__ __forceinline__ decltype(auto) patch_first_view(const P &p)
 {
+    if constexpr (MULTI) return PatchProb(p.pr[0]);
+    else return (p);
+}
+
+template <typename DT, int BN, int TW, bool FUSE = false, typename P = PatchParams>
+__global__ __launch_bounds__(768) void conv3x3_patch_kernel(const P p)
+{
+    constexpr bool MULTI = !std::is_same_v<P, PatchParams>;
     static_assert(!FUSE || (BN == 64 && TW == 32 && sizeof(DT) == 2), "fused first conv: 16-bit, 64 couts, 8x32 tiles");
+    static_assert(!MULTI || (BN == 128 && !FUSE), "multi-problem launches: 128-cout items, no fused first conv");
+    using View = std::conditional_t<MULTI, PatchProb, const PatchParams &>;
     constexpr bool FLAT = TW == 0;
     constexpr int LGTW = TW == 32 ? 5 : 4;
     constexpr int TPX = FUSE ? 512 : 256;
@@ -95,7 +130,7 @@
 
     const int lane = threadIdx.x & 63;
     const int wave = __builtin_amdgcn_readfirstlane(threadIdx.x >> 6);
-    const int nchunks = p.Cin / CK;
+    const int nchunks = patch_first_view<MULTI>(p).Cin / CK;
 #ifdef TDRN_PATCH_WGTIME
     if (threadIdx.x == 0) p.wgt[2 * blockIdx.x] = __builtin_amdgcn_s_memrealtime();
 #endif
@@ -121,19 +156,49 @@
         }
     }
     const int n_it = n_full + n_tail;
-    const int n_steps = n_it * nchunks * 9;
-    auto item_mt = [&](int it) { return (it < n_full ? item0 + it * istride : tail_enc >> 1) / p.n_tiles; };
-    auto item_c0 = [&](int it) {
+    auto item_in = [&](int it, auto &v) -> int {
         const int item = it < n_full ? item0 + it * istride : tail_enc >> 1;
-        return (item % p.n_tiles) * BN + (it < n_full ? 0 : (tail_enc & 1) * 64);
-    };
-    const int RS = TW ? TW + 2 : p.W;
+        if constexpr (MULTI) {
+            int q = 0;
+#pragma unroll
+            for (int k = 1; k < kMaxPatchProblems; ++k)
+                if (k < p.n && item >= p.start[k]) q = k;
+            v = p.pr[q];
+            return item - p.start[q];
+        } else {
+            return item;
+        }
+    };
+    auto item_mt = [&](int it, auto &v) { return item_in(it, v) / v.n_tiles; };
+    auto item_c0 = [&](int it, auto &v) { return (item_in(it, v) % v.n_tiles) * BN + (it < n_full ? 0 : (tail_enc & 1) * 64); };
+    auto tile_key = [](auto &v, int mt) -> int {
+        if constexpr (MULTI) return (v.q << 24) | mt;
+        else return mt;
+    };
+    auto item_nch = [&](int it) -> int {
+        if constexpr (MULTI) {
+            PatchProb t = p.pr[0];
+            item_in(it, t);
+            return t.Cin / CK;
+        } else {
+            return nchunks;
+        }
+    };
+    auto count_steps = [&](int n) -> int {
+        int k = 0;
+        for (int it = 0; it < n; ++it) k += item_nch(it) * 9;
+        return k;
+    };
+    int n_steps = n_it * nchunks * 9;
+    if constexpr (MULTI) n_steps = count_steps(n_it);
+    const int RS = TW ? TW + 2 : patch_first_view<MULTI>(p).W;
 
     if (wave >= 8) {
         if (TDRN_PATCH_PRIO == 4) __builtin_amdgcn_s_setprio(2);
         if (TDRN_PATCH_PRIO == 5) __builtin_amdgcn_s_setprio(3);
         const int lw = wave - 8;
         const int lrow = lane >> 3, pc = lane & 7;
+        View wv = patch_first_view<MULTI>(p), pv = patch_first_view<MULTI>(p), bv = patch_first_view<MULTI>(p);
         unsigned poff[kSlotsPerLoader];
         int pyx[kSlotsPerLoader];
         int plc[kSlotsPerLoader];
@@ -146,7 +211,7 @@
                     const int py = pr / RS, px = pr - py * RS;
                     pyx[j] = py < TH + 2 ? ((py << 16) | px) : -1;
                 } else {
-                    pyx[j] = pr < 256 + 2 * p.W + 2 ? pr : -1;
+                    pyx[j] = MULTI || pr < 256 + 2 * pv.W + 2 ? pr : -1;
                 }
             }
         }
@@ -183,9 +248,9 @@
             if (lw == 0) ((float *)(smem + OFF_R + 2 * RAWB))[lane] = lane < p.fCout ? p.fb[lane] : 0.f;
         }
         auto tile_origin = [&](int item, int &b, int &y0, int &x0) {
-            const int mt = item / p.n_tiles;
-            b = mt / p.tiles_per_img;
-            const int tt = mt - b * p.tiles_per_img, ty = tt / p.tiles_x, tx = tt - ty * p.tiles_x;
+            const int mt = item / pv.n_tiles;
+            b = mt / pv.tiles_per_img;
+            const int tt = mt - b * pv.tiles_per_img, ty = tt / pv.tiles_x, tx = tt - ty * pv.tiles_x;
             y0 = ty * TH; x0 = tx * TW;
         };
         auto load_raw = [&](int item, int buf) -> int {
@@ -258,25 +323,26 @@
         };
         int table_mt = -1;
         auto patch_table = [&](int mt) {
-            if (mt == table_mt) return;
-            table_mt = mt;
-            const long long rowbytes = (long long)p.Cin * ES;
+            const int key = tile_key(pv, mt);
+            if (key == table_mt) return;
+            table_mt = key;
+            const long long rowbytes = (long long)pv.Cin * ES;
             if (TW) {
-                const int b = mt / p.tiles_per_img, tt = mt - b * p.tiles_per_img;
-                const int ty = tt / p.tiles_x, tx = tt - ty * p.tiles_x;
+                const int b = mt / pv.tiles_per_img, tt = mt - b * pv.tiles_per_img;
+                const int ty = tt / pv.tiles_x, tx = tt - ty * pv.tiles_x;
                 const int y0 = ty * TH - 1, x0 = tx * TW - 1;
 #pragma unroll
                 for (int j = 0; j < kSlotsPerLoader; ++j) {
                     const int y = y0 + (pyx[j] >> 16), x = x0 + (pyx[j] & 0xffff);
-                    const bool ok = pyx[j] >= 0 && (unsigned)y < (unsigned)p.H && (unsigned)x < (unsigned)p.W;
-                    poff[j] = ok ? (unsigned)((((long long)b * p.H + y) * p.W + x) * rowbytes + plc[j]) : 0xFFFFFFFFu;
+                    const bool ok = pyx[j] >= 0 && (unsigned)y < (unsigned)pv.H && (unsigned)x < (unsigned)pv.W;
+                    poff[j] = ok ? (unsigned)((((long long)b * pv.H + y) * pv.W + x) * rowbytes + plc[j]) : 0xFFFFFFFFu;
                 }
             } else {
-                const long long j0 = (long long)mt * 256 - p.W - 1;
+                const long long j0 = (long long)mt * 256 - pv.W - 1;
 #pragma unroll
                 for (int j = 0; j < kSlotsPerLoader; ++j) {
                     const long long pix = j0 + pyx[j];
-                    const bool ok = pyx[j] >= 0 && pix >= 0 && pix < p.M;
+                    const bool ok = pyx[j] >= 0 && (!MULTI || pyx[j] < 256 + 2 * pv.W + 2) && pix >= 0 && pix < pv.M;
                     poff[j] = ok ? (unsigned)(pix * rowbytes + plc[j]) : 0xFFFFFFFFu;
                 }
             }
@@ -285,15 +351,27 @@
 #pragma unroll
         for (int k = 0; k < WL; ++k) {
             const int n = (lw + 4 * k) * 8 + lrow;
-            woff[k] = (unsigned)((size_t)n * p.Ktot * ES + ((pc ^ ((n >> 1) & 7)) << 4));
+            woff[k] = (unsigned)((size_t)n * wv.Ktot * ES + ((pc ^ ((n >> 1) & 7)) << 4));
         }
         constexpr bool live = !(TDRN_PATCH_ABLATE & 1);
         int ws = 0, w_it = 0, w_cc = 0, w_tap = 0, wslot = 0;
-        const char *wbase = p.w;
+        const char *wbase = wv.w;
         unsigned wk = 0;
         int w_pieces = WL;
         auto weight_item = [&]() {
-            wbase = p.w + (size_t)item_c0(w_it) * p.Ktot * ES;
+            if constexpr (MULTI) {
+                const int c0 = item_c0(w_it, wv);
+                wbase = wv.w + (size_t)c0 * wv.Ktot * ES;
+            } else {
+                wbase = wv.w + (size_t)item_c0(w_it, wv) * wv.Ktot * ES;
+            }
+            if constexpr (MULTI) {
+#pragma unroll
+                for (int k = 0; k < WL; ++k) {
+                    const int n = (lw + 4 * k) * 8 + lrow;
+                    woff[k] = (unsigned)((size_t)n * wv.Ktot * ES + ((pc ^ ((n >> 1) & 7)) << 4));
+                }
+            }
             if constexpr (TAILOK) w_pieces = w_it < n_full ? WL : WL / 2;
         };
         constexpr bool wfixed = (TDRN_PATCH_ABLATE & 16) != 0, pfixed = (TDRN_PATCH_ABLATE & 32) != 0;
@@ -303,14 +381,14 @@
                 char *dst = smem + OFF_W + wslot * WBYTES;
 #pragma unroll
                 for (int k = 0; k < WL; ++k)
-                    if (!TAILOK || k < np) lds_dma16_ptr(wfixed ? p.w + (woff[k] & 0xffffu) : wbase + wk + woff[k], dst + (lw + 4 * k) * 1024);
+                    if (!TAILOK || k < np) lds_dma16_ptr(wfixed ? wv.w + (woff[k] & 0xffffu) : wbase + wk + woff[k], dst + (lw + 4 * k) * 1024);
             }
             ++ws;
             wslot = wslot == RING - 1 ? 0 : wslot + 1;
-            wk += (unsigned)(p.Cin * ES);
+            wk += (unsigned)(wv.Cin * ES);
             if (++w_tap == 9) {
                 w_tap = 0;
-                if (++w_cc == nchunks) {
+                if (++w_cc == (MULTI ? wv.Cin / CK : nchunks)) {
                     w_cc = 0;
                     ++w_it;
                     if (w_it < n_it) weight_item();
@@ -322,12 +400,12 @@
         auto load_patch = [&](int j, unsigned ccoff, char *dstbuf) {
             if (!live || lw + 4 * j >= kPatchSlots || FUSE) return;
             const unsigned o = poff[j];
-            lds_dma16_ptr(o == 0xFFFFFFFFu ? p.zero : (pfixed ? p.in + (o & 0xfffffu) : p.in + (size_t)o + ccoff), dstbuf + (lw + 4 * j) * 1024);
+            lds_dma16_ptr(o == 0xFFFFFFFFu ? p.zero : (pfixed ? pv.in + (o & 0xfffffu) : pv.in + (size_t)o + ccoff), dstbuf + (lw + 4 * j) * 1024);
         };
         int p_it = 0, p_cc = 0, pbuf = 0;
         auto next_patch_chunk = [&]() {
             if (NPB == 2) pbuf ^= 1;
-            if (++p_cc == nchunks) {
+            if (++p_cc == (MULTI ? pv.Cin / CK : nchunks)) {
                 p_cc = 0;
                 ++p_it;
             }
@@ -348,7 +426,7 @@
         if (n_it > 0) {
             weight_item();
             if constexpr (!FUSE) {
-                patch_table(item_mt(0));
+                patch_table(item_mt(0, pv));
 #pragma unroll
                 for (int j = 0; j < kSlotsPerLoader; ++j) load_patch(j, 0u, smem);
             }
@@ -356,13 +434,16 @@
             for (int k = 0; k < RING - 1; ++k)
                 if (k < n_steps) load_weights();
             next_patch_chunk();
+            if constexpr (MULTI) item_in(0, bv);
             if (lw == 0 && live)
-                lds_dma16_ptr(lane < (n_full > 0 ? BN : 64) / 4 ? (const char *)(p.bias + item_c0(0)) + lane * 16 : p.zero, smem + OFF_B);
+                lds_dma16_ptr(lane < (n_full > 0 ? BN : 64) / 4 ? (const char *)(bv.bias + item_c0(0, bv)) + lane * 16 : p.zero, smem + OFF_B);
         }
         asm volatile("s_waitcnt vmcnt(0) lgkmcnt(0)" ::: "memory");
         __builtin_amdgcn_s_barrier();
 
         int tap = 0, c_it = 0, c_cc = 0, carried = 0;
+        int c_nch = nchunks;
+        if constexpr (MULTI) if (n_it > 0) c_nch = item_nch(0);
         STAMP_DECL
         const int last_piece = lw + 4 * (kSlotsPerLoader - 1) < kPatchSlots ? 1 : 0;
         for (int g = 0; g < n_steps; ++g) {
@@ -375,7 +456,7 @@
                 const unsigned ccoff = (unsigned)(p_cc * 128);
                 switch (tap) {
                     case 0:
-                        patch_table(item_mt(p_it));
+                        patch_table(item_mt(p_it, pv));
                         load_patch(0, ccoff, dstbuf); load_patch(1, ccoff, dstbuf); issued += 2; break;
                     case 1: load_patch(2, ccoff, dstbuf); load_patch(3, ccoff, dstbuf); issued += 2; break;
                     case 2: load_patch(4, ccoff, dstbuf); load_patch(5, ccoff, dstbuf); issued += 2; break;
@@ -384,8 +465,9 @@
                     default: load_patch(10, ccoff, dstbuf); issued += last_piece; break;
                 }
             }
-            if (lw == 0 && c_cc == nchunks - 1 && tap == 6 && c_it + 1 < n_it) {
-                if (live) lds_dma16_ptr(lane < (c_it + 1 < n_full ? BN : 64) / 4 ? (const char *)(p.bias + item_c0(c_it + 1)) + lane * 16 : p.zero, smem + OFF_B);
+            if (lw == 0 && c_cc == c_nch - 1 && tap == 6 && c_it + 1 < n_it) {
+                if constexpr (MULTI) item_in(c_it + 1, bv);
+                if (live) lds_dma16_ptr(lane < (c_it + 1 < n_full ? BN : 64) / 4 ? (const char *)(bv.bias + item_c0(c_it + 1, bv)) + lane * 16 : p.zero, smem + OFF_B);
                 issued += 1;
             }
             STAMP(0);
@@ -398,7 +480,7 @@
             if (++tap == 9) {
                 tap = 0;
                 next_patch_chunk();
-                if (++c_cc == nchunks) {
+                if (++c_cc == c_nch) {
                     if constexpr (FUSE) {
                         if (c_it + 1 < n_it) {
                             int b_;
@@ -412,6 +494,7 @@
                     }
                     c_cc = 0;
                     ++c_it;
+                    if constexpr (MULTI) if (c_it < n_it) c_nch = item_nch(c_it);
                 }
             }
         }
@@ -439,20 +522,27 @@
     const int my_ch = lane % CPR, my_row = lane / CPR;
     constexpr bool compute = !(TDRN_PATCH_ABLATE & 2);
 
+    View cv = patch_first_view<MULTI>(p);
     int cur_mt = -1, n0 = 0;
+    int c_nch = nchunks, rs = RS;
     long long tile_pix0 = 0;
     int tile_row0 = 0, tile_x0 = 0;
     auto setup_item = [&](int it) {
-        const int mt = item_mt(it);
-        n0 = item_c0(it);
-        if (mt == cur_mt) return;
-        cur_mt = mt;
+        const int mt = item_mt(it, cv);
+        n0 = item_c0(it, cv);
+        if constexpr (MULTI) {
+            c_nch = cv.Cin / CK;
+            if (!TW) rs = cv.W;
+        }
+        const int key = tile_key(cv, mt);
+        if (key == cur_mt) return;
+        cur_mt = key;
         if (TW) {
-            const int b = mt / p.tiles_per_img, tt = mt - b * p.tiles_per_img;
-            const int ty = tt / p.tiles_x, tx = tt - ty * p.tiles_x;
-            tile_row0 = b * p.H + ty * TH;
+            const int b = mt / cv.tiles_per_img, tt = mt - b * cv.tiles_per_img;
+            const int ty = tt / cv.tiles_x, tx = tt - ty * cv.tiles_x;
+            tile_row0 = b * cv.H + ty * TH;
             tile_x0 = tx * TW;
-            tile_pix0 = (long long)tile_row0 * p.W + tile_x0;
+            tile_pix0 = (long long)tile_row0 * cv.W + tile_x0;
             return;
         }
         tile_pix0 = (long long)mt * 256;
@@ -461,13 +551,13 @@
         for (int pt = 0; pt < 2; ++pt) {
             const long long m = tile_pix0 + cw * 64 + pt * 32 + r32;
             unsigned mk = 0;
-            if (m < p.M) {
-                const int rem = (int)(m % ((long long)p.H * p.W));
-                const int y = rem / p.W, x = rem - y * p.W;
+            if (m < cv.M) {
+                const int rem = (int)(m % ((long long)cv.H * cv.W));
+                const int y = rem / cv.W, x = rem - y * cv.W;
 #pragma unroll
                 for (int t = 0; t < 9; ++t) {
                     const int yy = y + t / 3 - 1, xx = x + t % 3 - 1;
-                    if ((unsigned)yy < (unsigned)p.H && (unsigned)xx < (unsigned)p.W) mk |= 1u << t;
+                    if ((unsigned)yy < (unsigned)cv.H && (unsigned)xx < (unsigned)cv.W) mk |= 1u << t;
                 }
             }
             tapmask[pt] = mk;
@@ -480,7 +570,7 @@
     };
 
     typedef short pk_s2 __attribute__((ext_vector_type(2)));
-    [[maybe_unused]] const pk_s2 relu_lo = p.relu ? pk_s2{0, 0} : pk_s2{(short)-32768, (short)-32768};
+    [[maybe_unused]] pk_s2 relu_lo = cv.relu ? pk_s2{0, 0} : pk_s2{(short)-32768, (short)-32768};
     auto pack_relu16 = [&](float a, float b) -> unsigned {
         if constexpr (sizeof(DT) == 2) return __builtin_bit_cast(unsigned, __builtin_elementwise_max(__builtin_bit_cast(pk_s2, pack2<DT>(a, b)), relu_lo));
         else return 0u;
@@ -490,14 +580,14 @@
             constexpr int WCN = decltype(wcn_tag)::value;
             const int cbase = n0 + chalf * (32 * WCN);
             constexpr int NPAIR = 2 * WCN;
-            if (p.out && !(TDRN_PATCH_ABLATE & 4)) {
+            if (cv.out && !(TDRN_PATCH_ABLATE & 4)) {
 #pragma unroll
                 for (int pt = 0; pt < 2; ++pt) {
                     const int i = cw * 64 + pt * 32 + r32;
                     long long gp;
-                    if (TW) gp = tile_pix0 + (long long)(i >> LGTW) * p.W + (i & (TW - 1));
-                    else { gp = tile_pix0 + i; if (gp >= p.M) gp = -1; }
-                    char *row = p.out + ((size_t)(gp < 0 ? 0 : gp) * p.Cs + cbase) * 2;
+                    if (TW) gp = tile_pix0 + (long long)(i >> LGTW) * cv.W + (i & (TW - 1));
+                    else { gp = tile_pix0 + i; if (gp >= cv.M) gp = -1; }
+                    char *row = cv.out + ((size_t)(gp < 0 ? 0 : gp) * cv.Cs + cbase) * 2;
 #pragma unroll
                     for (int pr = 0; pr < NPAIR; ++pr) {
                         const int ci = pr >> 1, g0 = 2 * (pr & 1);
@@ -506,13 +596,13 @@
                         const unsigned bx = pack_relu16(t[4 * g0 + 4], t[4 * g0 + 5]), by = pack_relu16(t[4 * g0 + 6], t[4 * g0 + 7]);
                         auto rx = __builtin_amdgcn_permlane32_swap(ax, bx, false, false);
                         auto ry = __builtin_amdgcn_permlane32_swap(ay, by, false, false);
-                        if (gp >= 0 && cbase + (2 * pr + hh) * 8 < p.Cout)
+                        if (gp >= 0 && cbase + (2 * pr + hh) * 8 < cv.Cout)
                             *(u32x4 *)(row + (2 * pr + hh) * 16) = u32x4{rx[0], ry[0], rx[1], ry[1]};
                     }
                 }
             }
-            if constexpr (TW != 0) if (p.out_pool) {
-                const int PW = p.W >> 1;
+            if constexpr (TW != 0) if (cv.out_pool) {
+                const int PW = cv.W >> 1;
 #pragma unroll
                 for (int pt = 0; pt < 2; ++pt) {
                     if (TW == 32 && pt == 1) break;
@@ -539,7 +629,7 @@
                         }
                     const int i = cw * 64 + pt * 32 + r32;
                     const long long gpool = (long long)((tile_row0 + (i >> LGTW)) >> 1) * PW + ((tile_x0 + (i & (TW - 1))) >> 1);
-                    char *row = p.out_pool + ((size_t)gpool * p.Cs + cbase) * 2;
+                    char *row = cv.out_pool + ((size_t)gpool * cv.Cs + cbase) * 2;
                     constexpr int NDUP = TW == 32 ? 2 : 4;
                     const int sel = TW == 32 ? (r32 & 1) : ((r32 & 1) | ((r32 >> 3) & 2));
 #pragma unroll
@@ -557,7 +647,7 @@
                         const int mypr = rd * NDUP + sel;
                         auto rx = __builtin_amdgcn_permlane32_swap(a.x, b.x, false, false);
                         auto ry = __builtin_amdgcn_permlane32_swap(a.y, b.y, false, false);
-                        if (mypr < NPAIR && cbase + (2 * mypr + hh) * 8 < p.Cout)
+                        if (mypr < NPAIR && cbase + (2 * mypr + hh) * 8 < cv.Cout)
                             *(u32x4 *)(row + (2 * mypr + hh) * 16) = u32x4{rx[0], ry[0], rx[1], ry[1]};
                     }
                 }
@@ -569,14 +659,14 @@
         if constexpr (sizeof(DT) == 2) { epilogue16(wcn_tag); return; }
         const int my_c = n0 + chalf * BNH + my_ch * P16;
         auto pixel_of = [&](int i) -> long long {
-            if (TW) return tile_pix0 + (long long)(i >> LGTW) * p.W + (i & (TW - 1));
+            if (TW) return tile_pix0 + (long long)(i >> LGTW) * cv.W + (i & (TW - 1));
             const long long m = tile_pix0 + i;
-            return m < p.M ? m : -1;
+            return m < cv.M ? m : -1;
         };
         auto stage_quad = [&](const f32x16 &t, int ci, int g, int srow) {
             float q4[4];
 #pragma unroll
-            for (int j = 0; j < 4; ++j) q4[j] = p.relu ? fmaxf(t[4 * g + j], 0.f) : t[4 * g + j];
+            for (int j = 0; j < 4; ++j) q4[j] = cv.relu ? fmaxf(t[4 * g + j], 0.f) : t[4 * g + j];
             char *d = stg + srow * SSTRIDE + (ci * 32 + 8 * g + 4 * hh) * ES;
             if constexpr (ES == 4) {
                 *(f32x4 *)d = f32x4{q4[0], q4[1], q4[2], q4[3]};
@@ -592,7 +682,7 @@
                 *(uint2 *)d = make_uint2(__builtin_bit_cast(unsigned, lo), __builtin_bit_cast(unsigned, hi));
             }
         };
-        if (p.out && !(TDRN_PATCH_ABLATE & 4)) {
+        if (cv.out && !(TDRN_PATCH_ABLATE & 4)) {
 #pragma unroll
             for (int pt = 0; pt < 2; ++pt) {
 #pragma unroll 1
@@ -609,15 +699,15 @@
                     for (int k = 0; k < SROWS / RPI; ++k) {
                         const int row = my_row + k * RPI;
                         const long long gp = pixel_of(cw * 64 + pt * 32 + rd * SROWS + row);
-                        if (gp >= 0 && my_c < p.Cout)
-                            *(u32x4 *)(p.out + ((size_t)gp * p.Cs + my_c) * ES) = *(const u32x4 *)(stg + row * SSTRIDE + my_ch * 16);
+                        if (gp >= 0 && my_c < cv.Cout)
+                            *(u32x4 *)(cv.out + ((size_t)gp * cv.Cs + my_c) * ES) = *(const u32x4 *)(stg + row * SSTRIDE + my_ch * 16);
                     }
                     __builtin_amdgcn_wave_barrier();
                 }
             }
         }
-        if (p.out_pool) {
-            const int PW = p.W >> 1;
+        if (cv.out_pool) {
+            const int PW = cv.W >> 1;
             constexpr int npool = TW == 32 ? 16 : 8;
             const bool holder = (r32 & 1) == 0 && (TW == 32 || r32 < 16);
             const int prow_l = r32 >> 1;
@@ -648,11 +738,11 @@
 #pragma unroll
                     for (int k = 0; k < SROWS / RPI; ++k) {
                         const int row = my_row + k * RPI;
-                        if (row < rows_here && my_c < p.Cout) {
+                        if (row < rows_here && my_c < cv.Cout) {
                             const int pl = rd * SROWS + row;
                             const int i0 = cw * 64 + pt * 32 + 2 * pl;
                             const long long gpool = (long long)((tile_row0 + (i0 >> LGTW)) >> 1) * PW + ((tile_x0 + (i0 & (TW - 1))) >> 1);
-                            *(u32x4 *)(p.out_pool + ((size_t)gpool * p.Cs + my_c) * ES) = *(const u32x4 *)(stg + row * SSTRIDE + my_ch * 16);
+                            *(u32x4 *)(cv.out_pool + ((size_t)gpool * cv.Cs + my_c) * ES) = *(const u32x4 *)(stg + row * SSTRIDE + my_ch * 16);
                         }
                     }
                     __builtin_amdgcn_wave_barrier();
@@ -713,6 +803,7 @@
     typedef std::integral_constant<int, 1> half_t;
     if (n_it > 0) {
         setup_item(0);
+        if constexpr (MULTI) relu_lo = cv.relu ? pk_s2{0, 0} : pk_s2{(short)-32768, (short)-32768};
         init_acc(full_t{});
         load_frags(full_t{}, wfA, pfA, 0);
     }
@@ -741,17 +832,17 @@
         STAMP(0);
         __builtin_amdgcn_s_barrier();
         STAMP(1);
-        const bool item_done = tap == 8 && cc == nchunks - 1;
+        const bool item_done = tap == 8 && cc == c_nch - 1;
         wslot = wslot == RING - 1 ? 0 : wslot + 1;
         ++tap;
         if (++tq == 3) {
             tq = 0;
-            delta += RS;
+            delta += rs;
         }
         if (tap == 9) {
             tap = 0; tq = 0; delta = 0;
             pbuf ^= 1;
-            if (++cc == nchunks) cc = 0;
+            if (++cc == c_nch) cc = 0;
         }
         wsb = smem + OFF_W + wslot * WBYTES;
         psb = smem + (NPB == 2 ? pbuf : 0) * PBYTES;
@@ -771,6 +862,7 @@
             ++it;
             if (it < n_it) {
                 setup_item(it);
+                if constexpr (MULTI) relu_lo = cv.relu ? pk_s2{0, 0} : pk_s2{(short)-32768, (short)-32768};
                 if (TAILOK && it >= n_full) {
                     init_acc(half_t{});
                     load_frags(half_t{}, wfA, pfA, 0);
@@ -785,7 +877,8 @@
             STAMP(3);
         }
     };
-    const int n_steps_full = n_full * nchunks * 9;
+    int n_steps_full = n_full * nchunks * 9;
+    if constexpr (MULTI) n_steps_full = count_steps(n_full);
 #pragma unroll 1
     for (int g = 0; g < n_steps_full; ++g) step(full_t{});
     if constexpr (TAILOK) {
@@ -932,4 +1025,73 @@
     return TDRN_E_ARG;
 }
 
+int patch_multi_member(const ConvArgs &a)
+{
+    const int mode = patch_conv_supported(a);
+    if (!mode || a.fuse_x || a.fuse_x8 || a.Npad % 128 || !a.out) return 0;
+    return mode;
 }
+
+int patch_items128(const ConvArgs &a)
+{
+    const int mode = patch_conv_supported(a);
+    int tiles_x, tiles_per_img, m_tiles;
+    conv_tiles(a.B, a.H, a.W, mode > 0 ? mode : 0, 256, tiles_x, tiles_per_img, m_tiles);
+    return m_tiles * (a.Npad / 128);
+}
+
+template <typename DT> static int launch_patch_multi_cfg(const PatchMulti &mp, int tw, hipStream_t s)
+{
+    const int grid = persistent_grid(mp.items);
+    if (tw == 0) hipLaunchKernelGGL((conv3x3_patch_kernel<DT, 128, 0, false, PatchMulti>), dim3(grid), dim3(768), 0, s, mp);
+    else if (tw == 32) hipLaunchKernelGGL((conv3x3_patch_kernel<DT, 128, 32, false, PatchMulti>), dim3(grid), dim3(768), 0, s, mp);
+    else hipLaunchKernelGGL((conv3x3_patch_kernel<DT, 128, 16, false, PatchMulti>), dim3(grid), dim3(768), 0, s, mp);
+    return hip_status(hipGetLastError());
+}
+
+int launch_conv3x3_patch_multi(const ConvArgs *a, int n, hipStream_t s)
+{
+    if (n < 1 || n > kMaxPatchProblems) return TDRN_E_ARG;
+    if (n == 1) return launch_conv3x3_patch(a[0], nullptr, s);
+    const int mode = patch_multi_member(a[0]);
+    if (!mode) return TDRN_E_UNSUPPORTED;
+    int order[kMaxPatchProblems];
+    for (int i = 0; i < n; ++i) {
+        if (patch_multi_member(a[i]) != mode || a[i].dtype != a[0].dtype || a[i].zero_page != a[0].zero_page) return TDRN_E_UNSUPPORTED;
+        int k = i;
+        for (; k > 0 && a[order[k - 1]].Cin < a[i].Cin; --k) order[k] = order[k - 1];
+        order[k] = i;
+    }
+    PatchMulti mp;
+    const int tw = mode > 0 ? mode : 0;
+    mp.start[0] = 0;
+    for (int i = 0; i < n; ++i) {
+        const ConvArgs &c = a[order[i]];
+        PatchProb &q = mp.pr[i];
+        q.in = (const char *)c.in; q.w = (const char *)c.w; q.bias = c.bias; q.out = (char *)c.out;
+        q.H = c.H; q.W = c.W; q.Cin = c.Cin; q.Cout = c.Cout; q.Cs = (int)c.o_cs; q.Ktot = 9 * c.Cin; q.M = c.B * c.H * c.W;
+        q.relu = c.relu;
+        int m_tiles;
+        conv_tiles(c.B, c.H, c.W, tw, 256, q.tiles_x, q.tiles_per_img, m_tiles);
+        q.n_tiles = c.Npad / 128;
+        q.q = i;
+        mp.start[i + 1] = mp.start[i] + m_tiles * q.n_tiles;
+    }
+    for (int i = n; i < kMaxPatchProblems; ++i) { mp.pr[i] = mp.pr[0]; mp.pr[i].q = i; mp.start[i + 1] = mp.start[n]; }
+    mp.n = n;
+    mp.zero = (const char *)a[0].zero_page;
+    mp.items = mp.start[n];
+    mp.tail_split = !(a[0].kdisable & KOFF_PATCH_TAIL);
+    if (mp.items <= 0) return TDRN_OK;
+#if defined(TDRN_PATCH_STAMP) || defined(TDRN_PATCH_WGTIME)
+    return TDRN_E_UNSUPPORTED;
+#endif
+    switch (a[0].dtype) {
+        case TDRN_F32: return launch_patch_multi_cfg<float>(mp, tw, s);
+        case TDRN_BF16: return launch_patch_multi_cfg<bf16_t>(mp, tw, s);
+        case TDRN_F16: return launch_patch_multi_cfg<f16_t>(mp, tw, s);
+    }
+    return TDRN_E_ARG;
+}
+
+}
diff --git a/tdrn_amd/csrc/conv3x3_pp.hip b/tdrn_amd/csrc/conv3x3_pp.hip
--- a/tdrn_amd/csrc/conv3x3_pp.hip
+++ b/tdrn_amd/csrc/conv3x3_pp.hip
@@ -495,6 +495,17 @@
     return patch_conv_supported(a);
 }
 
+constexpr int kPpMinItems = 192;
+
+int pp_conv_takes(const ConvArgs &a)
+{
+    const int mode = pp_conv_supported(a);
+    if (!mode) return 0;
+    int tiles_x, tiles_per_img, m_tiles;
+    conv_tiles(a.B, a.H, a.W, mode > 0 ? mode : 0, 256, tiles_x, tiles_per_img, m_tiles);
+    return m_tiles * (a.Npad / 256) >= kPpMinItems;
+}
+
 int launch_conv3x3_pp(const ConvArgs &a, hipStream_t s)
 {
     const int mode = pp_conv_supported(a);
@@ -511,7 +522,7 @@
     p.items = p.m_tiles * p.n_tiles;
     p.n_major = p.n_tiles > 1 ? 1 : 0;
     if (p.items <= 0) return TDRN_OK;
-    if (p.items < 192) return TDRN_E_UNSUPPORTED;
+    if (p.items < kPpMinItems) return TDRN_E_UNSUPPORTED;
     const int grid = persistent_grid(p.items);
     p.sk_slab = nullptr; p.sk_flag = nullptr;
     p.status = a.status; p.fault = a.fault_handoff; p.poll_max = a.fault_handoff ? (1u << 10) : (1u << 20);
diff --git a/tdrn_amd/csrc/kernels.h b/tdrn_amd/csrc/kernels.h
--- a/tdrn_amd/csrc/kernels.h
+++ b/tdrn_amd/csrc/kernels.h
@@ -58,7 +58,12 @@
 int patch_conv_supported(const ConvArgs &a);
 int patch_conv_takes(const ConvArgs &a);
 int launch_conv3x3_patch(const ConvArgs &a, void *out_pool, hipStream_t s);
+constexpr int kMaxPatchGroup = 4;
+int patch_multi_member(const ConvArgs &a);
+int patch_items128(const ConvArgs &a);
+int launch_conv3x3_patch_multi(const ConvArgs *a, int n, hipStream_t s);
 int pp_conv_supported(const ConvArgs &a);
+int pp_conv_takes(const ConvArgs &a);
 int launch_conv3x3_pp(const ConvArgs &a, hipStream_t s);
 size_t conv_pp_sk_bytes();
 int ws_conv_supported(const ConvArgs &a);
diff --git a/tdrn_amd/csrc/net.h b/tdrn_amd/csrc/net.h
--- a/tdrn_amd/csrc/net.h
+++ b/tdrn_amd/csrc/net.h
@@ -8,6 +8,8 @@
     std::vector<hipEvent_t> ev;
     std::vector<int> ev_stat;
     std::vector<int> ev_op;
+    std::vector<int> ev_slot;
+    std::vector<float> ev_share;
     tdrn_kernel_stat stats[tdrn::ST_COUNT];
     int last_batch = 0;
     const void *offs_ws = nullptr;
diff --git a/tdrn_amd/csrc/net.hip b/tdrn_amd/csrc/net.hip
--- a/tdrn_amd/csrc/net.hip
+++ b/tdrn_amd/csrc/net.hip
@@ -98,9 +98,10 @@
     }
     for (size_t i = 0; i < ev_stat.size(); ++i) {
         float ms = 0.f;
-        TDRN_HIP_TRY(hipEventSynchronize(ev[2 * i + 1]));
-        TDRN_HIP_TRY(hipEventElapsedTime(&ms, ev[2 * i], ev[2 * i + 1]));
-        stats[ev_stat[i]].ms += ms;
+        const int sl = ev_slot[i];
+        TDRN_HIP_TRY(hipEventSynchronize(ev[2 * sl + 1]));
+        TDRN_HIP_TRY(hipEventElapsedTime(&ms, ev[2 * sl], ev[2 * sl + 1]));
+        stats[ev_stat[i]].ms += ms * ev_share[i];
     }
     int n = 0;
     for (int i = 0; i < ST_COUNT && n < max_entries; ++i)
@@ -293,12 +294,25 @@
     for (size_t i = 0; i < net->ev_op.size() && n < max_entries; ++i) {
         const Op &o = net->ops[net->ev_op[i]];
         float ms = 0.f;
-        TDRN_HIP_TRY(hipEventSynchronize(net->ev[2 * i + 1]));
-        TDRN_HIP_TRY(hipEventElapsedTime(&ms, net->ev[2 * i], net->ev[2 * i + 1]));
+        const int sl = net->ev_slot[i];
+        TDRN_HIP_TRY(hipEventSynchronize(net->ev[2 * sl + 1]));
+        TDRN_HIP_TRY(hipEventElapsedTime(&ms, net->ev[2 * sl], net->ev[2 * sl + 1]));
         tdrn_kernel_stat &k = out[n++];
         memset(&k, 0, sizeof(k));
         std::string name = std::string(kStatNames[o.stat]) + ":" + (o.w.empty() ? (o.in >= 0 ? net->tensors[o.in].label : "") : o.w);
         if (o.kind == OP_CONV && o.chain == 0) name = "conv_chain:" + o.w + "+" + std::to_string(net->chain_ops.size() - 1);
+        if (net->ev_share[i] < 1.f && o.group_head >= 0) {
+            const std::string &h = net->ops[o.group_head].w;
+            std::string rest, hs = h;
+            for (int m = net->ops[o.group_head].group_next; m >= 0; m = net->ops[m].group_next) {
+                const std::string &w = net->ops[m].w;
+                size_t c = 0, dot = 0;
+                while (c < w.size() && c < h.size() && w[c] == h[c]) { if (w[c] == '.') dot = c + 1; ++c; }
+                rest += "+" + w.substr(dot);
+                hs = h.substr(dot);
+            }
+            name = std::string(kStatNames[o.stat]) + ":" + (o.group_head == net->ev_op[i] ? h + rest : o.w + "@" + hs + rest);
+        }
         strncpy(k.name, name.c_str(), sizeof(k.name) - 1);
         k.launches = 1;
         k.flops = o.flops * net->last_batch;
@@ -313,7 +327,7 @@
                 k.flops += net->ops[j].flops * net->last_batch;
                 k.bytes += net->ops[j].bytes * net->last_batch;
             }
-        k.ms = ms;
+        k.ms = ms * net->ev_share[i];
     }
     return n;
 }
@@ -323,9 +337,10 @@
     if (!net || !start_ms || !end_ms || max_entries <= 0) return TDRN_E_ARG;
     int n = 0;
     for (size_t i = 0; i < net->ev_op.size() && n < max_entries; ++i, ++n) {
-        TDRN_HIP_TRY(hipEventSynchronize(net->ev[2 * i + 1]));
-        TDRN_HIP_TRY(hipEventElapsedTime(&start_ms[n], net->ev[0], net->ev[2 * i]));
-        TDRN_HIP_TRY(hipEventElapsedTime(&end_ms[n], net->ev[0], net->ev[2 * i + 1]));
+        const int sl = net->ev_slot[i];
+        TDRN_HIP_TRY(hipEventSynchronize(net->ev[2 * sl + 1]));
+        TDRN_HIP_TRY(hipEventElapsedTime(&start_ms[n], net->ev[0], net->ev[2 * sl]));
+        TDRN_HIP_TRY(hipEventElapsedTime(&end_ms[n], net->ev[0], net->ev[2 * sl + 1]));
         if (lane) lane[n] = net->profile == 2 && net->use_lanes ? net->ops[net->ev_op[i]].lane : 0;
     }
     return n;
diff --git a/tdrn_amd/csrc/net_plan.h b/tdrn_amd/csrc/net_plan.h
--- a/tdrn_amd/csrc/net_plan.h
+++ b/tdrn_amd/csrc/net_plan.h
@@ -40,6 +40,7 @@
     int chain = -1;
     int fused_dw = 0;
     size_t chain_partial = 0;
+    int group_head = -1, group_next = -1;
 };
 
 constexpr int kLanes = 4;
@@ -80,7 +81,7 @@
     bool launch_head(size_t i) const
     {
         const Op &o = ops[i];
-        return !(i > 0 && launch_continues(i - 1)) && !(o.kind == OP_CONV && (o.chain > 0 || o.fused_dw));
+        return !(i > 0 && launch_continues(i - 1)) && !(o.kind == OP_CONV && (o.chain > 0 || o.fused_dw || (o.group_head >= 0 && o.group_head != (int)i)));
     }
 
 private:
@@ -122,6 +123,7 @@
     void plan_fuse_first();
     void plan_splitk();
     void plan_chain();
+    void plan_patch_groups();
     void place_splitk_slabs();
     void plan_dwpw();
     void plan_workspace_tail();
diff --git a/tdrn_amd/csrc/net_plan.hip b/tdrn_amd/csrc/net_plan.hip
--- a/tdrn_amd/csrc/net_plan.hip
+++ b/tdrn_amd/csrc/net_plan.hip
@@ -547,6 +547,38 @@
     for (size_t k = 0; k < chain_ops.size(); ++k) ops[chain_ops[k]].chain = (int)k;
 }
 
+void Plan::plan_patch_groups()
+{
+    if ((cfg.plan_flags & TDRN_PLAN_NO_PATCH_GROUP) || (kdisable & KOFF_CONV_PATCH)) return;
+    auto find = [&](const std::string &w) {
+        for (size_t i = 0; i < ops.size(); ++i)
+            if (ops[i].kind == OP_CONV && ops[i].w == w) return (int)i;
+        return -1;
+    };
+    auto mode_of = [&](int i) {
+        if (i < 0) return 0;
+        const Op &o = ops[i];
+        if (o.stat != ST_CONV3 || o.splitk != 1 || o.res >= 0 || o.pool_t >= 0 || o.out_kind != OUT_TENSOR || o.chain >= 0 || o.fused_dw ||
+            i == fuse_first || o.k != 3) return 0;
+        ConvArgs a;
+        conv_geometry(o, 1, a);
+        a.o_cs = tensors[o.out].Cpad; a.o_rs = (long long)a.Wo * a.o_cs; a.o_bs = (long long)a.Ho * a.Wo * a.o_cs;
+        a.out = (void *)1;
+        return patch_multi_member(a);
+    };
+    int prev_tail = -1;
+    for (const char *half : {".0", ".2"}) {
+        const int a = find(std::string("trans_layers.0") + half), b = find(std::string("trans_layers.1") + half);
+        const int ma = mode_of(a), mb = mode_of(b);
+        if (!ma || ma != mb) return;
+        if (b < a || (prev_tail >= 0 && a < prev_tail)) return;
+        ops[a].group_head = ops[b].group_head = a;
+        ops[a].group_next = b;
+        ops[a].lane = ops[b].lane = 1;
+        prev_tail = a;
+    }
+}
+
 void Plan::place_splitk_slabs()
 {
     size_t lane_bytes[kLanes] = {0, 0, 0, 0};
@@ -568,8 +600,9 @@
         if (atoi(pd))
             for (const Op &o : ops)
                 if (o.kind == OP_CONV)
-                    fprintf(stderr, "plan: %-28s lane %d  %dx%d k%d s%d d%d  Cin %4d Cout %4d  splitk %d  %s  chain %d\n", o.w.c_str(), o.lane,
-                            o.hw >> 16, o.hw & 0xffff, o.k, o.stride, o.dil, o.Cin, o.Cout, o.splitk, o.stat == ST_CONV3 ? "patch" : "igemm", o.chain);
+                    fprintf(stderr, "plan: %-28s lane %d  %dx%d k%d s%d d%d  Cin %4d Cout %4d  splitk %d  %s  chain %d%s\n", o.w.c_str(), o.lane,
+                            o.hw >> 16, o.hw & 0xffff, o.k, o.stride, o.dil, o.Cin, o.Cout, o.splitk, o.stat == ST_CONV3 ? "patch" : "igemm", o.chain,
+                            o.group_head < 0 ? "" : (ops[o.group_head].w == o.w ? "  group head" : "  group member"));
     }
     for (int l = 0; l < kLanes; ++l) {
         splitk_off[l] = ws_per_sample;
@@ -659,6 +692,7 @@
     plan_fuse_first();
     plan_splitk();
     plan_chain();
+    plan_patch_groups();
     place_splitk_slabs();
     plan_dwpw();
     plan_workspace_tail();
diff --git a/tdrn_amd/csrc/net_run.hip b/tdrn_amd/csrc/net_run.hip
--- a/tdrn_amd/csrc/net_run.hip
+++ b/tdrn_amd/csrc/net_run.hip
@@ -22,6 +22,9 @@
     int oq_op[4], n_oq = 0;
     size_t evi = 0;
     int offset_ops_enqueued = 0;
+    int group_issued[4] = {-1, -1, -1, -1}, n_group_issued = 0;
+    float group_share[kMaxPatchGroup];
+    int group_ops[kMaxPatchGroup], n_group_ops = 0;
 
     Run(tdrn_net &net, const void *blob_, void *ws_, size_t ws_bytes_, const tdrn_net_io *io_, hipStream_t s)
         : n(net), p(net), blob(blob_), ws(ws_), ws_bytes(ws_bytes_), io(io_), s0(s) {}
@@ -85,6 +88,8 @@
         }
         n.ev_stat.clear();
         n.ev_op.clear();
+        n.ev_slot.clear();
+        n.ev_share.clear();
         lanes = p.use_lanes && n.profile != 1;
         if (lanes) {
             TDRN_TRY(n.init_lanes());
@@ -181,6 +186,9 @@
         if (reuse_offsets && (o.kind == OP_REFLOC_IN || o.kind == OP_OFFSET)) return true;
         if (o.kind == OP_FIRST && p.fuse_first >= 0) return true;
         if (o.kind == OP_CONV && o.chain > 0) return true;
+        if (o.kind == OP_CONV && o.group_head >= 0 && o.group_head != (int)oi)
+            for (int k = 0; k < n_group_issued; ++k)
+                if (group_issued[k] == o.group_head) return true;
         return (int)oi < n.first_op;
     }
 
@@ -308,6 +316,32 @@
         }
         TDRN_TRY(launch_conv(a, s));
         return launch_maxpool2(a.out, tptr(o.pool_t), B, a.Ho, a.Wo, p.tensors[o.pool_t].Cpad, 0, p.cfg.dtype, s);
+    }
+
+    int run_patch_group(size_t oi, int lane, hipStream_t s)
+    {
+        ConvArgs ca[kMaxPatchGroup];
+        int items = 0;
+        n_group_ops = 0;
+        for (int m = (int)oi; m >= 0 && n_group_ops < kMaxPatchGroup; m = p.ops[m].group_next) {
+            conv_args(p.ops[m], ca[n_group_ops]);
+            if (!patch_multi_member(ca[n_group_ops])) return TDRN_E_UNSUPPORTED;
+            if (pp_conv_takes(ca[n_group_ops])) return TDRN_E_UNSUPPORTED;
+            group_share[n_group_ops] = (float)patch_items128(ca[n_group_ops]);
+            items += patch_items128(ca[n_group_ops]);
+            group_ops[n_group_ops++] = m;
+        }
+        if (n_group_ops < 2 || items <= 0 || n_group_issued == 4) return TDRN_E_UNSUPPORTED;
+        for (int k = 0; k < n_group_ops; ++k) group_share[k] /= (float)items;
+        if (lanes)
+            for (int k = 1; k < n_group_ops; ++k) {
+                const int t = p.ops[group_ops[k]].in;
+                if (p.tensor_lane[t] != lane) TDRN_HIP_TRY(hipStreamWaitEvent(s, n.tensor_ev[t], 0));
+            }
+        TDRN_TRY(launch_conv3x3_patch_multi(ca, n_group_ops, s));
+        for (int k = 1; k < n_group_ops; ++k) TDRN_TRY(record(p.ops[group_ops[k]].out, s));
+        group_issued[n_group_issued++] = (int)oi;
+        return TDRN_OK;
     }
 
     int run_dw(size_t oi, hipStream_t s)
@@ -472,12 +506,20 @@
         TDRN_TRY(stream_for(o, lane, s));
         if (n.profile && !launch_open(o)) TDRN_HIP_TRY(hipEventRecord(n.ev[evi], s));
         const Tensor *ti = o.in >= 0 ? &p.tensors[o.in] : nullptr;
+        bool grouped = false;
         switch (o.kind) {
             case OP_FIRST:
                 TDRN_TRY(ensure_f32_input(s));
                 TDRN_TRY(launch_first(o, s));
                 break;
-            case OP_CONV: TDRN_TRY(o.chain >= 0 ? run_conv_chain(s) : run_conv(oi, s)); break;
+            case OP_CONV:
+                if (o.group_head == (int)oi && (int)oi >= n.first_op) {
+                    const int rc = run_patch_group(oi, lane, s);
+                    grouped = rc == TDRN_OK;
+                    if (rc != TDRN_E_UNSUPPORTED) { TDRN_TRY(rc); break; }
+                }
+                TDRN_TRY(o.chain >= 0 ? run_conv_chain(s) : run_conv(oi, s));
+                break;
             case OP_POOL:
                 TDRN_TRY(launch_maxpool2(tptr(o.in), tptr(o.out), B, ti->H, ti->W, ti->Cpad, o.ceil, p.cfg.dtype, s));
                 break;
@@ -507,8 +549,12 @@
         TDRN_TRY(record(o.pool_t, s));
         if (n.profile && !launch_open(o)) {
             TDRN_HIP_TRY(hipEventRecord(n.ev[evi + 1], s));
-            n.ev_stat.push_back(o.stat);
-            n.ev_op.push_back((int)oi);
+            for (int k = 0; k < (grouped ? n_group_ops : 1); ++k) {
+                n.ev_stat.push_back(grouped ? p.ops[group_ops[k]].stat : o.stat);
+                n.ev_op.push_back(grouped ? group_ops[k] : (int)oi);
+                n.ev_slot.push_back((int)(evi / 2));
+                n.ev_share.push_back(grouped ? group_share[k] : 1.f);
+            }
             evi += 2;
         }
         return TDRN_OK;
```

After: 12540 frames/s. -1.2%, worse.
